# zeropoolnetwork/fawkes-crypto

Hardware: AMD Instinct MI355X
Metric: Groth16 proofs/sec + MSM scalar-muls/sec, BN254, 2^25 constraints (33552553 rows = 99.99 % of the 2^25 domain) (higher is better)
Workload: dtype u32

## Files before the change

### fawkes-crypto_amd/csrc/common.hpp

```cpp
#pragma once
#include <hip/hip_runtime.h>
#include <stdint.h>
#include <stdio.h>
#include <stdlib.h>
#include <map>
#include <string>
#include <new>
#include <stdexcept>
#include <type_traits>
#include <vector>
#include <functional>
#include <initializer_list>
#include "../../include/fawkes_hip.h"
#include "curve.hpp"

namespace fk {

struct DevBuf {
    void *p = nullptr;
    size_t cap = 0;
    hipError_t reserve(size_t bytes) {
        if (bytes <= cap) return hipSuccess;
        if (p) { hipError_t e = hipFree(p); p = nullptr; cap = 0; if (e != hipSuccess) return e; }
        size_t want = bytes + (bytes >> 3) + 256;
        hipError_t e = hipMalloc(&p, want);
        if (e != hipSuccess) { (void)hipGetLastError(); e = hipMalloc(&p, bytes); want = bytes; }
        if (e == hipSuccess) cap = want; else { p = nullptr; (void)hipGetLastError(); }
        return e;
    }
    void release() { if (p) (void)hipFree(p); p = nullptr; cap = 0; }
    template <class T> T *as() const { return (T *)p; }
};

struct CtxScratch {
    DevBuf misc;
    DevBuf ntt_s1, ntt_s2, ntt_io, hbuf, sc_a, sc_b, scan_tmp, stage_a, stage_b, stage_c, stage_z, stage_d;
    DevBuf check;
    DevBuf *begin() { return &misc; }
    DevBuf *end() { return begin() + sizeof(CtxScratch) / sizeof(DevBuf); }
    void release_scratch() { for (DevBuf *b = begin(); b != end(); ++b) b->release(); }
};
static_assert(std::is_standard_layout<CtxScratch>::value && sizeof(CtxScratch) % sizeof(DevBuf) == 0, "CtxScratch holds DevBuf members and nothing else");

struct NttDomain;

struct EventPair { hipEvent_t a, b; uint64_t units; };

struct MsmLane {
    hipStream_t st = nullptr;
    hipEvent_t ev_in = nullptr;
    hipEvent_t ev_sorted = nullptr;
    bool ev_sorted_valid = false;
    DevBuf digits, sorted, totals, starts, perm, overlist, tasktab, partials, s2_cnt1, s2_seg, s2_cnt2, s2_tmp_idx, s2_tmp_lo, buckets;
    DevBuf buckets2;
    const void *last_sort_scalars = nullptr; size_t last_sort_n = 0; unsigned last_sort_c = 0; bool last_merged = false;
};

struct MsmTail {
    bool active = false;
    uint32_t cb = 0, wide = 0, W = 0, nblk = 0;
    hipEvent_t done = nullptr;
    void *h_wp = nullptr;
    size_t h_cap = 0;
    DevBuf d_wp;
};
static constexpr int MSM_TAILS = 12;
static constexpr int MSM_LANES = 4;

struct QueryIdx {
    const uint32_t *a = nullptr, *b = nullptr;
    uint64_t n_a = 0, n_b = 0;
};

struct WitnessQueries {
    const uint8_t *d_a_aux = nullptr, *d_b_in = nullptr, *d_b_aux = nullptr;
    const QueryIdx *idx = nullptr;
};
struct FrontOpts {
    bool defer_back = false;
    bool gather_on_main = false;
};
struct ProveRun {
    WitnessQueries q;
    bool z_recorded = false;
    const std::function<int()> *before_block = nullptr;
};

struct KeyPre {
    void *lev = nullptr;
    size_t n = 0;
    uint32_t cb = 0, wide = 0, W = 0;
};

}

struct fk_ctx : fk::CtxScratch {
    int device = 0;
    hipStream_t stream = nullptr;
    std::string err;
    unsigned window_bits = 0;
    unsigned ntt_threads = 512;
    std::map<uint32_t, fk::NttDomain *> domains;
    fk::MsmLane lanes[fk::MSM_LANES];
    int lane_next = 0, lane_prev = 0;
    int co_tenants = 1;
    int lanes_in_use = fk::MSM_LANES;
    fk::MsmTail tails[fk::MSM_TAILS];
    hipStream_t aux = nullptr;
    hipEvent_t ev_aux = nullptr, ev_main = nullptr, ev_z = nullptr;
    std::vector<std::function<int()>> deferred, deferred_tails;
    hipEvent_t ev_acc_done = nullptr; bool ev_acc_done_valid = false;
    bool wit_active = false;
    struct EarlyFront { bool done = false; int tails[4] = {-1, -1, -1, -1}; const fk_key *key = nullptr; const struct fk_r1cs_dev *r1cs = nullptr; const void *d_z = nullptr; } early;
    int wit_tail[4] = {-1, -1, -1, -1};
    hipStream_t copy_st = nullptr;
    struct WitSlot {
        fk::DevBuf buf; hipEvent_t ready = nullptr; bool pending = false;
        hipEvent_t part = nullptr;
        bool deferred = false; const void *host_z = nullptr; size_t host_bytes = 0;
        const fk_key *key = nullptr; const struct fk_r1cs_dev *r1cs = nullptr; uint64_t r[4], s[4];
    } wslot[2];
    int wslot_next = 0;
    hipEvent_t ev_upload_gate = nullptr;
    hipEvent_t ev_chunk[16] = {nullptr};
    std::vector<fk::EventPair> ev_acc, ev_acc2, ev_ntt;
    std::vector<hipEvent_t> ev_pool;
    uint64_t acc_adds[2] = {0, 0};
    bool stats_on = true;
    bool debug = false;
};

struct fk_key {
    uint64_t m = 0;
    uint32_t num_input = 0, num_aux = 0;
    uint64_t n_h = 0, n_l = 0, n_a = 0, n_b = 0;
    uint32_t shard_index = 0, shard_count = 1;
    uint64_t h_lo = 0, h_hi = 0, l_lo = 0, l_hi = 0, a_lo = 0, a_hi = 0, b_lo = 0, b_hi = 0;
    uint64_t b2_lo = 0, b2_hi = 0;
    fk::G1Affine *d_h = nullptr, *d_l = nullptr, *d_a = nullptr, *d_b1 = nullptr;
    fk::G2Affine *d_b2 = nullptr;
    fk::G1Affine alpha_g1, beta_g1, delta_g1;
    fk::G2Affine beta_g2, delta_g2;
    fk::KeyPre pre_h, pre_l, pre_a, pre_b1, pre_b2;
    double load_s[2] = {0, 0};
};

#define FK_SET_ERR(ctx, code, ...)                                   \
    do {                                                             \
        char _b[512]; snprintf(_b, sizeof _b, __VA_ARGS__);          \
        (ctx)->err = _b;                                             \
        return (code);                                               \
    } while (0)

#define FK_HIP(ctx, expr)                                                                         \
    do {                                                                                          \
        hipError_t _e = (expr);                                                                   \
        if (_e != hipSuccess) {                                                                   \
            char _b[512];                                                                         \
            snprintf(_b, sizeof _b, "%s:%d: %s -> %s", __FILE__, __LINE__, #expr, hipGetErrorString(_e)); \
            (ctx)->err = _b;                                                                      \
            (void)hipGetLastError();    \
            return (_e == hipErrorOutOfMemory) ? FK_ERR_OOM : FK_ERR_HIP;                         \
        }                                                                                         \
    } while (0)

#define FK_DBG(ctx, name)                                                                         \
    do {                                                                                          \
        if ((ctx)->debug) {                                                                       \
            fprintf(stderr, "[fk] launch %s ...", name); fflush(stderr);                          \
            hipError_t _e = hipStreamSynchronize((ctx)->stream);                                  \
            fprintf(stderr, " %s\n", hipGetErrorString(_e)); fflush(stderr);                      \
        }                                                                                         \
    } while (0)

#define FK_TRY(expr) do { int _rc = (expr); if (_rc != FK_OK) return _rc; } while (0)
#define FK_CAT2_(a, b) a##b
#define FK_CAT_(a, b) FK_CAT2_(a, b)
#define FK_RANGE(name) fk::RoctxRange FK_CAT_(fk_range_, __LINE__)(name)

namespace fk {
static inline bool proof_holds_staging(const fk_ctx *ctx) { return ctx->early.done; }
static inline bool proof_holds_lanes(const fk_ctx *ctx) {
    return proof_holds_staging(ctx) || ctx->wit_active || !ctx->deferred.empty() || !ctx->deferred_tails.empty();
}

static inline int scratch_claim(fk_ctx *ctx, const char *who) {
    if (proof_holds_staging(ctx)) FK_SET_ERR(ctx, FK_ERR_BAD_ARG, "%s: an early front of a submitted proof is outstanding (call fk_prove_r1cs_wait first)", who);
    FK_HIP(ctx, hipSetDevice(ctx->device));
    return FK_OK;
}

struct HostStage {
    fk_ctx *ctx;
    size_t align = 16;
    uint8_t *cur = nullptr;
    size_t up(size_t bytes) const { return (bytes + align - 1) & ~(align - 1); }
    int use(DevBuf &buf, std::initializer_list<size_t> sizes, size_t slack = 0) {
        size_t sum = slack;
        for (size_t b : sizes) sum += up(b);
        FK_HIP(ctx, buf.reserve(sum));
        cur = buf.as<uint8_t>();
        return FK_OK;
    }
    template <class T> T *room(size_t bytes) { T *p = (T *)cur; cur += up(bytes); return p; }
    template <class T> int in(const void *host, size_t bytes, T **d) {
        *d = room<T>(bytes);
        if (bytes) FK_HIP(ctx, hipMemcpyAsync((void *)*d, host, bytes, hipMemcpyHostToDevice, ctx->stream));
        return FK_OK;
    }
    template <class T> int room(DevBuf &buf, size_t bytes, T **d) { FK_TRY(use(buf, {bytes})); *d = room<T>(bytes); return FK_OK; }
    template <class T> int in(DevBuf &buf, const void *host, size_t bytes, T **d) { FK_TRY(use(buf, {bytes})); return in(host, bytes, d); }
    int out(void *host, const void *d, size_t bytes, bool last = true) {
        FK_HIP(ctx, hipMemcpyAsync(host, d, bytes, hipMemcpyDeviceToHost, ctx->stream));
        if (last) FK_HIP(ctx, hipStreamSynchronize(ctx->stream));
        return FK_OK;
    }
};
}

template <class C, class F>
static inline int fk_guard(C *c, F &&body) noexcept {
    auto note = [&](const char *msg) noexcept { if (c) { try { c->err = msg; } catch (...) {} } };
    try { return body(); }
    catch (const std::bad_alloc &) { note("out of host memory"); return FK_ERR_OOM; }
    catch (const std::length_error &) { note("out of host memory (a container larger than this host can hold)"); return FK_ERR_OOM; }
    catch (const std::exception &e) { note(e.what()); return FK_ERR_HIP; }
    catch (...) { note("unknown C++ exception"); return FK_ERR_HIP; }
}

namespace fk {

std::string &tls_error();
unsigned host_threads();

struct RoctxApi { int (*push)(const char *) = nullptr; int (*pop)() = nullptr; };
const RoctxApi &roctx_api();
struct RoctxRange {
    bool on;
    explicit RoctxRange(const char *name) { const RoctxApi &r = roctx_api(); on = r.push != nullptr; if (on) (void)r.push(name); }
    ~RoctxRange() { if (on) (void)roctx_api().pop(); }
    RoctxRange(const RoctxRange &) = delete;
    RoctxRange &operator=(const RoctxRange &) = delete;
};

static inline int tune(const char *name, int dflt) {
#ifdef FK_EXPERIMENTS
    const char *e = getenv(name);
    return e ? atoi(e) : dflt;
#else
    (void)name;
    return dflt;
#endif
}

static inline uint32_t ceil_log2_u64(uint64_t n) { uint32_t k = 0; while (((uint64_t)1 << k) < n) k++; return k; }

static inline void h_slice(uint64_t n_h, uint32_t idx, uint32_t cnt, uint64_t *lo, uint64_t *hi) {
    const uint64_t m = n_h + 1;
    uint64_t a = (uint64_t)((unsigned __int128)m * idx / cnt), b = (uint64_t)((unsigned __int128)m * (idx + 1) / cnt);
    if (a > n_h) a = n_h;
    if (b > n_h) b = n_h;
    *lo = a; *hi = b;
}

static inline void work_slices(uint64_t n_l, uint64_t n_a, uint64_t n_b, uint32_t index, uint32_t count, uint64_t out[8], long double handicap = 0.0L) {
    const long double seg_w[4] = {1.0L, 1.0L, 1.0L, (long double)FK_G2_WORK};
    const uint64_t seg_n[4] = {n_l, n_a, n_b, n_b};
    long double total = 0; for (int i = 0; i < 4; i++) total += seg_w[i] * (long double)seg_n[i];
    auto cut = [&](uint32_t g, int seg) -> uint64_t {
        if (g >= count) return seg_n[seg];
        if (g == 0) return 0;
        long double x;
        if (handicap > 0 && count > 1 && handicap * (long double)count >= total + handicap)
            x = total * (long double)(g - 1) / (long double)(count - 1);
        else
            x = (total + handicap) * (long double)g / (long double)count - handicap;
        long double s0 = 0; for (int i = 0; i < seg; i++) s0 += seg_w[i] * (long double)seg_n[i];
        if (x <= s0) return 0;
        const long double q = (x - s0) / seg_w[seg];
        return q >= (long double)seg_n[seg] ? seg_n[seg] : (uint64_t)q;
    };
    for (int seg = 0; seg < 4; seg++) { out[2 * seg] = cut(index, seg); out[2 * seg + 1] = cut(index + 1, seg); }
}

static inline int key_plan_slices(fk_ctx *ctx, fk_key *k, double zlo, double zhi) {
    h_slice(k->n_h, k->shard_index, k->shard_count, &k->h_lo, &k->h_hi);
    auto eq = [&](uint64_t n, uint64_t *lo, uint64_t *hi) {
        *lo = (uint64_t)((unsigned __int128)n * k->shard_index / k->shard_count);
        *hi = (uint64_t)((unsigned __int128)n * (k->shard_index + 1) / k->shard_count);
    };
    auto fr = [&](uint64_t n, uint64_t *olo, uint64_t *ohi) {
        uint64_t a = (uint64_t)((long double)n * zlo + 0.5L), b = zhi >= 1.0 ? n : (uint64_t)((long double)n * zhi + 0.5L);
        if (a > n) a = n;
        if (b > n) b = n;
        if (b < a) b = a;
        *olo = a; *ohi = b;
    };
    if (zlo <= -1.5) {
        uint64_t r[8];
        const bool q0 = zlo <= -2.5 && k->shard_count > 1;
        if (q0) { k->h_lo = k->shard_index == 0 ? 0 : k->n_h; k->h_hi = k->n_h; }
        work_slices(k->n_l, k->n_a, k->n_b, k->shard_index, k->shard_count, r, q0 ? (long double)FK_Q0_HANDICAP * (long double)k->m : 0.0L);
        k->l_lo = r[0]; k->l_hi = r[1]; k->a_lo = r[2]; k->a_hi = r[3]; k->b_lo = r[4]; k->b_hi = r[5]; k->b2_lo = r[6]; k->b2_hi = r[7];
        return FK_OK;
    }
    if (zlo < 0.0) { eq(k->n_l, &k->l_lo, &k->l_hi); eq(k->n_a, &k->a_lo, &k->a_hi); eq(k->n_b, &k->b_lo, &k->b_hi); k->b2_lo = k->b_lo; k->b2_hi = k->b_hi; return FK_OK; }
    if (!(zhi <= 1.0 && zlo <= zhi)) FK_SET_ERR(ctx, FK_ERR_BAD_ARG, "key: bad z fraction range [%g, %g)", zlo, zhi);
    if (k->shard_count == 1 && !(zlo == 0.0 && zhi >= 1.0))
        FK_SET_ERR(ctx, FK_ERR_BAD_ARG, "key: a single shard holds the whole arrays (z_frac_lo = FK_Z_EQUAL_SPLIT or [0, 1)), got [%g, %g)", zlo, zhi);
    fr(k->n_l, &k->l_lo, &k->l_hi); fr(k->n_a, &k->a_lo, &k->a_hi); fr(k->n_b, &k->b_lo, &k->b_hi);
    k->b2_lo = k->b_lo; k->b2_hi = k->b_hi;
    return FK_OK;
}

int stats_begin(fk_ctx *ctx, std::vector<EventPair> &v, uint64_t units, hipStream_t st = nullptr);
int stats_end(fk_ctx *ctx, std::vector<EventPair> &v, hipStream_t st = nullptr);

int ntt_exec_simple(fk_ctx *ctx, Fr *d_data, uint32_t log_n, bool inverse, bool coset);
int quotient_dev(fk_ctx *ctx, Fr *d_a, Fr *d_b, Fr *d_c, uint64_t n, Fr *d_h_out, uint64_t *m_out);
void ntt_free_domains(fk_ctx *ctx);
int fr_mul_batch_dev(fk_ctx *ctx, const Fr *a, const Fr *b, Fr *o, size_t n);
int dq_gather(fk_ctx *ctx, const Fr *d_full, uint64_t n, uint32_t log_m, uint32_t rank, uint32_t log_w, Fr *d_local);
int dq_local(fk_ctx *ctx, Fr *d_x, const Fr *d_xb, const Fr *d_xc, uint32_t log_m, uint32_t rank, uint32_t log_w, int stage);
int dq_cross(fk_ctx *ctx, Fr *d_buf, uint32_t log_m, uint32_t rank, uint32_t log_w, int mode, const Fr *d_sub = nullptr);

int msm_g1_dev(fk_ctx *ctx, const G1Affine *d_bases, const Fr *d_scalars, size_t n, G1Xyzz *out, const KeyPre *pre = nullptr);
int msm_g1_begin(fk_ctx *ctx, const G1Affine *d_bases, const Fr *d_scalars, size_t n, int *tail, hipEvent_t ready = nullptr, const KeyPre *pre = nullptr, bool defer = false);
int msm_g1_end(fk_ctx *ctx, int tail, G1Xyzz *out);
int msm_g2_begin(fk_ctx *ctx, const G2Affine *d_bases, const Fr *d_scalars, size_t n, bool reuse_sort, int *tail, hipEvent_t ready = nullptr, const KeyPre *pre = nullptr, bool defer = false);
int key_precompute(fk_ctx *ctx, fk_key *key);
int key_levels_headroom(fk_ctx *ctx, const fk_key *key, int64_t *bytes);
void key_pre_free(fk_key *key);
int msm_g2_end(fk_ctx *ctx, int tail, G2Xyzz *out);
void msm_abandon(fk_ctx *ctx);
int msm_run_deferred(fk_ctx *ctx, hipEvent_t after);
int upload_deferred(fk_ctx *ctx, bool gate_on_main);
int witness_slot_reserve(fk_ctx *ctx, int slot, size_t bytes, bool *moved = nullptr);
int early_witness_begin(fk_ctx *ctx, const fk_key *key, const void *d_z, const WitnessQueries &q, int tails_out[4]);
bool early_front_applies(const fk_key *key);
int witness_queries_begin(fk_ctx *ctx, const fk_key *key, const void *d_z, const WitnessQueries &q);
int witness_queries_finish(fk_ctx *ctx, const fk_key *key, const void *d_h_slice, uint8_t out[FK_MSM_RESULT_BYTES]);
int prove_msms_dev(fk_ctx *ctx, const fk_key *key, Fr *d_a, Fr *d_b, Fr *d_c, uint64_t n, const Fr *d_z, const ProveRun &run,
                   uint8_t out[FK_MSM_RESULT_BYTES], fk_timings *tm);
int prove_dev(fk_ctx *ctx, const fk_key *key, Fr *d_a, Fr *d_b, Fr *d_c, uint64_t n, const Fr *d_z, const ProveRun &run, const uint64_t r[4],
              const uint64_t s[4], uint8_t out[FK_PROOF_BYTES], fk_timings *tm);
void msm_release(fk_ctx *ctx);
int streams_init(fk_ctx *ctx);
int msm_sync(fk_ctx *ctx);
int msm_g2_dev(fk_ctx *ctx, const G2Affine *d_bases, const Fr *d_scalars, size_t n, G2Xyzz *out, bool reuse_sort = false, const KeyPre *pre = nullptr);
int gen_points_g1(fk_ctx *ctx, G1Affine *d_out, size_t n, uint64_t seed);
int gen_points_g2(fk_ctx *ctx, G2Affine *d_out, size_t n, uint64_t seed);
int gen_scalars(fk_ctx *ctx, Fr *d_out, size_t n, uint64_t seed, int kind);
int gather_scalars(fk_ctx *ctx, const Fr *d_z, const uint32_t *d_idx, size_t n, Fr *d_out, hipStream_t st);
int compact_scalars(fk_ctx *ctx, const Fr *d_z, const uint8_t *d_density, size_t n, Fr *d_out, uint64_t *n_out, hipStream_t st = nullptr);

}
```

### fawkes-crypto_amd/csrc/msm.hip

```cpp
#include "common.hpp"
#include <algorithm>
#include <string.h>
#include <type_traits>

namespace fk {

static constexpr uint32_t SEG_MAX = 4096, SEG_MIN = 256;
static constexpr uint32_t SORT_THREADS = 256;

struct MsmPlan {
    size_t n;
    uint32_t c, W, B;
    uint32_t cb, wide;
    uint32_t nchunks;
    size_t chunk;
    uint32_t cap, cap_top;
    uint32_t L, T, nblk;
    uint32_t LB, nhi, nlo;
};
#ifndef FK_S2_TILE
#define FK_S2_TILE 8192
#endif
static constexpr uint32_t S2_TILE = FK_S2_TILE;
static constexpr uint32_t S2_EPT = S2_TILE / 1024;
// ... 653 lines not shown
        Walker<F> wk;
        for (uint32_t k = lo + threadIdx.x; k < hi; k += 64) {
            const uint32_t e = src[k];
            wk.add(bases[e & 0x7fffffffu], (e >> 31) != 0);
        }
        const Xyzz<F> acc = wk.result();
        static_assert(sizeof(Xyzz<F>) == sizeof(Xyzz<FC>), "layout");
        Xyzz<FC> accc;
        __builtin_memcpy(&accc, &acc, sizeof acc);
        wave_reduce(accc);
        if (threadIdx.x == 0) partials[task] = accc;
    }
}

template <class F>
__global__ __launch_bounds__(256) void msm_overflow_fold_kernel(const OverBucket *ob, const MsmDyn *dyn, const Xyzz<F> *partials, Xyzz<F> *buckets) {
    __shared__ Xyzz<F> sh[4];
    const uint32_t n_obs = dyn->n_obs;
    for (uint32_t i = blockIdx.x; i < n_obs; i += gridDim.x) {
        const OverBucket o = ob[i];
        Xyzz<F> acc = Xyzz<F>::inf();
        for (uint32_t k = threadIdx.x; k < o.ntask; k += 256) acc.add(partials[o.task0 + k]);
        block_reduce_256(acc, sh);
        if (threadIdx.x == 0) { Xyzz<F> b = buckets[o.g]; b.add(acc); buckets[o.g] = b; }
        __syncthreads();
    }
}

__global__ __launch_bounds__(1024) void msm_tasks_kernel(const OverEntry *over, MsmDyn *dyn, uint32_t B, int merged, Task *tasks, uint32_t max_tasks, OverBucket *obs) {
    __shared__ unsigned long long key[OVER_MAX];
    __shared__ uint32_t val[OVER_MAX];
    __shared__ uint32_t t0[OVER_MAX + 1];
    __shared__ uint32_t head[OVER_MAX + 1];
    __shared__ uint32_t wsum[16];
    __shared__ unsigned long long xsum[16];
    const uint32_t tid = threadIdx.x;
    uint32_t n = dyn->n_over; if (n > OVER_MAX) n = OVER_MAX;
    if (n == 0) { if (tid == 0) { dyn->seg = SEG_MIN; dyn->n_tasks = 0; dyn->n_obs = 0; } return; }
    const uint32_t cap = dyn->cap;
    uint32_t npow = 1; while (npow < n) npow <<= 1;
    for (uint32_t i = tid; i < npow; i += 1024) {
        if (i < n) { const OverEntry e = over[i]; key[i] = ((unsigned long long)(merged ? e.g % B : e.g) << 32) | e.g; val[i] = e.size; }
        else { key[i] = ~0ull; val[i] = 0; }
    }
    __syncthreads();
    for (uint32_t k = 2; k <= npow; k <<= 1)
        for (uint32_t j = k >> 1; j > 0; j >>= 1) {
            for (uint32_t i = tid; i < npow; i += 1024) {
                const uint32_t l = i ^ j;
                if (l > i) {
                    const bool up = (i & k) == 0;
                    const unsigned long long a = key[i], b = key[l];
                    if ((a > b) == up) { key[i] = b; key[l] = a; const uint32_t v = val[i]; val[i] = val[l]; val[l] = v; }
                }
            }
            __syncthreads();
        }
    unsigned long long mine = 0;
    for (uint32_t i = tid; i < n; i += 1024) mine += val[i] - cap;
    mine = wave_sum_u64(mine);
    if ((tid & 63) == 0) xsum[tid >> 6] = mine;
    __syncthreads();
    unsigned long long extra_total = 0;
    for (int w = 0; w < 16; w++) extra_total += xsum[w];
    unsigned long long sg = ((extra_total / 2048 + 63) / 64) * 64;
    const uint32_t SEG = (uint32_t)(sg < SEG_MIN ? SEG_MIN : (sg > SEG_MAX ? SEG_MAX : sg));
    const uint32_t per = (n + 1023) / 1024, lo = tid * per, hi = lo + per < n ? lo + per : n;
    uint32_t sum = 0, heads = 0;
    for (uint32_t i = lo; i < hi && lo < n; i++) {
        const uint32_t nt = (val[i] - cap + SEG - 1) / SEG;
        val[i] = nt; sum += nt;
        heads += (i == 0 || (key[i] >> 32) != (key[i - 1] >> 32)) ? 1u : 0u;
    }
    uint32_t n_tasks, n_obs;
    uint32_t run = block_excl_scan_1024(sum, wsum, &n_tasks);
    uint32_t hrun = block_excl_scan_1024(heads, wsum, &n_obs);
    for (uint32_t i = lo; i < hi && lo < n; i++) {
        t0[i] = run; run += val[i];
        if (i == 0 || (key[i] >> 32) != (key[i - 1] >> 32)) head[hrun++] = i;
    }
    if (tid == 0) { t0[n] = n_tasks; head[n_obs] = n; }
    __syncthreads();
    if (n_tasks > max_tasks) { if (tid == 0) { dyn->error = 2; dyn->seg = SEG; dyn->n_tasks = 0; dyn->n_obs = 0; } return; }
    for (uint32_t o = tid; o < n_obs; o += 1024) {
        const uint32_t a = head[o], b = head[o + 1];
        obs[o] = OverBucket{(uint32_t)(merged ? key[a] >> 32 : key[a] & 0xffffffffu), t0[a], t0[b] - t0[a]};
    }
    for (uint32_t t = tid; t < n_tasks; t += 1024) {
        uint32_t l = 0, h = n;
        while (h - l > 1) { const uint32_t mid = (l + h) >> 1; if (t0[mid] <= t) l = mid; else h = mid; }
        tasks[t] = Task{(uint32_t)(key[l] & 0xffffffffu), t - t0[l]};
    }
    if (tid == 0) { dyn->seg = SEG; dyn->n_tasks = n_tasks; dyn->n_obs = n_obs; }
}

template <class F>
__global__ __launch_bounds__(256) void msm_bucket_reduce_kernel(const Xyzz<F> *buckets, uint32_t B, uint32_t L, uint32_t T,
                                                                uint32_t nblk, Xyzz<F> *winparts) {
    __shared__ Xyzz<F> sh[4];
    const uint32_t w = blockIdx.y;
    const uint32_t t = blockIdx.x * 256 + threadIdx.x;
    Xyzz<F> acc = Xyzz<F>::inf();
    if (t < T) {
        Xyzz<F> run = Xyzz<F>::inf();
        const Xyzz<F> *bk = buckets + (size_t)w * B + (size_t)t * L;
        for (uint32_t s = L; s-- > 0;) {
            run.add(bk[s]);
            acc.add(run);
        }
        const uint32_t k = t * L;
        if (k) {
            Xyzz<F> m = Xyzz<F>::inf();
            for (int bit = 31 - __clz(k); bit >= 0; bit--) {
                m = Xyzz<F>::dbl(m);
                if ((k >> bit) & 1) m.add(run);
            }
            acc.add(m);
        }
    }
    block_reduce_256(acc, sh);
    if (threadIdx.x == 0) winparts[(size_t)w * nblk + blockIdx.x] = acc;
}

template <class F>
__global__ __launch_bounds__(256) void msm_fold_partials_kernel(const Xyzz<F> *winparts, uint32_t nblk, Xyzz<F> *out) {
    __shared__ Xyzz<F> sh[4];
    const uint32_t w = blockIdx.x;
    Xyzz<F> acc = Xyzz<F>::inf();
    for (uint32_t b = threadIdx.x; b < nblk; b += 256) acc.add(winparts[(size_t)w * nblk + b]);
    block_reduce_256(acc, sh);
    if (threadIdx.x == 0) out[w] = acc;
}

#define FK_DBG_ST(ctx, st, name)                                                                  \
    do {                                                                                          \
        if ((ctx)->debug) {                                                                       \
            fprintf(stderr, "[fk] launch %s ...", name); fflush(stderr);                          \
            hipError_t _e = hipStreamSynchronize(st);                                             \
            fprintf(stderr, " %s\n", hipGetErrorString(_e)); fflush(stderr);                      \
        }                                                                                         \
    } while (0)

int streams_init(fk_ctx *ctx) {
    if (!ctx->copy_st) FK_HIP(ctx, hipStreamCreateWithFlags(&ctx->copy_st, hipStreamNonBlocking));
    if (!ctx->aux) {
        FK_HIP(ctx, hipStreamCreateWithFlags(&ctx->aux, hipStreamNonBlocking));
        FK_HIP(ctx, hipEventCreateWithFlags(&ctx->ev_aux, hipEventDisableTiming));
    }
    for (MsmLane &ln : ctx->lanes) {
        if (ln.st) continue;
        FK_HIP(ctx, hipStreamCreateWithFlags(&ln.st, hipStreamNonBlocking));
        FK_HIP(ctx, hipEventCreateWithFlags(&ln.ev_in, hipEventDisableTiming));
        FK_HIP(ctx, hipEventCreateWithFlags(&ln.ev_sorted, hipEventDisableTiming));
    }
    for (hipEvent_t *e : {&ctx->ev_main, &ctx->ev_z, &ctx->ev_upload_gate}) if (!*e) FK_HIP(ctx, hipEventCreateWithFlags(e, hipEventDisableTiming));
    return FK_OK;
}

static int pinned_reserve(fk_ctx *ctx, void **p, size_t *cap, size_t bytes, size_t pad) {
    if (bytes + pad <= *cap) return FK_OK;
    if (*p) { FK_HIP(ctx, hipHostFree(*p)); *p = nullptr; *cap = 0; }
    FK_HIP(ctx, hipHostMalloc(p, bytes + (bytes >> 2) + pad, hipHostMallocDefault));
    *cap = bytes + (bytes >> 2) + pad;
    return FK_OK;
}

template <class F>
struct MsmJob {
    fk_ctx *ctx;
    MsmPlan p;
    MsmLane *ln;
    MsmTail *tl;
    const Affine<F> *bases, *lev;
    const Fr *scalars;
    size_t n, WB, max_tasks, max_tiles, wp_bytes;
    uint32_t WR;
    bool merged, have_sort;
    MsmDyn *dyn;
    uint32_t *digits, *sorted, *totals, *starts, *perm;
    Task *tasks;
    OverBucket *obs;
    Xyzz<F> *winparts;
};

template <class F>
static int msm_reserve(MsmJob<F> &j) {
    fk_ctx *ctx = j.ctx;
    const MsmPlan &p = j.p;
    MsmLane &ln = *j.ln;
    MsmTail &tl = *j.tl;
    const size_t n = j.n, WB = j.WB = (size_t)p.W * p.B;
    j.WR = j.merged ? 1 : p.W;
    j.wp_bytes = (size_t)j.WR * sizeof(Xyzz<F>);
    const size_t wp_dev_bytes = (size_t)j.WR * (p.nblk + 1) * sizeof(Xyzz<F>);
    const size_t max_tasks = j.max_tasks = std::max<size_t>(2048, (size_t)p.W * n / SEG_MAX) + OVER_MAX + 64;
    const uint32_t nseg = p.W * p.nhi;
    const size_t max_tiles = j.max_tiles = (size_t)p.W * ((n + S2_TILE - 1) / S2_TILE) + nseg + 1;
    struct Need { DevBuf *b; size_t bytes; };
    const Need needs[] = {
        {&ln.digits, (size_t)p.W * n * 4}, {&ln.sorted, (size_t)p.W * n * 4}, {&ln.totals, WB * 4}, {&ln.starts, WB * 4},
        {&ln.perm, WB * 4 + SIZE_BINS * 4}, {&ln.overlist, OVER_MAX * sizeof(OverEntry) + sizeof(MsmDyn) + 64}, {j.have_sort ? &ln.buckets2 : &ln.buckets, WB * sizeof(Xyzz<F>)},
        {&ln.tasktab, max_tasks * sizeof(Task) + OVER_MAX * sizeof(OverBucket) + 64}, {&ln.partials, max_tasks * sizeof(Xyzz<F>)},
        {&ln.s2_cnt1, (size_t)p.W * p.nchunks * p.nhi * 4}, {&ln.s2_seg, ((size_t)nseg * 4 + 2) * 4}, {&ln.s2_cnt2, max_tiles * p.nlo * 4},
        {&ln.s2_tmp_idx, (size_t)p.W * n * 4}, {&ln.s2_tmp_lo, (size_t)p.W * n * 2}};
    bool grow = false;
    for (const Need &nd : needs) grow = grow || nd.bytes > nd.b->cap;
    if (grow) {
        FK_HIP(ctx, hipStreamSynchronize(ln.st));
        for (const Need &nd : needs) FK_HIP(ctx, nd.b->reserve(nd.bytes));
        if (!j.have_sort) ln.last_sort_scalars = nullptr;
    }
    FK_HIP(ctx, tl.d_wp.reserve(wp_dev_bytes));
    FK_TRY(pinned_reserve(ctx, &tl.h_wp, &tl.h_cap, j.wp_bytes, 16));
    j.dyn = (MsmDyn *)((char *)ln.overlist.p + OVER_MAX * sizeof(OverEntry));
    j.tasks = ln.tasktab.as<Task>();
    j.obs = (OverBucket *)((char *)ln.tasktab.p + ((max_tasks * sizeof(Task) + 15) & ~(size_t)15));
    j.digits = ln.digits.as<uint32_t>(); j.sorted = ln.sorted.as<uint32_t>();
    j.totals = ln.totals.as<uint32_t>(); j.starts = ln.starts.as<uint32_t>();
    j.winparts = tl.d_wp.as<Xyzz<F>>();
    j.perm = ln.perm.as<uint32_t>();
    return FK_OK;
}

static void launch_scatter2(const MsmPlan &p, uint32_t n_tiles, hipStream_t st, const uint32_t *tmp_idx, const uint16_t *tmp_lo, size_t n, const uint32_t *tile_start, uint32_t nseg,
                            const uint32_t *seg_start, const uint32_t *seg_size, const uint32_t *cnt2, const uint32_t *starts, uint32_t *sorted) {
    const auto kernel = p.nlo <= 1024 ? s2_scatter2_kernel<1024> : (p.nlo <= 2048 ? s2_scatter2_kernel<2048> : s2_scatter2_kernel<4096>);
    hipLaunchKernelGGL(kernel, dim3(n_tiles), dim3(1024), 0, st, tmp_idx, tmp_lo, n, p.nhi, p.nlo, p.B, tile_start, nseg, seg_start, seg_size, cnt2, starts, sorted);
}

template <class F>
static int queue_sort(const MsmJob<F> &j) {
    fk_ctx *ctx = j.ctx;
    const MsmPlan &p = j.p;
    MsmLane &ln = *j.ln;
    hipStream_t st = ln.st;
    const size_t n = j.n;
    const uint32_t nseg = p.W * p.nhi;
    ln.last_sort_scalars = nullptr;
    hipLaunchKernelGGL(msm_digits_kernel, dim3((unsigned)(((n + 1) / 2 + 63) / 64)), dim3(64), 0, st, j.scalars, n, p.cb, p.wide, p.W, j.digits);
    FK_HIP(ctx, hipGetLastError());
    FK_DBG_ST(ctx, st, "msm_digits");
    FK_HIP(ctx, hipMemsetAsync(j.dyn, 0, sizeof(MsmDyn), st));
    uint32_t *cnt1 = ln.s2_cnt1.as<uint32_t>();
    uint32_t *seg_size = ln.s2_seg.as<uint32_t>(), *seg_start = seg_size + nseg, *seg_tiles = seg_start + nseg, *tile_start = seg_tiles + nseg;
    uint32_t *cnt2 = ln.s2_cnt2.as<uint32_t>(), *tmp_idx = ln.s2_tmp_idx.as<uint32_t>();
    uint16_t *tmp_lo = ln.s2_tmp_lo.as<uint16_t>();
    hipLaunchKernelGGL(s2_hist1_kernel, dim3(p.nchunks, p.W), dim3(SORT_THREADS), p.nhi * 4, st, j.digits, n, p.chunk, p.nchunks, p.LB, p.nhi, cnt1);
    hipLaunchKernelGGL(s2_prefix1_kernel, dim3(p.W), dim3(1024), p.nhi * 4, st, cnt1, p.nchunks, p.nhi, seg_size, seg_start, seg_tiles);
    hipLaunchKernelGGL(s2_tile_prefix_kernel, dim3(1), dim3(1024), 0, st, seg_tiles, nseg, tile_start);
    hipLaunchKernelGGL(s2_scatter1_n1024_kernel, dim3(p.nchunks, p.W), dim3(1024), 0, st, j.digits, n, p.chunk, p.nchunks, p.LB, p.nhi, cnt1, seg_start, tmp_idx, tmp_lo);
    FK_HIP(ctx, hipGetLastError());
    FK_DBG_ST(ctx, st, "msm_sort_pass1");
    const uint32_t n_tiles = (uint32_t)j.max_tiles;
    hipLaunchKernelGGL(s2_hist2_kernel, dim3(n_tiles), dim3(256), p.nlo * 4, st, tmp_lo, n, p.nhi, p.nlo, tile_start, nseg, seg_start, seg_size, cnt2);
    hipLaunchKernelGGL(s2_prefix2_kernel, dim3((nseg + 3) / 4), dim3(256), 0, st, cnt2, nseg, p.nhi, p.nlo, p.B, tile_start, seg_start, p.cap ? p.cap : 1u, j.totals, j.starts, j.dyn);
    launch_scatter2(p, n_tiles, st, tmp_idx, tmp_lo, n, tile_start, nseg, seg_start, seg_size, cnt2, j.starts, j.sorted);
    FK_HIP(ctx, hipGetLastError());
    FK_DBG_ST(ctx, st, "msm_sort_pass2");
    ln.last_sort_scalars = (const void *)j.scalars; ln.last_sort_n = n; ln.last_sort_c = p.c; ln.last_merged = j.merged;
    return FK_OK;
}

template <class F>
static int queue_size_order(const MsmJob<F> &j) {
    fk_ctx *ctx = j.ctx;
    const MsmPlan &p = j.p;
    MsmLane &ln = *j.ln;
    hipStream_t st = ln.st;
    const size_t WB = j.WB;
    MsmDyn *dyn = j.dyn;
    uint32_t *totals = j.totals, *perm = j.perm, *size_bins = perm + WB;
    unsigned long long *d_adds = &dyn->adds;
    static const int t_many = tune("FK_MSM_OVER_MANY", 2048);
    const uint32_t many = (uint32_t)std::min<size_t>(std::max<size_t>((size_t)t_many, WB / 8192), OVER_MAX - 64);
    hipLaunchKernelGGL(msm_cap_kernel, dim3(1), dim3(64), 0, st, dyn, p.cap ? p.cap : 1u, many);
    hipLaunchKernelGGL(msm_over_list_kernel, dim3((unsigned)((WB + 255) / 256)), dim3(256), 0, st, totals, WB, ln.overlist.as<OverEntry>(), dyn);
    hipLaunchKernelGGL(msm_tasks_kernel, dim3(1), dim3(1024), 0, st, ln.overlist.as<OverEntry>(), dyn, p.B, j.merged ? 1 : 0, j.tasks, (uint32_t)j.max_tasks, j.obs);
    FK_HIP(ctx, hipMemsetAsync(size_bins, 0, SIZE_BINS * 4, st));
    if (j.merged) {
        uint32_t *mt = perm + p.B;
        hipLaunchKernelGGL(msm_merge_totals_kernel, dim3(std::min<uint32_t>((p.B + 255) / 256, 1024)), dim3(256), 0, st, totals, p.B, p.W, dyn, mt, d_adds);
        hipLaunchKernelGGL(msm_size_hist_kernel, dim3((unsigned)std::min<size_t>((p.B + 255) / 256, 1024)), dim3(256), 0, st, mt, (size_t)p.B, dyn, p.W, size_bins, (unsigned long long *)nullptr);
        hipLaunchKernelGGL(msm_size_scan_kernel, dim3(1), dim3(SIZE_BINS), 0, st, size_bins);
        hipLaunchKernelGGL(msm_size_scatter_kernel, dim3((unsigned)((p.B + 1023) / 1024)), dim3(1024), 0, st, mt, (size_t)p.B, dyn, p.W, size_bins, perm);
    } else {
        hipLaunchKernelGGL(msm_size_hist_kernel, dim3((unsigned)std::min<size_t>((WB + 255) / 256, 1024)), dim3(256), 0, st, totals, WB, dyn, 1u, size_bins, d_adds);
        hipLaunchKernelGGL(msm_size_scan_kernel, dim3(1), dim3(SIZE_BINS), 0, st, size_bins);
        hipLaunchKernelGGL(msm_size_scatter_kernel, dim3((unsigned)((WB + 1023) / 1024)), dim3(1024), 0, st, totals, WB, dyn, 1u, size_bins, perm);
    }
    FK_HIP(ctx, hipGetLastError());
    FK_DBG_ST(ctx, st, "msm_size_order");
    if (ctx->debug) {
        MsmDyn h{};
        FK_HIP(ctx, hipMemcpy(&h, dyn, sizeof h, hipMemcpyDeviceToHost));
        fprintf(stderr, "[fk] msm n=%zu c=%u (W=%u: %u x %u bits + %u x %u bits) cap=%u (plan %u): %u oversized buckets, %u tasks of %u entries, %u fold groups\n", j.n, p.c,
                p.W, p.wide, p.cb + 1, p.W - p.wide, p.cb, h.cap, p.cap, h.n_over, h.n_tasks, h.seg, h.n_obs);
        fflush(stderr);
    }
    return FK_OK;
}

template <class F>
static Xyzz<F> *bucket_buf(const MsmJob<F> &j) { return (j.have_sort ? j.ln->buckets2 : j.ln->buckets).template as<Xyzz<F>>(); }

template <class F>
static int queue_accumulate(MsmJob<F> j) {
    fk_ctx *ctx = j.ctx;
    const MsmPlan &p = j.p;
    hipStream_t st = j.ln->st;
    constexpr int MINW = std::is_same<F, Fq>::value ? 4 : 2;
    Xyzz<F> *buckets = bucket_buf(j);
    std::vector<EventPair> &evv = (sizeof(F) == sizeof(Fq)) ? ctx->ev_acc : ctx->ev_acc2;
    FK_TRY(stats_begin(ctx, evv, (uint64_t)j.n, st));
    if (j.merged)
        hipLaunchKernelGGL(HIP_KERNEL_NAME(msm_accumulate_merged_kernel<F, MINW>), dim3((p.B + 255) / 256), dim3(256), 0, st, j.bases, j.lev, j.sorted, j.n,
                           j.starts, j.totals, p.B, p.W, j.dyn, j.perm, j.perm + p.B, buckets);
    else
        hipLaunchKernelGGL(HIP_KERNEL_NAME(msm_accumulate_kernel<F, MINW>), dim3((unsigned)((j.WB + 255) / 256)), dim3(256), 0, st, j.bases, j.sorted, j.n,
                           j.starts, j.totals, p.B, p.W, j.dyn, j.perm, buckets);
    FK_HIP(ctx, hipGetLastError());
    FK_TRY(stats_end(ctx, evv, st));
    if (!ctx->ev_acc_done) FK_HIP(ctx, hipEventCreateWithFlags(&ctx->ev_acc_done, hipEventDisableTiming));
    FK_HIP(ctx, hipEventRecord(ctx->ev_acc_done, st)); ctx->ev_acc_done_valid = true;
    FK_DBG_ST(ctx, st, "msm_accumulate");
    return FK_OK;
}

template <class F>
static int queue_tail(MsmJob<F> j) {
    using FC = typename ColdOf<F>::type;
    fk_ctx *ctx = j.ctx;
    const MsmPlan &p = j.p;
    MsmLane &ln = *j.ln;
    MsmTail &tl = *j.tl;
    hipStream_t st = ln.st;
    Xyzz<F> *buckets = bucket_buf(j);
    hipLaunchKernelGGL(HIP_KERNEL_NAME(msm_overflow_kernel<F, FC>), dim3(2048), dim3(64), 0, st,
                       j.bases, j.lev, j.sorted, j.n, j.starts, j.totals, p.B, j.dyn, j.tasks, ln.partials.as<Xyzz<FC>>());
    FK_HIP(ctx, hipGetLastError());
    FK_DBG_ST(ctx, st, "msm_overflow");
    hipLaunchKernelGGL(HIP_KERNEL_NAME(msm_overflow_fold_kernel<F>), dim3(256), dim3(256), 0, st, j.obs, j.dyn, ln.partials.as<Xyzz<F>>(), buckets);
    FK_HIP(ctx, hipGetLastError());
    FK_DBG_ST(ctx, st, "msm_overflow_fold");
    hipLaunchKernelGGL(HIP_KERNEL_NAME(msm_bucket_reduce_kernel<F>), dim3(p.nblk, j.WR), dim3(256), 0, st, buckets, p.B, p.L, p.T, p.nblk, j.winparts);
    Xyzz<F> *folded = j.winparts + (size_t)j.WR * p.nblk;
    hipLaunchKernelGGL(HIP_KERNEL_NAME(msm_fold_partials_kernel<F>), dim3(j.WR), dim3(256), 0, st, j.winparts, p.nblk, folded);
    FK_HIP(ctx, hipGetLastError());
    FK_HIP(ctx, hipMemcpyAsync(tl.h_wp, folded, j.wp_bytes, hipMemcpyDeviceToHost, st));
    FK_HIP(ctx, hipMemcpyAsync((char *)tl.h_wp + j.wp_bytes, &j.dyn->adds, 8, hipMemcpyDeviceToHost, st));
    FK_HIP(ctx, hipMemcpyAsync((char *)tl.h_wp + j.wp_bytes + 8, &j.dyn->error, 4, hipMemcpyDeviceToHost, st));
    FK_HIP(ctx, hipEventRecord(tl.done, st));
    FK_DBG_ST(ctx, st, "msm_bucket_reduce");
    return FK_OK;
}

static void lanes_advance(fk_ctx *ctx, int li, bool defer = false) {
    static const int t_lanes = tune("FK_MSM_LANES", 0);
    const int n_lanes = (t_lanes >= 1 && t_lanes <= MSM_LANES && !defer && ctx->deferred.empty())
                            ? t_lanes : (ctx->lanes_in_use >= 2 && ctx->lanes_in_use <= MSM_LANES ? ctx->lanes_in_use : MSM_LANES);
    ctx->lane_prev = li; ctx->lane_next = (li + 1) % n_lanes;
}

template <class F>
static int msm_begin(fk_ctx *ctx, const Affine<F> *d_bases, const Fr *d_scalars, size_t n, bool reuse_sort, int *tail_out, hipEvent_t ready, const KeyPre *pre = nullptr, bool defer = false) {
    *tail_out = -1;
    if (n == 0) return FK_OK;
    if (n >= ((size_t)1 << 31)) FK_SET_ERR(ctx, FK_ERR_BAD_ARG, "msm: n too large");
    int ti = -1;
    for (int i = 0; i < MSM_TAILS; i++) if (!ctx->tails[i].active) { ti = i; break; }
    if (ti < 0) FK_SET_ERR(ctx, FK_ERR_BAD_ARG, "msm: too many outstanding multiplications");
    MsmTail &tl = ctx->tails[ti];
    if (!tl.done) FK_HIP(ctx, hipEventCreateWithFlags(&tl.done, hipEventDisableTiming));
    MsmPlan p = make_plan(n, ctx->window_bits);
    bool merged = false;
    if (pre && pre->lev && pre->n == n) {
        const MsmPlan pm = make_plan(n, ctx->window_bits, true);
        if (pm.cb == pre->cb && pm.wide == pre->wide && pm.W == pre->W) { p = pm; merged = true; }
    }
    MsmLane &prev = ctx->lanes[ctx->lane_prev];
    const bool have_sort = reuse_sort && prev.st && prev.last_sort_scalars == (const void *)d_scalars && prev.last_sort_n == n && prev.last_sort_c == p.c && prev.last_merged == merged;
    const int li = have_sort ? ctx->lane_prev : ctx->lane_next;
    MsmLane &ln = ctx->lanes[li];
    if (!ln.st) FK_SET_ERR(ctx, FK_ERR_HIP, "msm: the context's streams were not created");
    lanes_advance(ctx, li, defer);
    if (ready) FK_HIP(ctx, hipStreamWaitEvent(ln.st, ready, 0));
    else {
        FK_HIP(ctx, hipEventRecord(ln.ev_in, ctx->stream));
        FK_HIP(ctx, hipStreamWaitEvent(ln.st, ln.ev_in, 0));
    }
    MsmJob<F> job{};
    job.ctx = ctx; job.p = p; job.ln = &ln; job.tl = &tl;
    job.bases = d_bases; job.lev = merged ? (const Affine<F> *)pre->lev : nullptr; job.scalars = d_scalars;
    job.n = n; job.merged = merged; job.have_sort = have_sort;
    FK_TRY(msm_reserve(job));
    if (!have_sort) {
        FK_TRY(queue_sort(job));
        FK_TRY(queue_size_order(job));
        FK_HIP(ctx, hipEventRecord(ln.ev_sorted, ln.st)); ln.ev_sorted_valid = true;
    }
    tl.active = true; tl.cb = p.cb; tl.wide = p.wide; tl.W = job.WR; tl.nblk = 1;
    *tail_out = ti;
    if (defer) {
        ctx->deferred.push_back([job] { return queue_accumulate<F>(job); });
        ctx->deferred_tails.push_back([job] { return queue_tail<F>(job); });
        return FK_OK;
    }
    FK_TRY(queue_accumulate<F>(job));
    return queue_tail<F>(job);
}

int msm_run_deferred(fk_ctx *ctx, hipEvent_t after) {
    if (after) for (MsmLane &ln : ctx->lanes) if (ln.st) FK_HIP(ctx, hipStreamWaitEvent(ln.st, after, 0));
    std::vector<std::function<int()>> accs, tails;
    accs.swap(ctx->deferred); tails.swap(ctx->deferred_tails);
    for (auto &f : accs) FK_TRY(f());
    for (auto &f : tails) FK_TRY(f());
    return FK_OK;
}

template <class F>
static int msm_end(fk_ctx *ctx, int tail, Xyzz<F> *out) {
    *out = Xyzz<F>::inf();
    if (tail < 0) return FK_OK;
    if (tail >= MSM_TAILS || !ctx->tails[tail].active) FK_SET_ERR(ctx, FK_ERR_BAD_ARG, "msm: bad tail handle");
    MsmTail &tl = ctx->tails[tail];
    tl.active = false;
    FK_HIP(ctx, hipEventSynchronize(tl.done));
    const Xyzz<F> *wp = (const Xyzz<F> *)tl.h_wp;
    { const char *extra = (const char *)tl.h_wp + (size_t)tl.W * tl.nblk * sizeof(Xyzz<F>);
      uint64_t adds; uint32_t err;
      memcpy(&adds, extra, 8); memcpy(&err, extra + 8, 4);
      ctx->acc_adds[sizeof(F) == sizeof(Fq) ? 0 : 1] += adds;
      if (err) FK_SET_ERR(ctx, FK_ERR_HIP, "msm: the oversized-bucket tables overflowed (%s)", err == 1 ? "more than OVER_MAX buckets above the cap" : "more segment tasks than the bound"); }
    Xyzz<F> acc = Xyzz<F>::inf();
    for (uint32_t w = tl.W; w-- > 0;) {
        const uint32_t cw = tl.cb + (w < tl.wide ? 1 : 0);
        for (uint32_t k = 0; k < cw; k++) acc = Xyzz<F>::dbl(acc);
        for (uint32_t b = 0; b < tl.nblk; b++) acc.add(wp[(size_t)w * tl.nblk + b]);
    }
    *out = acc;
    if (ctx->debug) { fprintf(stderr, "[fk] msm host horner done\n"); fflush(stderr); }
    return FK_OK;
}

int msm_sync(fk_ctx *ctx) {
    if (ctx->aux) FK_HIP(ctx, hipStreamSynchronize(ctx->aux));
    for (MsmLane &ln : ctx->lanes) if (ln.st) FK_HIP(ctx, hipStreamSynchronize(ln.st));
    return FK_OK;
}

void msm_abandon(fk_ctx *ctx) {
    ctx->wit_active = false;
    ctx->early.done = false;
    ctx->deferred.clear(); ctx->deferred_tails.clear();
    if (ctx->aux) (void)hipStreamSynchronize(ctx->aux);
    for (int i = 0; i < MSM_TAILS; i++) ctx->tails[i].active = false;
    for (MsmLane &ln : ctx->lanes) { if (ln.st) (void)hipStreamSynchronize(ln.st); ln.last_sort_scalars = nullptr; }
}

void msm_release(fk_ctx *ctx) {
    if (ctx->aux) { (void)hipStreamSynchronize(ctx->aux); (void)hipStreamDestroy(ctx->aux); ctx->aux = nullptr; }
    if (ctx->ev_aux) { (void)hipEventDestroy(ctx->ev_aux); ctx->ev_aux = nullptr; }
    if (ctx->ev_main) { (void)hipEventDestroy(ctx->ev_main); ctx->ev_main = nullptr; }
    if (ctx->ev_z) { (void)hipEventDestroy(ctx->ev_z); ctx->ev_z = nullptr; }
    if (ctx->ev_upload_gate) { (void)hipEventDestroy(ctx->ev_upload_gate); ctx->ev_upload_gate = nullptr; }
    for (hipEvent_t &e : ctx->ev_chunk) if (e) { (void)hipEventDestroy(e); e = nullptr; }
    if (ctx->ev_acc_done) { (void)hipEventDestroy(ctx->ev_acc_done); ctx->ev_acc_done = nullptr; ctx->ev_acc_done_valid = false; }
    for (MsmLane &ln : ctx->lanes) {
        if (ln.st) (void)hipStreamSynchronize(ln.st);
        for (DevBuf *b : {&ln.digits, &ln.sorted, &ln.totals, &ln.starts, &ln.perm, &ln.overlist, &ln.tasktab, &ln.partials, &ln.s2_cnt1, &ln.s2_seg,
                          &ln.s2_cnt2, &ln.s2_tmp_idx, &ln.s2_tmp_lo, &ln.buckets, &ln.buckets2})
            b->release();
        if (ln.ev_in) (void)hipEventDestroy(ln.ev_in);
        if (ln.ev_sorted) (void)hipEventDestroy(ln.ev_sorted);
        if (ln.st) (void)hipStreamDestroy(ln.st);
        ln = MsmLane();
    }
    for (int i = 0; i < MSM_TAILS; i++) {
        MsmTail &tl = ctx->tails[i];
        if (tl.done) (void)hipEventDestroy(tl.done);
        if (tl.h_wp) (void)hipHostFree(tl.h_wp);
        tl.d_wp.release();
        tl = MsmTail();
    }
}

int msm_g1_begin(fk_ctx *ctx, const G1Affine *d_bases, const Fr *d_scalars, size_t n, int *tail, hipEvent_t ready, const KeyPre *pre, bool defer) {
    return msm_begin<Fq>(ctx, d_bases, d_scalars, n, false, tail, ready, pre, defer);
}
int msm_g1_end(fk_ctx *ctx, int tail, G1Xyzz *out) { return msm_end<Fq>(ctx, tail, out); }
int msm_g2_begin(fk_ctx *ctx, const G2Affine *d_bases, const Fr *d_scalars, size_t n, bool reuse_sort, int *tail, hipEvent_t ready, const KeyPre *pre, bool defer) {
    return msm_begin<Fq2>(ctx, d_bases, d_scalars, n, reuse_sort, tail, ready, pre, defer);
}
int msm_g2_end(fk_ctx *ctx, int tail, G2Xyzz *out) { return msm_end<Fq2>(ctx, tail, out); }

template <class F>
static int msm_run(fk_ctx *ctx, const Affine<F> *d_bases, const Fr *d_scalars, size_t n, Xyzz<F> *out, bool reuse_sort = false, const KeyPre *pre = nullptr) {
    int tail = -1;
    *out = Xyzz<F>::inf();
    FK_TRY(msm_begin<F>(ctx, d_bases, d_scalars, n, reuse_sort, &tail, nullptr, pre));
    return msm_end<F>(ctx, tail, out);
}

int msm_g1_dev(fk_ctx *ctx, const G1Affine *d_bases, const Fr *d_scalars, size_t n, G1Xyzz *out, const KeyPre *pre) {
    return msm_run<Fq>(ctx, d_bases, d_scalars, n, out, false, pre);
}
int msm_g2_dev(fk_ctx *ctx, const G2Affine *d_bases, const Fr *d_scalars, size_t n, G2Xyzz *out, bool reuse_sort, const KeyPre *pre) {
    return msm_run<Fq2>(ctx, d_bases, d_scalars, n, out, reuse_sort, pre);
}

static void msm_plan_info(size_t n, unsigned window_bits, bool merged, fk_msm_plan_info *out) {
    const MsmPlan p = make_plan(n, window_bits, merged);
    *out = fk_msm_plan_info{(uint64_t)p.n, (uint64_t)p.chunk, p.c, p.W, p.B, p.cb, p.wide, p.nchunks, p.cap, p.L, p.T, p.nblk, p.LB, p.nhi, p.nlo,
                            S1_TILE, S2_TILE, S2_MAX_HI, OVER_MAX, SEG_MIN, SEG_MAX, SIZE_BINS};
}

static int msm_front_dump(fk_ctx *ctx, const Fr *d_scalars, size_t n, bool merged, uint32_t *digits, uint32_t *sorted, uint32_t *totals, uint32_t *starts,
                          uint32_t *perm, fk_msm_dyn_info *dyn_out, uint32_t *tasks, size_t tasks_cap, uint32_t *obs, size_t obs_cap) {
    if (n == 0) return FK_OK;
    if (n >= ((size_t)1 << 31)) FK_SET_ERR(ctx, FK_ERR_BAD_ARG, "msm: n too large");
    if (proof_holds_lanes(ctx)) FK_SET_ERR(ctx, FK_ERR_BAD_ARG, "msm front dump: a proof is in flight on this context");
    int ti = -1;
    for (int i = 0; i < MSM_TAILS; i++) if (!ctx->tails[i].active) { ti = i; break; }
    if (ti < 0) FK_SET_ERR(ctx, FK_ERR_BAD_ARG, "msm: too many outstanding multiplications");
    const int li = ctx->lane_next;
    MsmLane &ln = ctx->lanes[li];
    if (!ln.st) FK_SET_ERR(ctx, FK_ERR_HIP, "msm: the context's streams were not created");
    lanes_advance(ctx, li);
    FK_HIP(ctx, hipEventRecord(ln.ev_in, ctx->stream));
    FK_HIP(ctx, hipStreamWaitEvent(ln.st, ln.ev_in, 0));
    MsmJob<Fq> job{};
    job.ctx = ctx; job.p = make_plan(n, ctx->window_bits, merged); job.ln = &ln; job.tl = &ctx->tails[ti];
    job.scalars = d_scalars; job.n = n; job.merged = merged;
    const MsmPlan &p = job.p;
    FK_TRY(msm_reserve(job));
    FK_TRY(queue_sort(job));
    FK_TRY(queue_size_order(job));
    ln.last_sort_scalars = nullptr;
    FK_HIP(ctx, hipStreamSynchronize(ln.st));
    const size_t Wn = (size_t)p.W * n, WB = job.WB;
    FK_HIP(ctx, hipMemcpy(digits, job.digits, Wn * 4, hipMemcpyDeviceToHost));
    FK_HIP(ctx, hipMemcpy(sorted, job.sorted, Wn * 4, hipMemcpyDeviceToHost));
    FK_HIP(ctx, hipMemcpy(totals, job.totals, WB * 4, hipMemcpyDeviceToHost));
    FK_HIP(ctx, hipMemcpy(starts, job.starts, WB * 4, hipMemcpyDeviceToHost));
    FK_HIP(ctx, hipMemcpy(perm, job.perm, (merged ? 2 * (size_t)p.B : WB) * 4, hipMemcpyDeviceToHost));
    MsmDyn h{};
    FK_HIP(ctx, hipMemcpy(&h, job.dyn, sizeof h, hipMemcpyDeviceToHost));
    *dyn_out = fk_msm_dyn_info{h.cap, h.n_over, h.seg, h.n_tasks, h.n_obs, h.error, (uint64_t)h.adds};
    static_assert(sizeof(Task) == 8 && sizeof(OverBucket) == 12, "fk_msm_front_dump hands these out as 2 and 3 words");
    const size_t nt = std::min<size_t>(std::min<size_t>(h.n_tasks, job.max_tasks), tasks_cap), no = std::min<size_t>(std::min<size_t>(h.n_obs, OVER_MAX), obs_cap);
    if (nt) FK_HIP(ctx, hipMemcpy(tasks, job.tasks, nt * sizeof(Task), hipMemcpyDeviceToHost));
    if (no) FK_HIP(ctx, hipMemcpy(obs, job.obs, no * sizeof(OverBucket), hipMemcpyDeviceToHost));
    return FK_OK;
}

template <class F>
static int precompute_levels(fk_ctx *ctx, const Affine<F> *d_bases, size_t n, KeyPre *out, const char *name, bool require, size_t reserve) {
    *out = KeyPre();
    const char *e = getenv("FK_MSM_PRE_MIN_LOG2");
    const int min_lg = e ? atoi(e) : 21;
    if (min_lg < 6 || min_lg > 40 || n + n / 2 < ((size_t)1 << min_lg)) return FK_OK;
    const MsmPlan p = make_plan(n, ctx->window_bits, true);
    if (p.W < 2) return FK_OK;
    const size_t bytes = (size_t)(p.W - 1) * n * sizeof(Affine<F>);
    size_t fr = 0, tot = 0;
    FK_HIP(ctx, hipMemGetInfo(&fr, &tot));
    void *lev = nullptr;
    const bool fits = bytes + reserve <= fr;
    if (!fits || hipMalloc(&lev, bytes) != hipSuccess) {
        (void)hipGetLastError();
        char msg[320];
        snprintf(msg, sizeof msg, "key: fixed-base levels of %s (%zu points, %.1f GiB) do not fit into the %.1f GiB of free HBM", name, n,
                 (double)bytes / (double)(1ull << 30), (double)fr / (double)(1ull << 30));
        if (require) { ctx->err = std::string(msg) + " and FK_MSM_PRECOMP=require"; return FK_ERR_OOM; }
        ctx->err += (ctx->err.empty() ? "warning: " : "; ") + std::string(msg) + " -- that array takes the slower W-bucket-set path";
        return FK_OK;
    }
    const Affine<F> *prev = d_bases;
    for (uint32_t w = 1; w < p.W; w++) {
        Affine<F> *cur = (Affine<F> *)lev + (size_t)(w - 1) * n;
        const uint32_t bits = p.cb + ((w - 1) < p.wide ? 1 : 0);
        constexpr int NB = sizeof(F) == sizeof(Fq) ? 4 : 2;
        hipLaunchKernelGGL(HIP_KERNEL_NAME(msm_level_kernel<F, NB>), dim3((unsigned)(((n + NB - 1) / NB + 255) / 256)), dim3(256), 0, ctx->stream, prev, n, bits, cur);
        prev = cur;
    }
    if (hipGetLastError() != hipSuccess || hipStreamSynchronize(ctx->stream) != hipSuccess) { (void)hipFree(lev); FK_SET_ERR(ctx, FK_ERR_HIP, "msm: level precomputation failed"); }
    out->lev = lev; out->n = n; out->cb = p.cb; out->wide = p.wide; out->W = p.W;
    return FK_OK;
}

void key_pre_free(fk_key *k) {
    for (KeyPre *p : {&k->pre_h, &k->pre_l, &k->pre_a, &k->pre_b1, &k->pre_b2}) { if (p->lev) (void)hipFree(p->lev); *p = KeyPre(); }
}

static size_t proof_scratch_still_needed(fk_ctx *ctx, const fk_key *k) {
    const size_t pts = (size_t)(k->h_hi - k->h_lo) + (k->l_hi - k->l_lo) + (k->a_hi - k->a_lo) + std::max(k->b_hi - k->b_lo, k->b2_hi - k->b2_lo);
    const size_t nv = (size_t)k->num_input + k->num_aux;
    const size_t nmax = std::max<size_t>(std::max<size_t>(k->h_hi - k->h_lo, k->l_hi - k->l_lo), std::max<size_t>(k->a_hi - k->a_lo, std::max(k->b_hi - k->b_lo, k->b2_hi - k->b2_lo)));
    const MsmPlan pl = make_plan(nmax, ctx->window_bits, true);
    const size_t lane_fixed = (size_t)pl.W * pl.B * (MSM_LANES * (sizeof(Xyzz<Fq>) + 16) + sizeof(Xyzz<Fq2>)) + ((size_t)1 << 30);
    const uint64_t h_held = k->h_hi - k->h_lo;
    const size_t quot = h_held == 0 ? 0 : h_held >= k->n_h ? (size_t)k->m * 32 * (6 + 10) : (size_t)k->m * 32 * 6 + (size_t)k->m / k->shard_count * 32 * 10;
    const size_t need = pts * 14 * 13 + lane_fixed + quot + 2 * nv * 32;
    size_t have = 0;
    for (const MsmLane &ln : ctx->lanes)
        for (const DevBuf *b : {&ln.digits, &ln.sorted, &ln.totals, &ln.starts, &ln.perm, &ln.overlist, &ln.tasktab, &ln.partials, &ln.s2_cnt1, &ln.s2_seg,
                                &ln.s2_cnt2, &ln.s2_tmp_idx, &ln.s2_tmp_lo, &ln.buckets, &ln.buckets2}) have += b->cap;
    for (const DevBuf *b : {&ctx->ntt_s1, &ctx->ntt_s2, &ctx->ntt_io, &ctx->hbuf, &ctx->sc_a, &ctx->sc_b, &ctx->stage_a, &ctx->stage_b, &ctx->stage_c, &ctx->stage_z,
                            &ctx->stage_d, &ctx->wslot[0].buf, &ctx->wslot[1].buf}) have += b->cap;
    return (need > have ? need - have : 0) * (size_t)std::max(1, ctx->co_tenants);
}

int key_levels_headroom(fk_ctx *ctx, const fk_key *k, int64_t *bytes) {
    size_t fr = 0, tot = 0;
    FK_HIP(ctx, hipMemGetInfo(&fr, &tot));
    *bytes = (int64_t)fr - (int64_t)proof_scratch_still_needed(ctx, k) - ((int64_t)2 << 30);
    return FK_OK;
}

int key_precompute(fk_ctx *ctx, fk_key *k) {
    const char *e = getenv("FK_MSM_PRECOMP");
    const bool require = e && !strcmp(e, "require");
    const int on = e && !require ? atoi(e) : 1;
    key_pre_free(k);
    ctx->err.clear();
    if (!on) return FK_OK;
    const size_t reserve = proof_scratch_still_needed(ctx, k) + ((size_t)8 << 30);
    struct Cand { const char *name; int which; size_t n, bytes; double worth; };
    std::vector<Cand> cand;
    const bool b_shared = k->b2_lo == k->b_lo && k->b2_hi == k->b_hi && k->d_b1 && k->d_b2;
    auto level_bytes = [&](size_t n, size_t pt) -> size_t {
        const char *e2 = getenv("FK_MSM_PRE_MIN_LOG2");
        const int min_lg = e2 ? atoi(e2) : 21;
        if (min_lg < 6 || min_lg > 40 || n + n / 2 < ((size_t)1 << min_lg)) return 0;
        const MsmPlan p = make_plan(n, ctx->window_bits, true);
        return p.W < 2 ? 0 : (size_t)(p.W - 1) * n * pt;
    };
    auto add_cand = [&](const char *name, int which, const void *d, size_t n, size_t pt, double w) {
        const size_t b = d ? level_bytes(n, pt) : 0;
        if (b) cand.push_back({name, which, n, b, w * (double)n});
    };
    add_cand("h", 0, k->d_h, k->h_hi - k->h_lo, 64, 1.0);
    add_cand("l", 1, k->d_l, k->l_hi - k->l_lo, 64, 1.0);
    add_cand("a", 2, k->d_a, k->a_hi - k->a_lo, 64, 1.0);
    if (b_shared) {
        const size_t nb = k->b_hi - k->b_lo, bb = level_bytes(nb, 64 + 128);
        if (bb) cand.push_back({"b_g1 + b_g2", 5, nb, bb, (1.0 + (double)FK_G2_WORK) * (double)nb});
    } else {
        add_cand("b_g1", 3, k->d_b1, k->b_hi - k->b_lo, 64, 1.0);
        add_cand("b_g2", 4, k->d_b2, k->b2_hi - k->b2_lo, 128, (double)FK_G2_WORK);
    }
    size_t fr = 0, tot = 0;
    FK_HIP(ctx, hipMemGetInfo(&fr, &tot));
    const size_t budget = fr > reserve ? fr - reserve : 0;
    uint32_t best = 0; double best_w = -1; size_t best_b = 0;
    for (uint32_t mask = 0; mask < (1u << cand.size()); mask++) {
        size_t b = 0; double w = 0;
        for (size_t i = 0; i < cand.size(); i++) if ((mask >> i) & 1) { b += cand[i].bytes; w += cand[i].worth; }
        if (b <= budget && (w > best_w || (w == best_w && b < best_b))) { best = mask; best_w = w; best_b = b; }
    }
    for (size_t i = 0; i < cand.size(); i++) {
        const Cand &c = cand[i];
        if (!((best >> i) & 1)) {
            char msg[320];
            snprintf(msg, sizeof msg, "key: fixed-base levels of %s (%zu points, %.1f GiB) left out: %.1f GiB of HBM are free for levels and the arrays chosen instead carry more work",
                     c.name, c.n, (double)c.bytes / (double)(1ull << 30), (double)budget / (double)(1ull << 30));
            if (require) { ctx->err = std::string(msg) + " and FK_MSM_PRECOMP=require"; return FK_ERR_OOM; }
            ctx->err += (ctx->err.empty() ? "warning: " : "; ") + std::string(msg) + " -- that array takes the slower W-bucket-set path";
            continue;
        }
        switch (c.which) {
            case 0: FK_TRY(precompute_levels<Fq>(ctx, k->d_h, c.n, &k->pre_h, "h", require, 0)); break;
            case 1: FK_TRY(precompute_levels<Fq>(ctx, k->d_l, c.n, &k->pre_l, "l", require, 0)); break;
            case 2: FK_TRY(precompute_levels<Fq>(ctx, k->d_a, c.n, &k->pre_a, "a", require, 0)); break;
            case 3: FK_TRY(precompute_levels<Fq>(ctx, k->d_b1, c.n, &k->pre_b1, "b_g1", require, 0)); break;
            case 4: FK_TRY(precompute_levels<Fq2>(ctx, k->d_b2, c.n, &k->pre_b2, "b_g2", require, 0)); break;
            default:
                FK_TRY(precompute_levels<Fq2>(ctx, k->d_b2, c.n, &k->pre_b2, "b_g2", require, 0));
                FK_TRY(precompute_levels<Fq>(ctx, k->d_b1, c.n, &k->pre_b1, "b_g1", require, 0));
                if (k->pre_b2.lev && !k->pre_b1.lev) { (void)hipFree(k->pre_b2.lev); k->pre_b2 = KeyPre(); }
                if (k->pre_b1.lev && !k->pre_b2.lev) { (void)hipFree(k->pre_b1.lev); k->pre_b1 = KeyPre(); }
        }
    }
    return FK_OK;
}

static __host__ __device__ inline uint64_t splitmix64(uint64_t &s) {
    s += 0x9E3779B97F4A7C15ull;
    uint64_t z = s;
    z = (z ^ (z >> 30)) * 0xBF58476D1CE4E5B9ull;
    z = (z ^ (z >> 27)) * 0x94D049BB133111EBull;
    return z ^ (z >> 31);
}

template <class F>
__global__ __launch_bounds__(64) void gen_points_kernel(Affine<F> gen, Affine<F> step, Affine<F> *out, size_t n, uint32_t per, uint64_t seed) {
    size_t t = (size_t)blockIdx.x * blockDim.x + threadIdx.x;
    size_t lo = t * per;
    if (lo >= n) return;
    uint64_t s = seed ^ (0xA0761D6478BD642Full * (t + 1));
    uint32_t k[8];
    for (int i = 0; i < 4; i++) { uint64_t v = splitmix64(s); k[2 * i] = (uint32_t)v; k[2 * i + 1] = (uint32_t)(v >> 32); }
    k[7] &= 0x0fffffffu;
    Xyzz<F> acc = Xyzz<F>::inf();
    for (int i = 251; i >= 0; i--) {
        acc = Xyzz<F>::dbl(acc);
        if ((k[i >> 5] >> (i & 31)) & 1) acc.add_mixed(gen);
    }
    size_t hi = lo + per < n ? lo + per : n;
    for (size_t i = lo; i < hi; i++) {
        out[i] = acc.to_affine();
        acc.add_mixed(step);
    }
}

static G1Affine g1_generator() { G1Affine g; g.x = Fq::from_u64(1); g.y = Fq::from_u64(2); return g; }
static Fq fq_words(const uint32_t (&w)[8]) { Fq t; for (int i = 0; i < 8; i++) t.v[i] = w[i]; return t; }
static G2Affine g2_generator() {
    const uint32_t x0[8] = FK_G2_GEN_X0, x1[8] = FK_G2_GEN_X1, y0[8] = FK_G2_GEN_Y0, y1[8] = FK_G2_GEN_Y1;
    G2Affine g;
    g.x.c0 = fq_words(x0); g.x.c1 = fq_words(x1);
    g.y.c0 = fq_words(y0); g.y.c1 = fq_words(y1);
    return g;
}

template <class F>
static int gen_points(fk_ctx *ctx, const Affine<F> &gen, Affine<F> *d_out, size_t n, uint64_t seed) {
    if (!n) return FK_OK;
    uint64_t s = seed * 0x9E3779B97F4A7C15ull + 12345;
    uint32_t kd[8];
    for (int i = 0; i < 4; i++) { uint64_t v = splitmix64(s); kd[2 * i] = (uint32_t)v; kd[2 * i + 1] = (uint32_t)(v >> 32); }
    kd[7] &= 0x0fffffffu; kd[0] |= 1;
    Affine<F> step = Xyzz<F>::mul_scalar(Xyzz<F>::from_affine(gen), kd).to_affine();
    const uint32_t per = 16;
    const size_t threads = (n + per - 1) / per;
    using FC = typename ColdOf<F>::type;
    Affine<FC> genc, stepc;
    static_assert(sizeof(genc) == sizeof(gen), "layout");
    memcpy(&genc, &gen, sizeof gen); memcpy(&stepc, &step, sizeof step);
    hipLaunchKernelGGL(HIP_KERNEL_NAME(gen_points_kernel<FC>), dim3((unsigned)((threads + 63) / 64)), dim3(64), 0, ctx->stream, genc, stepc,
                       reinterpret_cast<Affine<FC> *>(d_out), n, per, seed);
    FK_HIP(ctx, hipGetLastError());
    return FK_OK;
}
int gen_points_g1(fk_ctx *ctx, G1Affine *d_out, size_t n, uint64_t seed) { return gen_points<Fq>(ctx, g1_generator(), d_out, n, seed); }
int gen_points_g2(fk_ctx *ctx, G2Affine *d_out, size_t n, uint64_t seed) { return gen_points<Fq2>(ctx, g2_generator(), d_out, n, seed); }

__global__ void gen_scalars_kernel(Fr *out, size_t n, uint64_t seed, int kind) {
    size_t i = (size_t)blockIdx.x * blockDim.x + threadIdx.x;
    if (i >= n) return;
    uint64_t s = seed ^ (0xE7037ED1A0B428DBull * (i + 1));
    Fr v;
    for (int k = 0; k < 4; k++) { uint64_t x = splitmix64(s); v.v[2 * k] = (uint32_t)x; v.v[2 * k + 1] = (uint32_t)(x >> 32); }
    v.v[7] &= 0x3fffffffu;
    v = Fr::reduce_once(v);
    if (kind == 1) {
        uint64_t sel = splitmix64(s);
        if (sel & 1) { for (int k = 0; k < 8; k++) v.v[k] = 0; v.v[0] = (uint32_t)((sel >> 1) & 1); }
    } else if (kind == 2) {
        const uint32_t sel = (uint32_t)(splitmix64(s) >> 32) >> 12;
        if (sel < 55575u) { for (int k = 0; k < 8; k++) v.v[k] = 0; }
        else if (sel < 55575u + 26214u) { for (int k = 0; k < 8; k++) v.v[k] = 0; v.v[0] = 1; }
    }
    out[i] = Fr::to_mont(v);
}
int gen_scalars(fk_ctx *ctx, Fr *d_out, size_t n, uint64_t seed, int kind) {
    if (!n) return FK_OK;
    hipLaunchKernelGGL(gen_scalars_kernel, dim3((unsigned)((n + 255) / 256)), dim3(256), 0, ctx->stream, d_out, n, seed, kind);
    FK_HIP(ctx, hipGetLastError());
    return FK_OK;
}

static constexpr uint32_t CP_BLOCK = 2048;

__global__ __launch_bounds__(256) void compact_count_kernel(const uint8_t *dens, size_t n, uint32_t *blk) {
    __shared__ uint32_t sh[256];
    const size_t base = (size_t)blockIdx.x * CP_BLOCK + (size_t)threadIdx.x * 8;
    uint32_t c = 0;
    for (int k = 0; k < 8; k++) if (base + k < n && dens[base + k]) c++;
    sh[threadIdx.x] = c;
    __syncthreads();
    for (uint32_t off = 128; off; off >>= 1) { if (threadIdx.x < off) sh[threadIdx.x] += sh[threadIdx.x + off]; __syncthreads(); }
    if (threadIdx.x == 0) blk[blockIdx.x] = sh[0];
}
__global__ __launch_bounds__(1024) void scan_small_kernel(uint32_t *v, uint32_t n, uint32_t *total) {
    __shared__ uint32_t part[1024];
    const uint32_t tid = threadIdx.x, ipt = (n + 1023) / 1024;
    const uint32_t lo = tid * ipt, hi = lo + ipt < n ? lo + ipt : n;
    uint32_t sum = 0;
    for (uint32_t i = lo; i < hi && lo < n; i++) sum += v[i];
    part[tid] = sum;
    __syncthreads();
    for (uint32_t off = 1; off < 1024; off <<= 1) {
        uint32_t x = tid >= off ? part[tid - off] : 0;
        __syncthreads();
        part[tid] += x;
        __syncthreads();
    }
    uint32_t run = part[tid] - sum;
    for (uint32_t i = lo; i < hi && lo < n; i++) { uint32_t x = v[i]; v[i] = run; run += x; }
    if (tid == 1023) *total = part[1023];
}
__global__ __launch_bounds__(256) void compact_scatter_kernel(const Fr *z, const uint8_t *dens, size_t n, const uint32_t *blk, Fr *out) {
    __shared__ uint32_t sh[256];
    const size_t base = (size_t)blockIdx.x * CP_BLOCK + (size_t)threadIdx.x * 8;
    uint32_t c = 0;
    for (int k = 0; k < 8; k++) if (base + k < n && dens[base + k]) c++;
    sh[threadIdx.x] = c;
    __syncthreads();
    for (uint32_t off = 1; off < 256; off <<= 1) {
        uint32_t x = threadIdx.x >= off ? sh[threadIdx.x - off] : 0;
        __syncthreads();
        sh[threadIdx.x] += x;
        __syncthreads();
    }
    size_t pos = (size_t)blk[blockIdx.x] + sh[threadIdx.x] - c;
    for (int k = 0; k < 8; k++) if (base + k < n && dens[base + k]) out[pos++] = z[base + k];
}

__global__ __launch_bounds__(256) void gather_scalars_kernel(const Fr *z, const uint32_t *idx, size_t n, Fr *out) {
    const size_t i = (size_t)blockIdx.x * blockDim.x + threadIdx.x;
    if (i < n) out[i] = z[idx[i]];
}

int gather_scalars(fk_ctx *ctx, const Fr *d_z, const uint32_t *d_idx, size_t n, Fr *d_out, hipStream_t st) {
    if (!n) return FK_OK;
    hipLaunchKernelGGL(gather_scalars_kernel, dim3((unsigned)((n + 63) / 64)), dim3(64), 0, st, d_z, d_idx, n, d_out);
    FK_HIP(ctx, hipGetLastError());
    return FK_OK;
}

int compact_scalars(fk_ctx *ctx, const Fr *d_z, const uint8_t *d_density, size_t n, Fr *d_out, uint64_t *n_out, hipStream_t st) {
    *n_out = 0;
    if (!n) return FK_OK;
    if (!st) st = ctx->stream;
    const uint32_t nb = (uint32_t)((n + CP_BLOCK - 1) / CP_BLOCK);
    FK_HIP(ctx, ctx->scan_tmp.reserve((size_t)nb * 4 + 16));
    uint32_t *blk = ctx->scan_tmp.as<uint32_t>();
    uint32_t *d_total = blk + nb;
// ... 29 lines not shown
```

### fawkes-crypto_amd/csrc/prover.hip

```cpp
#include <execinfo.h>
#include <signal.h>
#include <unistd.h>
#include "common.hpp"
#include <chrono>
#include <mutex>
#include <string.h>
#include <stdlib.h>

using namespace fk;

namespace fk {

int stats_begin(fk_ctx *ctx, std::vector<EventPair> &v, uint64_t units, hipStream_t st) {
    if (!ctx->stats_on) return FK_OK;
    if (v.size() >= 4096) {
        for (auto &old : v) { ctx->ev_pool.push_back(old.a); ctx->ev_pool.push_back(old.b); }
        v.clear();
    }
    EventPair ep{};
    ep.units = units;
    for (hipEvent_t *e : {&ep.a, &ep.b}) {
        if (!ctx->ev_pool.empty()) { *e = ctx->ev_pool.back(); ctx->ev_pool.pop_back(); }
        else FK_HIP(ctx, hipEventCreate(e));
    }
    FK_HIP(ctx, hipEventRecord(ep.a, st ? st : ctx->stream));
    v.push_back(ep);
    return FK_OK;
}
int stats_end(fk_ctx *ctx, std::vector<EventPair> &v, hipStream_t st) {
    if (!ctx->stats_on) return FK_OK;
    FK_HIP(ctx, hipEventRecord(v.back().b, st ? st : ctx->stream));
    return FK_OK;
}

static void g1_to_raw(uint8_t out[64], const G1Xyzz &p) { G1Affine a = p.to_affine(); memcpy(out, &a, 64); }
static void g2_to_raw(uint8_t out[128], const G2Xyzz &p) { G2Affine a = p.to_affine(); memcpy(out, &a, 128); }
static G1Affine g1_from_raw(const uint8_t *b) { G1Affine a; memcpy(&a, b, 64); return a; }
static G2Affine g2_from_raw(const uint8_t *b) { G2Affine a; memcpy(&a, b, 128); return a; }

static void slice(uint64_t n, uint32_t idx, uint32_t cnt, uint64_t *lo, uint64_t *hi) {
    *lo = (uint64_t)((unsigned __int128)n * idx / cnt);
    *hi = (uint64_t)((unsigned __int128)n * (idx + 1) / cnt);
}

static double now_ms() {
    return std::chrono::duration<double, std::milli>(std::chrono::steady_clock::now().time_since_epoch()).count();
}

}

static_assert(sizeof(G1Affine) == 64 && sizeof(G2Affine) == 128 && sizeof(Fr) == 32, "raw layouts");

extern "C" {

int fk_init(int device_id, fk_ctx **out) {
    if (!out) return FK_ERR_BAD_ARG;
    *out = nullptr;
    int ndev = 0;
    if (hipGetDeviceCount(&ndev) != hipSuccess || ndev <= 0) return FK_ERR_HIP;
    if (device_id < 0 || device_id >= ndev) return FK_ERR_BAD_ARG;
    if (hipSetDevice(device_id) != hipSuccess) return FK_ERR_HIP;
    fk_ctx *ctx = new fk_ctx();
    ctx->device = device_id;
    { const char *d = getenv("FK_DEBUG"); ctx->debug = d && d[0] && d[0] != '0'; }
    { const char *t = getenv("FK_CO_TENANTS"); if (t) { const int v = atoi(t); if (v >= 1 && v <= 64) ctx->co_tenants = v; } }
    if (ctx->debug || getenv("FK_BACKTRACE")) {
        static std::once_flag once;
        std::call_once(once, [] {
            void *warm[4];
            (void)backtrace(warm, 4);
            static struct sigaction prev_segv, prev_abrt;
            auto h = +[](int sig, siginfo_t *info, void *uctx) {
                void *bt[64];
                const int n = backtrace(bt, 64);
                const char msg[] = "[fk] fatal signal, native backtrace:\n";
                (void)!write(2, msg, sizeof msg - 1);
                backtrace_symbols_fd(bt, n, 2);
                const struct sigaction &prev = sig == SIGSEGV ? prev_segv : prev_abrt;
                if ((prev.sa_flags & SA_SIGINFO) && prev.sa_sigaction) { prev.sa_sigaction(sig, info, uctx); return; }
                if (!(prev.sa_flags & SA_SIGINFO) && prev.sa_handler != SIG_DFL && prev.sa_handler != SIG_IGN && prev.sa_handler) { prev.sa_handler(sig); return; }
                signal(sig, SIG_DFL); raise(sig);
            };
            struct sigaction sa;
            memset(&sa, 0, sizeof sa);
            sa.sa_sigaction = h;
            sa.sa_flags = SA_SIGINFO | SA_ONSTACK;
            sigemptyset(&sa.sa_mask);
            sigaction(SIGSEGV, &sa, &prev_segv);
            sigaction(SIGABRT, &sa, &prev_abrt);
        });
    }
    { const int v = tune("FK_NTT_THREADS", 512); if (v == 64 || v == 128 || v == 256 || v == 512 || v == 1024) ctx->ntt_threads = (unsigned)v; }
    if (hipStreamCreate(&ctx->stream) != hipSuccess) { delete ctx; return FK_ERR_HIP; }
    if (streams_init(ctx) != FK_OK) { fk_free(ctx); return FK_ERR_HIP; }
    *out = ctx;
    return FK_OK;
}

void fk_free(fk_ctx *ctx) {
    if (!ctx) return;
    (void)hipSetDevice(ctx->device);
    (void)hipStreamSynchronize(ctx->stream);
    ntt_free_domains(ctx);
    msm_release(ctx);
    ctx->release_scratch();
    for (auto &v : {&ctx->ev_acc, &ctx->ev_acc2, &ctx->ev_ntt}) for (auto &ep : *v) { (void)hipEventDestroy(ep.a); (void)hipEventDestroy(ep.b); }
    for (hipEvent_t e : ctx->ev_pool) (void)hipEventDestroy(e);
    if (ctx->copy_st) { (void)hipStreamSynchronize(ctx->copy_st); (void)hipStreamDestroy(ctx->copy_st); }
    for (auto &w : ctx->wslot) { w.buf.release(); if (w.ready) (void)hipEventDestroy(w.ready); if (w.part) (void)hipEventDestroy(w.part); }
    (void)hipStreamDestroy(ctx->stream);
    delete ctx;
}

const char *fk_last_error(const fk_ctx *ctx) { return ctx ? ctx->err.c_str() : fk::tls_error().c_str(); }

int fk_trim(fk_ctx *ctx) { return fk_guard(ctx, [&]() -> int {
    if (!ctx) return FK_ERR_BAD_ARG;
    FK_HIP(ctx, hipSetDevice(ctx->device));
    for (const auto &w : ctx->wslot) if (w.pending) FK_SET_ERR(ctx, FK_ERR_BAD_ARG, "trim: a submitted proof is outstanding (call fk_prove_r1cs_wait first)");
    if (proof_holds_lanes(ctx)) FK_SET_ERR(ctx, FK_ERR_BAD_ARG, "trim: multiplications are in flight");
    for (const auto &t : ctx->tails) if (t.active) FK_SET_ERR(ctx, FK_ERR_BAD_ARG, "trim: a multiplication begun with a *_begin_* call has not been collected");
    FK_HIP(ctx, hipStreamSynchronize(ctx->stream));
    FK_TRY(msm_sync(ctx));
    if (ctx->copy_st) FK_HIP(ctx, hipStreamSynchronize(ctx->copy_st));
    ntt_free_domains(ctx);
    msm_release(ctx);
    ctx->release_scratch();
    for (auto &w : ctx->wslot) { w.buf.release(); w.deferred = false; if (w.ready) { (void)hipEventDestroy(w.ready); w.ready = nullptr; } if (w.part) { (void)hipEventDestroy(w.part); w.part = nullptr; } }
    ctx->lane_prev = 0; ctx->lane_next = 0;
    FK_TRY(streams_init(ctx));
    return FK_OK;
}); }

int fk_set_window_bits(fk_ctx *ctx, unsigned c) { return fk_guard(ctx, [&]() -> int {
    if (!ctx) return FK_ERR_BAD_ARG;
    if (c != 0 && (c < 2 || c > 22)) FK_SET_ERR(ctx, FK_ERR_BAD_ARG, "window bits must be 0 or 2..22");
    ctx->window_bits = c;
    return FK_OK;
}); }

int fk_dev_alloc(fk_ctx *ctx, size_t bytes, void **dptr) { return fk_guard(ctx, [&]() -> int {
    if (!ctx || !dptr) return FK_ERR_BAD_ARG;
    FK_HIP(ctx, hipSetDevice(ctx->device));
    FK_HIP(ctx, hipMalloc(dptr, bytes ? bytes : 16));
    return FK_OK;
}); }
int fk_dev_free(fk_ctx *ctx, void *dptr) { return fk_guard(ctx, [&]() -> int {
    if (!ctx) return FK_ERR_BAD_ARG;
    if (dptr) FK_HIP(ctx, hipFree(dptr));
    return FK_OK;
}); }
int fk_upload(fk_ctx *ctx, void *dptr, const void *host, size_t bytes) { return fk_guard(ctx, [&]() -> int {
    if (!ctx) return FK_ERR_BAD_ARG;
    if (bytes) FK_HIP(ctx, hipMemcpyAsync(dptr, host, bytes, hipMemcpyHostToDevice, ctx->stream));
    FK_HIP(ctx, hipStreamSynchronize(ctx->stream));
    return FK_OK;
// ... 34 lines not shown
int fk_witness_upload_async(fk_ctx *ctx, int slot, const void *z_host, size_t bytes) { return fk_guard(ctx, [&]() -> int {
    if (!ctx) return FK_ERR_BAD_ARG;
    if (slot < 0 || slot > 1 || (bytes && !z_host)) FK_SET_ERR(ctx, FK_ERR_BAD_ARG, "witness upload: slot must be 0 or 1, buffer non-null");
    FK_TRY(witness_slot_reserve(ctx, slot, bytes));
    fk_ctx::WitSlot &w = ctx->wslot[slot];
    if (bytes) FK_HIP(ctx, hipMemcpyAsync(w.buf.p, z_host, bytes, hipMemcpyHostToDevice, ctx->copy_st));
    FK_HIP(ctx, hipEventRecord(w.ready, ctx->copy_st));
    return FK_OK;
}); }
int fk_witness_slot(fk_ctx *ctx, int slot, size_t total_bytes, void **dptr, void **copy_stream) { return fk_guard(ctx, [&]() -> int {
    if (!ctx) return FK_ERR_BAD_ARG;
    if (slot < 0 || slot > 1) FK_SET_ERR(ctx, FK_ERR_BAD_ARG, "witness slot must be 0 or 1");
    FK_TRY(witness_slot_reserve(ctx, slot, total_bytes));
    if (dptr) *dptr = ctx->wslot[slot].buf.p;
    if (copy_stream) *copy_stream = (void *)ctx->copy_st;
    return FK_OK;
}); }
int fk_witness_upload_part_async(fk_ctx *ctx, int slot, const void *z_host_part, size_t offset, size_t len) { return fk_guard(ctx, [&]() -> int {
    if (!ctx) return FK_ERR_BAD_ARG;
    if (slot < 0 || slot > 1 || (len && !z_host_part)) FK_SET_ERR(ctx, FK_ERR_BAD_ARG, "witness upload: slot must be 0 or 1, buffer non-null");
    fk_ctx::WitSlot &w = ctx->wslot[slot];
    if (!w.ready || offset + len > w.buf.cap) FK_SET_ERR(ctx, FK_ERR_BAD_ARG, "witness upload: piece [%zu, %zu) outside the slot (call fk_witness_slot first)", offset, offset + len);
    FK_HIP(ctx, hipSetDevice(ctx->device));
    if (len) FK_HIP(ctx, hipMemcpyAsync((uint8_t *)w.buf.p + offset, z_host_part, len, hipMemcpyHostToDevice, ctx->copy_st));
    FK_HIP(ctx, hipEventRecord(w.part, ctx->copy_st));
    return FK_OK;
}); }
int fk_witness_mark_ready(fk_ctx *ctx, int slot) { return fk_guard(ctx, [&]() -> int {
    if (!ctx) return FK_ERR_BAD_ARG;
    if (slot < 0 || slot > 1 || !ctx->wslot[slot].ready) FK_SET_ERR(ctx, FK_ERR_BAD_ARG, "witness slot %d holds nothing", slot);
    FK_HIP(ctx, hipSetDevice(ctx->device));
    FK_HIP(ctx, hipEventRecord(ctx->wslot[slot].ready, ctx->copy_st));
    return FK_OK;
}); }
int fk_witness_ptr(fk_ctx *ctx, int slot, void **dptr) { return fk_guard(ctx, [&]() -> int {
    if (!ctx || !dptr) return FK_ERR_BAD_ARG;
    if (slot < 0 || slot > 1 || !ctx->wslot[slot].ready) FK_SET_ERR(ctx, FK_ERR_BAD_ARG, "witness slot %d holds nothing", slot);
    FK_HIP(ctx, hipSetDevice(ctx->device));
    FK_HIP(ctx, hipStreamWaitEvent(ctx->stream, ctx->wslot[slot].ready, 0));
    *dptr = ctx->wslot[slot].buf.p;
    return FK_OK;
}); }

}
namespace fk {
int witness_slot_reserve(fk_ctx *ctx, int slot, size_t bytes, bool *moved) {
    FK_HIP(ctx, hipSetDevice(ctx->device));
    if (!ctx->copy_st) FK_HIP(ctx, hipStreamCreateWithFlags(&ctx->copy_st, hipStreamNonBlocking));
    fk_ctx::WitSlot &w = ctx->wslot[slot];
    if (!w.ready) FK_HIP(ctx, hipEventCreateWithFlags(&w.ready, hipEventDisableTiming));
    if (!w.part) FK_HIP(ctx, hipEventCreateWithFlags(&w.part, hipEventDisableTiming));
    if (moved) *moved = false;
    if (bytes > w.buf.cap) {
        FK_HIP(ctx, hipStreamSynchronize(ctx->copy_st));
        FK_HIP(ctx, hipStreamSynchronize(ctx->stream));
        FK_TRY(msm_sync(ctx));
        FK_HIP(ctx, w.buf.reserve(bytes));
        if (moved) *moved = true;
    }
    return FK_OK;
}
int upload_deferred(fk_ctx *ctx, bool gate_on_main) {
    for (int s = 0; s < 2; s++) {
        fk_ctx::WitSlot &w = ctx->wslot[s];
        if (!w.deferred) continue;
        w.deferred = false;
        if (gate_on_main) {
            FK_HIP(ctx, hipEventRecord(ctx->ev_upload_gate, ctx->stream));
            FK_HIP(ctx, hipStreamWaitEvent(ctx->copy_st, ctx->ev_upload_gate, 0));
        }
        FK_TRY(fk_witness_upload_async(ctx, s, w.host_z, w.host_bytes));
    }
    return FK_OK;
}
}
extern "C" {

static int key_alloc_slices(fk_ctx *ctx, fk_key *k, double zlo, double zhi) {
    FK_TRY(key_plan_slices(ctx, k, zlo, zhi));
    FK_HIP(ctx, hipMalloc((void **)&k->d_h, (k->h_hi - k->h_lo) * 64 + 64));
    FK_HIP(ctx, hipMalloc((void **)&k->d_l, (k->l_hi - k->l_lo) * 64 + 64));
    FK_HIP(ctx, hipMalloc((void **)&k->d_a, (k->a_hi - k->a_lo) * 64 + 64));
    FK_HIP(ctx, hipMalloc((void **)&k->d_b1, (k->b_hi - k->b_lo) * 64 + 64));
    FK_HIP(ctx, hipMalloc((void **)&k->d_b2, (k->b2_hi - k->b2_lo) * 128 + 128));
    return FK_OK;
}

void fk_key_free(fk_ctx *ctx, fk_key *k) {
    if (!k) return;
    if (ctx) (void)hipSetDevice(ctx->device);
    for (void *p : {(void *)k->d_h, (void *)k->d_l, (void *)k->d_a, (void *)k->d_b1, (void *)k->d_b2}) if (p) (void)hipFree(p);
    key_pre_free(k);
    delete k;
}

static int key_check_shape(fk_ctx *ctx, uint64_t m, uint32_t num_input, uint64_t n_h, uint64_t n_l, uint32_t num_aux,
                           uint32_t shard_index, uint32_t shard_count) {
    if (m == 0 || (m & (m - 1))) FK_SET_ERR(ctx, FK_ERR_BAD_ARG, "key: m must be a power of two");
    if (m > ((uint64_t)1 << (FK_FR_S - 1))) FK_SET_ERR(ctx, FK_ERR_DOMAIN_TOO_LARGE, "key: m exceeds 2^%d", FK_FR_S - 1);
    if (num_input == 0) FK_SET_ERR(ctx, FK_ERR_BAD_ARG, "key: num_input must include the constant ONE");
    if (n_h != m - 1) FK_SET_ERR(ctx, FK_ERR_KEY_MISMATCH, "key: h must hold m-1 points");
    if (n_l != num_aux) FK_SET_ERR(ctx, FK_ERR_KEY_MISMATCH, "key: l must hold num_aux points");
    if (shard_count == 0 || shard_index >= shard_count) FK_SET_ERR(ctx, FK_ERR_BAD_ARG, "key: bad shard %u/%u", shard_index, shard_count);
    return FK_OK;
}
int fk_key_load(fk_ctx *ctx, const fk_key_desc *d, fk_key **out) { return fk_guard(ctx, [&]() -> int {
    FK_RANGE("fk_key_load");
    if (!ctx || !d || !out) return FK_ERR_BAD_ARG;
    *out = nullptr;
    FK_HIP(ctx, hipSetDevice(ctx->device));
    FK_TRY(key_check_shape(ctx, d->m, d->num_input, d->n_h, d->n_l, d->num_aux, d->shard_index, d->shard_count));
    if (!d->alpha_g1 || !d->beta_g1 || !d->delta_g1 || !d->beta_g2 || !d->delta_g2) FK_SET_ERR(ctx, FK_ERR_BAD_ARG, "key: missing vk points");
    if ((d->n_h && !d->h) || (d->n_l && !d->l) || (d->n_a && !d->a) || (d->n_b && (!d->b_g1 || !d->b_g2)))
        FK_SET_ERR(ctx, FK_ERR_BAD_ARG, "key: missing key array");
    fk_key *k = new fk_key();
    k->m = d->m; k->num_input = d->num_input; k->num_aux = d->num_aux;
    k->n_h = d->n_h; k->n_l = d->n_l; k->n_a = d->n_a; k->n_b = d->n_b;
    k->shard_index = d->shard_index; k->shard_count = d->shard_count;
    k->alpha_g1 = g1_from_raw(d->alpha_g1); k->beta_g1 = g1_from_raw(d->beta_g1); k->delta_g1 = g1_from_raw(d->delta_g1);
    k->beta_g2 = g2_from_raw(d->beta_g2); k->delta_g2 = g2_from_raw(d->delta_g2);
    int rc = key_alloc_slices(ctx, k, d->z_frac_lo, d->z_frac_hi);
    auto up = [&](void *dst, const uint8_t *src, uint64_t lo, uint64_t hi, size_t w) -> int {
        if (hi > lo) FK_HIP(ctx, hipMemcpy(dst, src + lo * w, (hi - lo) * w, hipMemcpyHostToDevice));
        return FK_OK;
    };
    if (rc == FK_OK) rc = up(k->d_h, d->h, k->h_lo, k->h_hi, 64);
    if (rc == FK_OK) rc = up(k->d_l, d->l, k->l_lo, k->l_hi, 64);
    if (rc == FK_OK) rc = up(k->d_a, d->a, k->a_lo, k->a_hi, 64);
    if (rc == FK_OK) rc = up(k->d_b1, d->b_g1, k->b_lo, k->b_hi, 64);
    if (rc == FK_OK) rc = up(k->d_b2, d->b_g2, k->b2_lo, k->b2_hi, 128);
    if (rc == FK_OK) rc = key_precompute(ctx, k);
    if (rc != FK_OK) { fk_key_free(ctx, k); return rc; }
    *out = k;
    return FK_OK;
}); }

int fk_key_host_vk(const uint8_t *alpha_g1, const uint8_t *beta_g1, const uint8_t *delta_g1, const uint8_t *beta_g2,
                   const uint8_t *delta_g2, fk_key **out) {
    if (!alpha_g1 || !beta_g1 || !delta_g1 || !beta_g2 || !delta_g2 || !out) return FK_ERR_BAD_ARG;
    fk_key *k = new fk_key();
    k->alpha_g1 = g1_from_raw(alpha_g1); k->beta_g1 = g1_from_raw(beta_g1); k->delta_g1 = g1_from_raw(delta_g1);
    k->beta_g2 = g2_from_raw(beta_g2); k->delta_g2 = g2_from_raw(delta_g2);
    *out = k;
    return FK_OK;
}

int fk_key_precomputed(const fk_key *k, uint32_t out[5]) {
    if (!k || !out) return FK_ERR_BAD_ARG;
    const KeyPre *p[5] = {&k->pre_h, &k->pre_l, &k->pre_a, &k->pre_b1, &k->pre_b2};
    for (int i = 0; i < 5; i++) out[i] = p[i]->lev ? p[i]->W : 0;
    return FK_OK;
}

int fk_key_levels_plan(const fk_key *k, double out[15]) {
    if (!k || !out) return FK_ERR_BAD_ARG;
    const KeyPre *p[5] = {&k->pre_h, &k->pre_l, &k->pre_a, &k->pre_b1, &k->pre_b2};
    const uint64_t n[5] = {k->h_hi - k->h_lo, k->l_hi - k->l_lo, k->a_hi - k->a_lo, k->b_hi - k->b_lo, k->b2_hi - k->b2_lo};
    for (int i = 0; i < 5; i++) {
        const double pt = i == 4 ? 128.0 : 64.0, work = (i == 4 ? (double)FK_G2_WORK : 1.0) * (double)n[i];
        if (p[i]->lev) { out[3 * i] = p[i]->W; out[3 * i + 1] = (double)(p[i]->W - 1) * (double)n[i] * pt / 1073741824.0; out[3 * i + 2] = work * 4.6e-8; }
        else { out[3 * i] = 0; out[3 * i + 1] = n[i] + n[i] / 2 >= (1ull << 21) ? -11.0 * (double)n[i] * pt / 1073741824.0 : 0.0; out[3 * i + 2] = 0; }
    }
    return FK_OK;
}

int fk_key_derive_levels(fk_ctx *ctx, fk_key *k) { return fk_guard(ctx, [&]() -> int {
    if (!ctx || !k) return FK_ERR_BAD_ARG;
    FK_HIP(ctx, hipSetDevice(ctx->device));
    FK_HIP(ctx, hipStreamSynchronize(ctx->stream));
    FK_TRY(msm_sync(ctx));
    const auto t0 = std::chrono::steady_clock::now();
    FK_TRY(key_precompute(ctx, k));
    k->load_s[1] = std::chrono::duration<double>(std::chrono::steady_clock::now() - t0).count();
    return FK_OK;
}); }

int fk_key_drop_levels(fk_ctx *ctx, fk_key *k) { return fk_guard(ctx, [&]() -> int {
    if (!ctx || !k) return FK_ERR_BAD_ARG;
    FK_HIP(ctx, hipSetDevice(ctx->device));
    FK_HIP(ctx, hipStreamSynchronize(ctx->stream));
    FK_TRY(msm_sync(ctx));
    key_pre_free(k);
    return FK_OK;
}); }

int fk_key_levels_headroom(fk_ctx *ctx, const fk_key *k, int64_t *bytes) { return fk_guard(ctx, [&]() -> int {
    if (!ctx || !k || !bytes) return FK_ERR_BAD_ARG;
    FK_HIP(ctx, hipSetDevice(ctx->device));
    return key_levels_headroom(ctx, k, bytes);
}); }

int fk_key_load_profile(const fk_key *k, double out[2]) {
    if (!k || !out) return FK_ERR_BAD_ARG;
    out[0] = k->load_s[0]; out[1] = k->load_s[1];
    return FK_OK;
}

int fk_key_shard_info(const fk_key *k, uint64_t out[8]) {
    if (!k || !out) return FK_ERR_BAD_ARG;
    const uint64_t v[8] = {k->h_lo, k->h_hi, k->l_lo, k->l_hi, k->a_lo, k->a_hi, k->b_lo, k->b_hi};
    memcpy(out, v, sizeof v);
    return FK_OK;
}

int fk_key_shard_info2(const fk_key *k, uint64_t out[10]) {
    if (!k || !out) return FK_ERR_BAD_ARG;
    const uint64_t v[10] = {k->h_lo, k->h_hi, k->l_lo, k->l_hi, k->a_lo, k->a_hi, k->b_lo, k->b_hi, k->b2_lo, k->b2_hi};
    memcpy(out, v, sizeof v);
    return FK_OK;
}

int fk_key_synthetic(fk_ctx *ctx, uint64_t m, uint32_t num_input, uint32_t num_aux, uint64_t n_a, uint64_t n_b,
                     uint64_t seed, uint32_t shard_index, uint32_t shard_count, double z_frac_lo, double z_frac_hi, fk_key **out) { return fk_guard(ctx, [&]() -> int {
    if (!ctx || !out) return FK_ERR_BAD_ARG;
    *out = nullptr;
    FK_HIP(ctx, hipSetDevice(ctx->device));
    FK_TRY(key_check_shape(ctx, m, num_input, m - 1, num_aux, num_aux, shard_index, shard_count));
    fk_key *k = new fk_key();
    k->m = m; k->num_input = num_input; k->num_aux = num_aux;
    k->n_h = m - 1; k->n_l = num_aux; k->n_a = n_a; k->n_b = n_b;
    k->shard_index = shard_index; k->shard_count = shard_count;
    int rc = key_alloc_slices(ctx, k, z_frac_lo, z_frac_hi);
    const uint64_t sd = seed * 1000003ull + shard_index * 7919ull;
    if (rc == FK_OK) rc = gen_points_g1(ctx, k->d_h, k->h_hi - k->h_lo, sd + 1);
    if (rc == FK_OK) rc = gen_points_g1(ctx, k->d_l, k->l_hi - k->l_lo, sd + 2);
    if (rc == FK_OK) rc = gen_points_g1(ctx, k->d_a, k->a_hi - k->a_lo, sd + 3);
    if (rc == FK_OK) rc = gen_points_g1(ctx, k->d_b1, k->b_hi - k->b_lo, sd + 4);
    if (rc == FK_OK) rc = gen_points_g2(ctx, k->d_b2, k->b2_hi - k->b2_lo, sd + 5);
    if (rc == FK_OK) {
        FK_HIP(ctx, ctx->misc.reserve(8 * 128));
        G1Affine *t1 = ctx->misc.as<G1Affine>();
        rc = gen_points_g1(ctx, t1, 3, seed + 99);
        G1Affine h1[3];
        if (rc == FK_OK) { if (hipMemcpy(h1, t1, sizeof h1, hipMemcpyDeviceToHost) != hipSuccess) rc = FK_ERR_HIP; }
        G2Affine *t2 = ctx->misc.as<G2Affine>();
        if (rc == FK_OK) rc = gen_points_g2(ctx, t2, 2, seed + 98);
        G2Affine h2[2];
        if (rc == FK_OK) { if (hipMemcpy(h2, t2, sizeof h2, hipMemcpyDeviceToHost) != hipSuccess) rc = FK_ERR_HIP; }
        k->alpha_g1 = h1[0]; k->beta_g1 = h1[1]; k->delta_g1 = h1[2]; k->beta_g2 = h2[0]; k->delta_g2 = h2[1];
    }
    if (rc == FK_OK) { if (hipStreamSynchronize(ctx->stream) != hipSuccess) rc = FK_ERR_HIP; }
    if (rc == FK_OK) rc = key_precompute(ctx, k);
    if (rc != FK_OK) { fk_key_free(ctx, k); return rc; }
    *out = k;
    return FK_OK;
}); }

static bool sorts_first(const fk_key *key) {
    static int t = -2;
    if (t == -2) { const char *e = getenv("FK_PROVE_SORTS_FIRST"); t = e ? atoi(e) : -1; }
    return t >= 0 ? t != 0 : key->h_hi - key->h_lo >= (1ull << 25) - 1;
}

static void lanes_choose(fk_ctx *ctx, const fk_key *key) { ctx->lanes_in_use = sorts_first(key) ? MSM_LANES : 3; }

static int witness_begin(fk_ctx *ctx, const fk_key *key, const Fr *d_z, const WitnessQueries &q, hipEvent_t z_ready, FrontOpts opt = {}) {
    if (!key || !d_z) FK_SET_ERR(ctx, FK_ERR_BAD_ARG, "prove: null argument");
    if (ctx->wit_active) FK_SET_ERR(ctx, FK_ERR_BAD_ARG, "prove: witness multiplications already in flight");
    bool any_tail = false;
    for (int i = 0; i < MSM_TAILS; i++) any_tail = any_tail || ctx->tails[i].active;
    if (!any_tail) ctx->lane_next = 0;
    lanes_choose(ctx, key);
    FK_HIP(ctx, hipSetDevice(ctx->device));
    const uint32_t v_in = key->num_input, v_aux = key->num_aux;
    for (int i = 0; i < 4; i++) ctx->wit_tail[i] = -1;
    auto body = [&]() -> int {
        hipStream_t ax = opt.gather_on_main ? ctx->stream : ctx->aux;
        if (z_ready && !opt.gather_on_main) FK_HIP(ctx, hipStreamWaitEvent(ax, z_ready, 0));
        FK_HIP(ctx, ctx->sc_b.reserve(((size_t)v_in + v_aux) * sizeof(Fr)));
        FK_HIP(ctx, ctx->sc_a.reserve(((size_t)v_in + v_aux) * sizeof(Fr)));
        Fr *sb = ctx->sc_b.as<Fr>(), *sa = ctx->sc_a.as<Fr>();
        if (const QueryIdx *qi = q.idx) {
            if (qi->n_b != key->n_b) FK_SET_ERR(ctx, FK_ERR_KEY_MISMATCH, "prove: b query needs %llu points, key holds %llu",
                                                (unsigned long long)qi->n_b, (unsigned long long)key->n_b);
            if (qi->n_a != key->n_a) FK_SET_ERR(ctx, FK_ERR_KEY_MISMATCH, "prove: a query needs %llu points, key holds %llu",
                                                (unsigned long long)qi->n_a, (unsigned long long)key->n_a);
            FK_TRY(gather_scalars(ctx, d_z, qi->b + key->b_lo, key->b_hi - key->b_lo, sb + key->b_lo, ax));
            if (key->b2_lo != key->b_lo || key->b2_hi != key->b_hi) {
                const uint64_t lo = key->b2_lo, hi = key->b2_hi;
                const uint64_t c_lo = std::max(lo, key->b_lo), c_hi = std::min(hi, key->b_hi);
                if (c_lo >= c_hi) FK_TRY(gather_scalars(ctx, d_z, qi->b + lo, hi - lo, sb + lo, ax));
                else {
                    if (lo < c_lo) FK_TRY(gather_scalars(ctx, d_z, qi->b + lo, c_lo - lo, sb + lo, ax));
                    if (c_hi < hi) FK_TRY(gather_scalars(ctx, d_z, qi->b + c_hi, hi - c_hi, sb + c_hi, ax));
                }
            }
            FK_TRY(gather_scalars(ctx, d_z, qi->a + key->a_lo, key->a_hi - key->a_lo, sa + key->a_lo, ax));
        } else {
            uint64_t n_b_in = 0, n_b_aux = 0, n_a_aux = 0;
            FK_TRY(compact_scalars(ctx, d_z, q.d_b_in, v_in, sb, &n_b_in, ax));
            FK_TRY(compact_scalars(ctx, d_z + v_in, q.d_b_aux, v_aux, sb + n_b_in, &n_b_aux, ax));
            if (n_b_in + n_b_aux != key->n_b) FK_SET_ERR(ctx, FK_ERR_KEY_MISMATCH, "prove: b query needs %llu points, key holds %llu",
                                                         (unsigned long long)(n_b_in + n_b_aux), (unsigned long long)key->n_b);
            FK_HIP(ctx, hipMemcpyAsync(sa, d_z, (size_t)v_in * sizeof(Fr), hipMemcpyDeviceToDevice, ax));
            FK_TRY(compact_scalars(ctx, d_z + v_in, q.d_a_aux, v_aux, sa + v_in, &n_a_aux, ax));
            if (v_in + n_a_aux != key->n_a) FK_SET_ERR(ctx, FK_ERR_KEY_MISMATCH, "prove: a query needs %llu points, key holds %llu",
                                                       (unsigned long long)(v_in + n_a_aux), (unsigned long long)key->n_a);
        }
        FK_HIP(ctx, hipEventRecord(ctx->ev_aux, ax));
        FK_TRY(msm_g1_begin(ctx, key->d_b1, sb + key->b_lo, key->b_hi - key->b_lo, &ctx->wit_tail[0], ctx->ev_aux, &key->pre_b1, opt.defer_back));
        FK_TRY(msm_g2_begin(ctx, key->d_b2, sb + key->b2_lo, key->b2_hi - key->b2_lo, key->b2_lo == key->b_lo && key->b2_hi == key->b_hi,
                            &ctx->wit_tail[1], ctx->ev_aux, &key->pre_b2, opt.defer_back));
        FK_TRY(msm_g1_begin(ctx, key->d_l, d_z + v_in + key->l_lo, key->l_hi - key->l_lo, &ctx->wit_tail[2], z_ready ? z_ready : ctx->ev_aux, &key->pre_l, opt.defer_back));
        FK_TRY(msm_g1_begin(ctx, key->d_a, sa + key->a_lo, key->a_hi - key->a_lo, &ctx->wit_tail[3], ctx->ev_aux, &key->pre_a, opt.defer_back));
        return FK_OK;
    };
    const int rc = body();
    if (rc != FK_OK) { msm_abandon(ctx); return rc; }
    ctx->wit_active = true;
    return FK_OK;
}

extern "C++" {
namespace fk {
int early_witness_begin(fk_ctx *ctx, const fk_key *key, const void *d_z, const WitnessQueries &q, int tails_out[4]) {
    if (!early_front_applies(key)) return 0;
    const int rc = witness_begin(ctx, key, (const Fr *)d_z, q, ctx->ev_z, FrontOpts{true, true});
    if (rc != FK_OK) return -rc;
    memcpy(tails_out, ctx->wit_tail, 4 * sizeof(int));
    return 1;
}
bool early_front_applies(const fk_key *key) {
    static const int t_wfirst = tune("FK_PROVE_WITNESS_FIRST", 1), t_accgate = tune("FK_PROVE_ACC_AFTER_NTT", 1), t_early = tune("FK_PROVE_EARLY_FRONT", 1);
    return t_early && t_wfirst && t_accgate && key && sorts_first(key);
}
}
}

static int witness_end(fk_ctx *ctx, uint8_t out[FK_MSM_RESULT_BYTES], int tail_h = -1, const int *tails = nullptr) {
    if (!tails) {
        if (!ctx->wit_active) { msm_abandon(ctx); FK_SET_ERR(ctx, FK_ERR_BAD_ARG, "prove: no witness multiplications in flight"); }
        ctx->wit_active = false;
        tails = ctx->wit_tail;
    }
    const int tw[4] = {tails[0], tails[1], tails[2], tails[3]};
    G1Xyzz H = G1Xyzz::inf(), L, A, B1; G2Xyzz B2;
    auto body = [&]() -> int {
        FK_TRY(msm_g1_end(ctx, tw[0], &B1));
        FK_TRY(msm_g2_end(ctx, tw[1], &B2));
        FK_TRY(msm_g1_end(ctx, tw[2], &L));
        FK_TRY(msm_g1_end(ctx, tw[3], &A));
        if (tail_h >= 0) FK_TRY(msm_g1_end(ctx, tail_h, &H));
        return FK_OK;
    };
    const int rc = body();
    if (rc != FK_OK) { msm_abandon(ctx); return rc; }
    g1_to_raw(out, H); g1_to_raw(out + 64, L); g1_to_raw(out + 128, A); g1_to_raw(out + 192, B1); g2_to_raw(out + 256, B2);
    return FK_OK;
}

static int prove_msms_z(fk_ctx *ctx, const fk_key *key, const Fr *d_z, const WitnessQueries &q, uint8_t out[FK_MSM_RESULT_BYTES], fk_timings *tm) {
    if (!out) FK_SET_ERR(ctx, FK_ERR_BAD_ARG, "prove: null argument");
    const double t0 = now_ms();
    FK_HIP(ctx, hipSetDevice(ctx->device));
    FK_HIP(ctx, hipEventRecord(ctx->ev_main, ctx->stream));
    FK_TRY(witness_begin(ctx, key, d_z, q, ctx->ev_main));
    FK_TRY(witness_end(ctx, out));
    if (tm) tm->msm_l_ms = now_ms() - t0;
    return FK_OK;
}

static int prove_msms_run(fk_ctx *ctx, const fk_key *key, Fr *d_a, Fr *d_b, Fr *d_c, uint64_t n, const Fr *d_z, const ProveRun &run,
                          uint8_t out[FK_MSM_RESULT_BYTES], fk_timings *tm) {
    if (!key || !d_a || !d_b || !d_c || !d_z || !out) FK_SET_ERR(ctx, FK_ERR_BAD_ARG, "prove: null argument");
    if (n == 0 || n > key->m || (key->m > 1 && n <= key->m / 2)) FK_SET_ERR(ctx, FK_ERR_KEY_MISMATCH, "prove: %llu rows do not match key domain %llu",
                                                      (unsigned long long)n, (unsigned long long)key->m);
    FK_HIP(ctx, hipSetDevice(ctx->device));
    FK_RANGE("prove: queue front, quotient, accumulations; wait for the results");
    const double t0 = now_ms();
    FK_HIP(ctx, ctx->hbuf.reserve(key->m * sizeof(Fr)));
    Fr *d_h = ctx->hbuf.as<Fr>();
    uint64_t m = 0;
    const bool early = ctx->early.done && ctx->early.key == key && ctx->early.d_z == (const void *)d_z;
    if (ctx->early.done && !early) { msm_abandon(ctx); FK_SET_ERR(ctx, FK_ERR_BAD_ARG, "prove: an early front of another proof is outstanding"); }
    ctx->early.done = false;
    if (!early) ctx->lane_next = 0;
    lanes_choose(ctx, key);
    static const int t_wfirst = tune("FK_PROVE_WITNESS_FIRST", 1);
    const bool wfirst = t_wfirst != 0;
    if (!run.z_recorded) FK_HIP(ctx, hipEventRecord(ctx->ev_z, ctx->stream));
    const bool gate = wfirst && sorts_first(key);
    static const int t_accgate = tune("FK_PROVE_ACC_AFTER_NTT", 1);
    if (early && !gate) { msm_abandon(ctx); FK_SET_ERR(ctx, FK_ERR_BAD_ARG, "prove: early front without the sorts-first schedule"); }
    if (gate) {
        if (early) {
            memcpy(ctx->wit_tail, ctx->early.tails, sizeof ctx->wit_tail);
            ctx->wit_active = true;
        } else {
            const int rcw = witness_begin(ctx, key, d_z, run.q, ctx->ev_z, FrontOpts{t_accgate != 0});
            if (rcw != FK_OK) { msm_abandon(ctx); return rcw; }
        }
        for (MsmLane &ln : ctx->lanes)
            if (ln.ev_sorted_valid) { FK_HIP(ctx, hipStreamWaitEvent(ctx->stream, ln.ev_sorted, 0)); ln.ev_sorted_valid = false; }
    }
    { const int rcu = upload_deferred(ctx, true); if (rcu != FK_OK) { if (gate) msm_abandon(ctx); return rcu; } }
    int rcq;
    { FK_RANGE("prove: queue quotient (6 transforms)"); rcq = quotient_dev(ctx, d_a, d_b, d_c, n, d_h, &m); }
    if (rcq != FK_OK) { if (gate) msm_abandon(ctx); return rcq; }
    const double t1 = now_ms();
    if (wfirst) {
        FK_HIP(ctx, hipEventRecord(ctx->ev_main, ctx->stream));
        if (gate) { const int rcd = msm_run_deferred(ctx, ctx->ev_main); if (rcd != FK_OK) { msm_abandon(ctx); return rcd; } }
        if (!gate) {
            const int rcw = witness_begin(ctx, key, d_z, run.q, ctx->ev_z);
            if (rcw != FK_OK) { msm_abandon(ctx); return rcw; }
        }
        int t_h0 = -1;
        const int rch = msm_g1_begin(ctx, key->d_h, d_h + key->h_lo, key->h_hi - key->h_lo, &t_h0, ctx->ev_main, &key->pre_h);
        if (rch != FK_OK) { msm_abandon(ctx); return rch; }
        const double t2w = now_ms();
        if (gate && run.before_block) {
            int mine[4];
            memcpy(mine, ctx->wit_tail, sizeof mine);
            ctx->wit_active = false;
            int rce;
            { FK_RANGE("prove: queue the NEXT proof's early front"); rce = (*run.before_block)(); }
            if (rce != FK_OK) { msm_abandon(ctx); return rce; }
            { FK_RANGE("prove: wait for the five multiplications"); FK_TRY(witness_end(ctx, out, t_h0, mine)); }
        } else { FK_RANGE("prove: wait for the five multiplications"); FK_TRY(witness_end(ctx, out, t_h0)); }
        if (tm) { tm->ntt_ms = t1 - t0; tm->msm_l_ms = t2w - t1; tm->msm_h_ms = now_ms() - t2w; tm->total_ms = now_ms() - t0; }
        return FK_OK;
    }
    FK_HIP(ctx, hipEventRecord(ctx->ev_main, ctx->stream));
    int t_h = -1;
    FK_TRY(msm_g1_begin(ctx, key->d_h, d_h + key->h_lo, key->h_hi - key->h_lo, &t_h, ctx->ev_main, &key->pre_h));
    const int rc = witness_begin(ctx, key, d_z, run.q, ctx->ev_main);
    if (rc != FK_OK) { msm_abandon(ctx); return rc; }
    const double t2 = now_ms();
    FK_TRY(witness_end(ctx, out, t_h));
    if (tm) { tm->ntt_ms = t1 - t0; tm->msm_l_ms = t2 - t1; tm->msm_h_ms = now_ms() - t2; tm->total_ms = now_ms() - t0; }
    return FK_OK;
}

extern "C++" {
namespace fk {
int prove_msms_dev(fk_ctx *ctx, const fk_key *key, Fr *d_a, Fr *d_b, Fr *d_c, uint64_t n, const Fr *d_z, const ProveRun &run,
                   uint8_t out[FK_MSM_RESULT_BYTES], fk_timings *tm) {
    return fk_guard(ctx, [&]() -> int { return prove_msms_run(ctx, key, d_a, d_b, d_c, n, d_z, run, out, tm); });
}

int prove_dev(fk_ctx *ctx, const fk_key *key, Fr *d_a, Fr *d_b, Fr *d_c, uint64_t n, const Fr *d_z, const ProveRun &run, const uint64_t r[4],
              const uint64_t s[4], uint8_t out[FK_PROOF_BYTES], fk_timings *tm) {
    if (key && key->shard_count != 1) FK_SET_ERR(ctx, FK_ERR_BAD_ARG, "fk_prove needs an unsharded key (use fk_prove_msms + fk_prove_assemble)");
    if (tm) memset(tm, 0, sizeof *tm);
    uint8_t msms[FK_MSM_RESULT_BYTES];
    FK_TRY(prove_msms_dev(ctx, key, d_a, d_b, d_c, n, d_z, run, msms, tm));
    const double t0 = now_ms();
    FK_TRY(fk_prove_assemble(ctx, key, msms, 1, r, s, out));
    if (tm) { tm->assemble_ms = now_ms() - t0; tm->total_ms += tm->assemble_ms; }
    return FK_OK;
}

int witness_queries_begin(fk_ctx *ctx, const fk_key *key, const void *d_z, const WitnessQueries &q) {
    FK_HIP(ctx, hipSetDevice(ctx->device));
    FK_HIP(ctx, hipEventRecord(ctx->ev_main, ctx->stream));
    return witness_begin(ctx, key, (const Fr *)d_z, q, ctx->ev_main);
}

int witness_queries_finish(fk_ctx *ctx, const fk_key *key, const void *d_h_slice, uint8_t out[FK_MSM_RESULT_BYTES]) {
    if (!key || !out || (!d_h_slice && key->h_hi > key->h_lo)) { msm_abandon(ctx); FK_SET_ERR(ctx, FK_ERR_BAD_ARG, "prove: null argument"); }
    FK_HIP(ctx, hipSetDevice(ctx->device));
    int t_h = -1;
    const int rc = msm_g1_begin(ctx, key->d_h, (const Fr *)d_h_slice, key->h_hi - key->h_lo, &t_h, nullptr, &key->pre_h);
    if (rc != FK_OK) { msm_abandon(ctx); return rc; }
    return witness_end(ctx, out, t_h);
}
}
}

int fk_prove_msms_z_dev(fk_ctx *ctx, const fk_key *key, const void *d_z, const void *d_a_aux, const void *d_b_in,
                        const void *d_b_aux, uint8_t out[FK_MSM_RESULT_BYTES], fk_timings *tm) { return fk_guard(ctx, [&]() -> int {
    if (!ctx) return FK_ERR_BAD_ARG;
    if (tm) memset(tm, 0, sizeof *tm);
    return prove_msms_z(ctx, key, (const Fr *)d_z, {(const uint8_t *)d_a_aux, (const uint8_t *)d_b_in, (const uint8_t *)d_b_aux}, out, tm);
}); }

int fk_prove_msm_h_dev(fk_ctx *ctx, const fk_key *key, const void *d_h_slice, uint8_t out[FK_G1_BYTES]) { return fk_guard(ctx, [&]() -> int {
    if (!ctx) return FK_ERR_BAD_ARG;
    if (!key || !out || (!d_h_slice && key->h_hi > key->h_lo)) FK_SET_ERR(ctx, FK_ERR_BAD_ARG, "prove: null argument");
    FK_TRY(scratch_claim(ctx, "msm over the h array"));
    G1Xyzz H;
    FK_TRY(msm_g1_dev(ctx, key->d_h, (const Fr *)d_h_slice, key->h_hi - key->h_lo, &H, &key->pre_h));
    g1_to_raw(out, H);
    return FK_OK;
}); }

int fk_prove_msm_array_dev(fk_ctx *ctx, const fk_key *key, int which, const void *d_scalars, uint8_t *out) { return fk_guard(ctx, [&]() -> int {
    if (!ctx) return FK_ERR_BAD_ARG;
    if (!key || !out || which < FK_ARRAY_H || which > FK_ARRAY_B_G2) FK_SET_ERR(ctx, FK_ERR_BAD_ARG, "msm over a key array: null argument or unknown array");
    FK_TRY(scratch_claim(ctx, "msm over a key array"));
    const uint64_t n = which == FK_ARRAY_H ? key->h_hi - key->h_lo : which == FK_ARRAY_L ? key->l_hi - key->l_lo
                     : which == FK_ARRAY_A ? key->a_hi - key->a_lo : which == FK_ARRAY_B_G1 ? key->b_hi - key->b_lo : key->b2_hi - key->b2_lo;
    if (!d_scalars && n) FK_SET_ERR(ctx, FK_ERR_BAD_ARG, "msm over a key array: null scalars");
    if (which == FK_ARRAY_B_G2) {
        G2Xyzz R;
        FK_TRY(msm_g2_dev(ctx, key->d_b2, (const Fr *)d_scalars, n, &R, false, &key->pre_b2));
        g2_to_raw(out, R);
        return FK_OK;
    }
    const G1Affine *bases = which == FK_ARRAY_H ? key->d_h : which == FK_ARRAY_L ? key->d_l : which == FK_ARRAY_A ? key->d_a : key->d_b1;
    const KeyPre *pre = which == FK_ARRAY_H ? &key->pre_h : which == FK_ARRAY_L ? &key->pre_l : which == FK_ARRAY_A ? &key->pre_a : &key->pre_b1;
    G1Xyzz R;
    FK_TRY(msm_g1_dev(ctx, bases, (const Fr *)d_scalars, n, &R, pre));
    g1_to_raw(out, R);
    return FK_OK;
}); }

int fk_prove_msms_z_begin_dev(fk_ctx *ctx, const fk_key *key, const void *d_z, const void *d_a_aux, const void *d_b_in, const void *d_b_aux) { return fk_guard(ctx, [&]() -> int {
    if (!ctx) return FK_ERR_BAD_ARG;
    return witness_queries_begin(ctx, key, d_z, {(const uint8_t *)d_a_aux, (const uint8_t *)d_b_in, (const uint8_t *)d_b_aux});
}); }

int fk_prove_msms_finish_dev(fk_ctx *ctx, const fk_key *key, const void *d_h_slice, uint8_t out[FK_MSM_RESULT_BYTES]) { return fk_guard(ctx, [&]() -> int {
    if (!ctx) return FK_ERR_BAD_ARG;
    return witness_queries_finish(ctx, key, d_h_slice, out);
}); }

int fk_prove_msms_hz_dev(fk_ctx *ctx, const fk_key *key, const void *d_h_slice, const void *d_z, const void *d_a_aux, const void *d_b_in,
                         const void *d_b_aux, uint8_t out[FK_MSM_RESULT_BYTES], fk_timings *tm) { return fk_guard(ctx, [&]() -> int {
    if (!ctx) return FK_ERR_BAD_ARG;
    if (tm) memset(tm, 0, sizeof *tm);
    FK_TRY(witness_queries_begin(ctx, key, d_z, {(const uint8_t *)d_a_aux, (const uint8_t *)d_b_in, (const uint8_t *)d_b_aux}));
    return witness_queries_finish(ctx, key, d_h_slice, out);
}); }

int fk_prove_msms_dev(fk_ctx *ctx, const fk_key *key, void *d_a, void *d_b, void *d_c, uint64_t n, const void *d_z,
                      const void *d_a_aux, const void *d_b_in, const void *d_b_aux, uint8_t out[FK_MSM_RESULT_BYTES], fk_timings *tm) { return fk_guard(ctx, [&]() -> int {
    if (!ctx) return FK_ERR_BAD_ARG;
    if (tm) memset(tm, 0, sizeof *tm);
    return prove_msms_dev(ctx, key, (Fr *)d_a, (Fr *)d_b, (Fr *)d_c, n, (const Fr *)d_z,
                          ProveRun{{(const uint8_t *)d_a_aux, (const uint8_t *)d_b_in, (const uint8_t *)d_b_aux}}, out, tm);
}); }

int fk_prove_assemble(fk_ctx *ctx, const fk_key *key, const uint8_t *parts, uint32_t n_parts, const uint64_t r_[4],
                      const uint64_t s_[4], uint8_t out[FK_PROOF_BYTES]) { return fk_guard(ctx, [&]() -> int {
    fk_ctx local;
    if (!ctx) ctx = &local;
    if (!key || !parts || !n_parts || !r_ || !s_ || !out) FK_SET_ERR(ctx, FK_ERR_BAD_ARG, "assemble: null argument");
    if (key->delta_g1.is_inf() || key->delta_g2.is_inf()) FK_SET_ERR(ctx, FK_ERR_UNEXPECTED_IDENTITY, "delta is the identity");
    G1Xyzz H = G1Xyzz::inf(), L = G1Xyzz::inf(), A = G1Xyzz::inf(), B1 = G1Xyzz::inf();
    G2Xyzz B2 = G2Xyzz::inf();
    for (uint32_t i = 0; i < n_parts; i++) {
        const uint8_t *p = parts + (size_t)i * FK_MSM_RESULT_BYTES;
        H.add_mixed(g1_from_raw(p)); L.add_mixed(g1_from_raw(p + 64)); A.add_mixed(g1_from_raw(p + 128));
        B1.add_mixed(g1_from_raw(p + 192)); B2.add_mixed(g2_from_raw(p + 256));
    }
    Fr rm, sm; memcpy(&rm, r_, 32); memcpy(&sm, s_, 32);
    const Fr rc = Fr::from_mont(rm), sc = Fr::from_mont(sm), rsc = Fr::from_mont(Fr::mul(rm, sm));
    const G1Xyzz d1 = G1Xyzz::from_affine(key->delta_g1), a1 = G1Xyzz::from_affine(key->alpha_g1), b1 = G1Xyzz::from_affine(key->beta_g1);
    const G2Xyzz d2 = G2Xyzz::from_affine(key->delta_g2);
    G1Xyzz gA = G1Xyzz::mul_scalar(d1, rc.v); gA.add_mixed(key->alpha_g1); gA.add(A);
    G2Xyzz gB = G2Xyzz::mul_scalar(d2, sc.v); gB.add_mixed(key->beta_g2); gB.add(B2);
    G1Xyzz gC = G1Xyzz::mul_scalar(d1, rsc.v);
    gC.add(G1Xyzz::mul_scalar(a1, sc.v));
    gC.add(G1Xyzz::mul_scalar(b1, rc.v));
    gC.add(G1Xyzz::mul_scalar(A, sc.v));
    gC.add(G1Xyzz::mul_scalar(B1, rc.v));
    gC.add(H); gC.add(L);
    const G1Affine pa = gA.to_affine(), pc = gC.to_affine();
    const G2Affine pb = gB.to_affine();
    const Fq words[8] = {Fq::from_mont(pa.x), Fq::from_mont(pa.y), Fq::from_mont(pb.x.c0), Fq::from_mont(pb.x.c1),
                         Fq::from_mont(pb.y.c0), Fq::from_mont(pb.y.c1), Fq::from_mont(pc.x), Fq::from_mont(pc.y)};
    memcpy(out, words, 256);
    return FK_OK;
}); }
// ... 315 lines not shown
```

### fawkes-crypto_amd/csrc/spmv.hip

```cpp
#include "common.hpp"
#include <string.h>
#include <algorithm>
#include <atomic>
#include <chrono>
#include <thread>
#include <unordered_map>
#include <string>

#include "r1cs.hpp"
#include "../../include/fawkes_hip_inspect.h"

namespace fk {

struct SpmvArgs {
    const uint64_t *ptr[3];
    const uint32_t *col[3];
    const uint32_t *cidx[3];
    Fr *out[3];
};

struct TileDims { uint32_t base_gates, base_input, base_aux; };
template <bool TILED, bool SLICED>
__global__ __launch_bounds__(256) void spmv_kernel(SpmvArgs a, const Fr *table, const Fr *z, uint64_t num_gates, uint32_t num_input, uint32_t lg0, uint32_t lg1,
                                                   uint32_t lg2, TileDims td, uint32_t binned, uint32_t log_w, uint32_t rank) {
// ... 389 lines not shown
            std::vector<uint64_t> hs(R * 3), ln(R * 3, 0);
            for (uint64_t g = g0 > dd_back ? g0 - dd_back : 0; g < g1; g++) {
                const size_t slot = (size_t)(g % R) * 3;
                for (int k = 0; k < 3; k++) {
                    const uint64_t lo = ptrs[k][g], len = ptrs[k][g + 1] - lo;
                    ln[slot + k] = 0;
                    if (len < dd_min) continue;
                    uint64_t h = len;
                    for (uint64_t i = 0; i < len; i++) h = (h ^ (cols[k][lo + i] | (uint64_t)h_cidx[k][lo + i] << 32)) * 0x9e3779b97f4a7c15ull + (h >> 31);
                    hs[slot + k] = h; ln[slot + k] = len;
                    if (g < g0) continue;
                    auto same = [&](uint64_t g2, int k2) {
                        const size_t s2 = (size_t)(g2 % R) * 3 + k2;
                        if (ln[s2] != len || hs[s2] != h) return false;
                        const uint64_t lo2 = ptrs[k2][g2];
                        return memcmp(cols[k2] + lo2, cols[k] + lo, len * 4) == 0 && memcmp(h_cidx[k2] + lo2, h_cidx[k] + lo, len * 4) == 0;
                    };
                    uint64_t prev = NONE;
                    for (int k2 = k - 1; k2 >= 0 && prev == NONE; k2--) if (same(g, k2)) prev = g * 3 + k2;
                    for (uint64_t d = 1; d <= dd_back && d <= g && prev == NONE; d++)
                        for (int k2 = 2; k2 >= 0 && prev == NONE; k2--) if (same(g - d, k2)) prev = (g - d) * 3 + k2;
                    if (prev != NONE) found.push_back({g * 3 + k, prev});
                }
            }
        };
        const uint32_t n_thr = ng >= ((uint64_t)1 << 20) ? std::min(16u, std::max(1u, host_threads())) : 1u;
        std::vector<std::vector<Cand>> found(n_thr);
        std::vector<uint64_t> alias;
        std::vector<uint8_t> is_alias[3];
        try {
            std::atomic<bool> threw{false};
            auto guarded = [&](uint32_t t) { try { scan(ng * t / n_thr, ng * (t + 1) / n_thr, found[t]); } catch (...) { threw = true; } };
            {
                std::vector<std::thread> pool;
                for (uint32_t t = 1; t < n_thr; t++) { try { pool.emplace_back(guarded, t); } catch (...) { guarded(t); } }
                guarded(0);
                for (auto &th : pool) th.join();
            }
            if (threw) throw std::bad_alloc();
            struct Seen { uint64_t key, prev; bool alias; };
            const uint64_t RS = 3 * ((uint64_t)dd_back + 1);
            std::vector<Seen> ring(RS, Seen{NONE, NONE, false});
            for (uint32_t t = 0; t < n_thr; t++) {
                for (const Cand &c : found[t]) {
                    const uint64_t g = c.key / 3; const uint32_t dm = (uint32_t)(c.key % 3);
                    Seen &me = ring[c.key % RS];
                    me = Seen{c.key, c.prev, false};
                    if (!((r->bins.mask >> dm) & 1)) continue;
                    uint64_t best = NONE;
                    for (uint64_t cur = c.prev; cur != NONE && g - cur / 3 <= dd_back;) {
                        const Seen &e = ring[cur % RS];
                        const bool known = e.key == cur;
                        if (!known || !e.alias) best = cur;
                        cur = known ? e.prev : NONE;
                    }
                    if (best == NONE) continue;
                    me.alias = true;
                    const uint64_t sg = best / 3, sm = best % 3;
                    if (is_alias[dm].empty()) is_alias[dm].assign(ng, 0);
                    is_alias[dm][g] = 1;
                    alias.push_back(g | (g - sg) << 32 | (uint64_t)dm << 48 | sm << 50);
                    r->alias_terms += ptrs[dm][g + 1] - ptrs[dm][g];
                }
                std::vector<Cand>().swap(found[t]);
            }
        } catch (...) { ctx->err = "r1cs: out of host memory while looking for repeated rows"; return fail(FK_ERR_OOM); }
        if (!alias.empty()) {
            BinArgs &d = r->bins_dd;
            d.mask = r->bins.mask;
            std::vector<uint32_t> dd[3];
            for (uint32_t s = 0; s < r->bins.nseg; s++) {
                const uint32_t k = r->bins.mtx[s], nr = r->bins.n_rows[s];
                const uint32_t *src = r->h_rowlist[k].data() + r->bins.list_off[s];
                uint32_t off = r->bins.list_off[s], kept = nr;
                const uint32_t *lo = src;
                if (!is_alias[k].empty()) {
                    off = (uint32_t)dd[k].size();
                    for (uint32_t i = 0; i < nr; i++) if (!is_alias[k][src[i]]) dd[k].push_back(src[i]);
                    kept = (uint32_t)dd[k].size() - off;
                }
                if (!kept) continue;
                const uint32_t sd = d.nseg++;
                const uint64_t per = 256u >> r->bins.lg[s];
                d.lg[sd] = r->bins.lg[s]; d.mtx[sd] = k; d.n_rows[sd] = kept; d.list_off[sd] = off;
                d.first_block[sd + 1] = d.first_block[sd] + (uint32_t)((kept + per - 1) / per);
                if (!is_alias[k].empty()) lo = dd[k].data() + off;
                for (uint32_t j = 0; j <= r->win_k && r->win_k; j++) {
                    const uint64_t bound = r->win_row[j];
                    r->win_cnt_dd[j][sd] = (uint32_t)(std::partition_point(lo, lo + kept, [&](uint32_t row) { return row < bound; }) - lo);
                }
            }
            for (uint32_t j = 0; j <= r->win_k && r->win_k; j++) {
                const uint64_t bound = r->win_row[j];
                r->win_alias[j] = (uint64_t)(std::partition_point(alias.begin(), alias.end(), [&](uint64_t e) { return (e & 0xffffffffull) < bound; }) - alias.begin());
            }
            for (int k = 0; k < 3; k++) {
                d.rowlist[k] = r->rowlist[k];
                if (is_alias[k].empty()) continue;
                if (hipMalloc((void **)&r->rowlist_dd[k], dd[k].size() * 4 + 4) != hipSuccess) { ctx->err = "r1cs: device allocation failed"; return fail(FK_ERR_OOM); }
                if (!dd[k].empty() && hipMemcpy(r->rowlist_dd[k], dd[k].data(), dd[k].size() * 4, hipMemcpyHostToDevice) != hipSuccess) { ctx->err = "r1cs: upload failed"; return fail(FK_ERR_HIP); }
                d.rowlist[k] = r->rowlist_dd[k];
            }
            if (hipMalloc((void **)&r->d_alias, alias.size() * 8) != hipSuccess) { ctx->err = "r1cs: device allocation failed"; return fail(FK_ERR_OOM); }
            if (hipMemcpy(r->d_alias, alias.data(), alias.size() * 8, hipMemcpyHostToDevice) != hipSuccess) { ctx->err = "r1cs: upload failed"; return fail(FK_ERR_HIP); }
            r->n_alias = alias.size();
        }
        if (getenv("FK_GATES_TRACE")) fprintf(stderr, "[fk] r1cs load: %.2f s so far, alias plan done (%llu aliases for %llu terms)\n", std::chrono::duration<double>(std::chrono::steady_clock::now() - t_load0).count(),
                                              (unsigned long long)r->n_alias, (unsigned long long)r->alias_terms);
    }
    if (copies > 1 && wave_copies && copies >= wave_copies && r->bins.mask && cs->num_gates < ((uint64_t)1 << 30)) {
        std::vector<uint32_t> wl;
        for (uint64_t g = 0; g < cs->num_gates; g++)
            for (uint32_t k = 0; k < 3; k++) {
                const uint64_t l = ptrs[k][g + 1] - ptrs[k][g];
                if (((r->bins.mask >> k) & 1) && l >= wave_lo && l < wave_hi) wl.push_back(k << 30 | (uint32_t)g);
            }
        if (!wl.empty() && (uint64_t)((copies + 63) / 64) * wl.size() < 0xfffffff0ull) {
            if (hipMalloc((void **)&r->d_wavelist, wl.size() * 4) != hipSuccess) { ctx->err = "r1cs: device allocation failed"; return fail(FK_ERR_OOM); }
            if (hipMemcpy(r->d_wavelist, wl.data(), wl.size() * 4, hipMemcpyHostToDevice) != hipSuccess) { ctx->err = "r1cs: upload failed"; return fail(FK_ERR_HIP); }
            r->n_wavelist = (uint32_t)wl.size();
        }
    }
    if (copies > 1) {
        auto rep = [&](std::vector<uint8_t> &f, size_t skip, size_t per) {
            std::vector<uint8_t> o(skip + per * copies + (skip + per * copies == 0));
            for (size_t i = 0; i < skip; i++) o[i] = f[i];
            for (uint32_t j = 0; j < copies; j++) for (size_t i = 0; i < per; i++) o[skip + j * per + i] = f[skip + i];
            f.swap(o);
        };
        rep(a_aux, 0, cs->num_aux); rep(b_aux, 0, cs->num_aux); rep(b_in, 1, cs->num_input - 1);
    }
    r->n_table = table.size();
    if (hipMalloc((void **)&r->table, table.size() * sizeof(Fr)) != hipSuccess || hipMalloc((void **)&r->d_a_aux, a_aux.size()) != hipSuccess ||
        hipMalloc((void **)&r->d_b_in, b_in.size()) != hipSuccess || hipMalloc((void **)&r->d_b_aux, b_aux.size()) != hipSuccess) {
        ctx->err = "r1cs: device allocation failed"; return fail(FK_ERR_OOM);
    }
    if (hipMemcpy(r->table, table.data(), table.size() * sizeof(Fr), hipMemcpyHostToDevice) != hipSuccess ||
        hipMemcpy(r->d_a_aux, a_aux.data(), a_aux.size(), hipMemcpyHostToDevice) != hipSuccess ||
        hipMemcpy(r->d_b_in, b_in.data(), b_in.size(), hipMemcpyHostToDevice) != hipSuccess ||
        hipMemcpy(r->d_b_aux, b_aux.data(), b_aux.size(), hipMemcpyHostToDevice) != hipSuccess) { ctx->err = "r1cs: upload failed"; return fail(FK_ERR_HIP); }
    for (uint32_t j = 0; j < r->num_aux; j++) { r->n_a_aux += a_aux[j]; r->n_b_aux += b_aux[j]; }
    for (uint32_t i = 0; i < r->num_input; i++) r->n_b_in += b_in[i];
    {
        std::vector<uint32_t> ia, ib;
        ia.reserve(r->num_input + r->n_a_aux); ib.reserve(r->n_b_in + r->n_b_aux);
        for (uint32_t i = 0; i < r->num_input; i++) { ia.push_back(i); if (b_in[i]) ib.push_back(i); }
        for (uint32_t j = 0; j < r->num_aux; j++) { if (a_aux[j]) ia.push_back(r->num_input + j); if (b_aux[j]) ib.push_back(r->num_input + j); }
        if (hipMalloc((void **)&r->d_idx_a, ia.size() * 4 + 4) != hipSuccess || hipMalloc((void **)&r->d_idx_b, ib.size() * 4 + 4) != hipSuccess) {
            ctx->err = "r1cs: device allocation failed"; return fail(FK_ERR_OOM);
        }
        if ((ia.size() && hipMemcpy(r->d_idx_a, ia.data(), ia.size() * 4, hipMemcpyHostToDevice) != hipSuccess) ||
            (ib.size() && hipMemcpy(r->d_idx_b, ib.data(), ib.size() * 4, hipMemcpyHostToDevice) != hipSuccess)) { ctx->err = "r1cs: upload failed"; return fail(FK_ERR_HIP); }
        r->qidx.a = r->d_idx_a; r->qidx.b = r->d_idx_b; r->qidx.n_a = ia.size(); r->qidx.n_b = ib.size();
    }
    *out = r;
    return FK_OK;
}

int fk_r1cs_load(fk_ctx *ctx, const fk_r1cs *cs, fk_r1cs_dev **out) { return fk_guard(ctx, [&]() -> int { return r1cs_load_impl(ctx, cs, 1, out); }); }
}
namespace fk {
int r1cs_load_coded(fk_ctx *ctx, uint32_t num_input, uint32_t num_aux, uint64_t num_gates, const uint64_t *const ptr[3], const uint32_t *const col[3],
                    const uint32_t *const cidx[3], const Fr *table, uint64_t n_table, fk_r1cs_dev **out, const uint8_t *const density[3]) {
    fk_r1cs cs{};
    cs.num_input = num_input; cs.num_aux = num_aux; cs.num_gates = num_gates;
    cs.a_ptr = ptr[0]; cs.a_col = col[0]; cs.b_ptr = ptr[1]; cs.b_col = col[1]; cs.c_ptr = ptr[2]; cs.c_col = col[2];
    return r1cs_load_impl(ctx, &cs, 1, out, cidx, table, n_table, density);
}
}
extern "C" {
int fk_r1cs_load_tiled(fk_ctx *ctx, const fk_r1cs *instance, uint32_t copies, fk_r1cs_dev **out) { return fk_guard(ctx, [&]() -> int { return r1cs_load_impl(ctx, instance, copies, out); }); }

int fk_r1cs_load_coded(fk_ctx *ctx, const fk_r1cs *cs, const uint32_t *a_cidx, const uint32_t *b_cidx, const uint32_t *c_cidx, const uint64_t *table,
                       uint64_t n_table, fk_r1cs_dev **out) { return fk_guard(ctx, [&]() -> int {
    if (!ctx) return FK_ERR_BAD_ARG;
    if (!cs || !table || !n_table || !out) FK_SET_ERR(ctx, FK_ERR_BAD_ARG, "r1cs: null argument");
    const uint32_t *cidx[3] = {a_cidx, b_cidx, c_cidx};
    const uint64_t *ptrs[3] = {cs->a_ptr, cs->b_ptr, cs->c_ptr};
    for (int k = 0; k < 3; k++) if (ptrs[k] && ptrs[k][cs->num_gates] && !cidx[k]) FK_SET_ERR(ctx, FK_ERR_BAD_ARG, "r1cs: null coefficient index array");
    return r1cs_load_impl(ctx, cs, 1, out, cidx, (const Fr *)table, n_table);
}); }

int fk_r1cs_density_ptrs(const fk_r1cs_dev *r, const void *out[3]) {
    if (!r || !out) return FK_ERR_BAD_ARG;
    out[0] = r->d_a_aux; out[1] = r->d_b_in; out[2] = r->d_b_aux;
    return FK_OK;
}

int fk_r1cs_info(const fk_r1cs_dev *r, uint64_t out[8]) {
    if (!r || !out) return FK_ERR_BAD_ARG;
    const uint64_t v[8] = {r->num_gates + r->num_input, r->nnz[0], r->nnz[1], r->nnz[2], r->n_table,
                           (uint64_t)r->num_input + r->n_a_aux, r->n_b_in + r->n_b_aux, (uint64_t)r->num_input + r->num_aux};
    memcpy(out, v, sizeof v);
    return FK_OK;
}

int fk_r1cs_alias_info(const fk_r1cs_dev *r, uint64_t out[4]) {
    if (!r || !out) return FK_ERR_BAD_ARG;
    out[0] = r->n_alias; out[1] = r->n_alias ? r->alias_terms : 0; out[2] = r->alias_min; out[3] = r->alias_lookback;
    return FK_OK;
}

int fk_r1cs_aliases(const fk_r1cs_dev *r, uint64_t cap, uint32_t *dst_mtx, uint32_t *dst_row, uint32_t *src_mtx, uint32_t *src_row) {
    if (!r || !dst_mtx || !dst_row || !src_mtx || !src_row || cap < r->n_alias) return FK_ERR_BAD_ARG;
    if (!r->n_alias) return FK_OK;
    try {
        std::vector<uint64_t> h(r->n_alias);
        if (hipMemcpy(h.data(), r->d_alias, h.size() * 8, hipMemcpyDeviceToHost) != hipSuccess) return FK_ERR_HIP;
        for (uint64_t i = 0; i < h.size(); i++) {
            const uint64_t e = h[i];
            dst_row[i] = (uint32_t)e; src_row[i] = (uint32_t)e - ((uint32_t)(e >> 32) & 0xffffu);
            dst_mtx[i] = (uint32_t)(e >> 48) & 3u; src_mtx[i] = (uint32_t)(e >> 50) & 3u;
        }
    } catch (...) { return FK_ERR_OOM; }
    return FK_OK;
}

int fk_r1cs_windows(const fk_r1cs_dev *r, uint32_t *n_windows, uint64_t rows[17], uint64_t need[16]) {
    if (!r || !n_windows) return FK_ERR_BAD_ARG;
    *n_windows = r->win_k;
    for (uint32_t j = 0; j <= r->win_k && rows; j++) rows[j] = r->win_row[j];
    for (uint32_t j = 0; j < r->win_k && need; j++) need[j] = r->win_need[j];
    return FK_OK;
}

}
namespace fk {
static int slice_lists(fk_ctx *ctx, const fk_r1cs_dev *r, uint32_t log_w, const SliceLists **out) {
    std::lock_guard<std::mutex> lock(r->slice_mu);
    SliceLists &sl = r->slices[log_w];
    if (!sl.built) {
        const uint32_t W = 1u << log_w;
        for (int k = 0; k < 3; k++) {
            if (!((r->bins.mask >> k) & 1)) continue;
            const std::vector<uint32_t> &src = r->h_rowlist[k];
            std::vector<uint32_t> dst(src.size());
            for (uint32_t s = 0; s < r->bins.nseg; s++) {
                if (r->bins.mtx[s] != (uint32_t)k) continue;
                const uint32_t off = r->bins.list_off[s], nr = r->bins.n_rows[s];
                uint32_t c[8] = {0};
                for (uint32_t i = 0; i < nr; i++) c[src[off + i] & (W - 1)]++;
                uint32_t pos[8], acc = 0;
                for (uint32_t q = 0; q < W; q++) { sl.cnt[s][q] = c[q]; sl.offs[s][q] = acc; pos[q] = acc; acc += c[q]; }
                for (uint32_t i = 0; i < nr; i++) { const uint32_t row = src[off + i]; dst[off + pos[row & (W - 1)]++] = row; }
            }
            FK_HIP(ctx, hipMalloc((void **)&sl.d_list[k], dst.size() * 4 + 4));
            if (!dst.empty()) FK_HIP(ctx, hipMemcpy(sl.d_list[k], dst.data(), dst.size() * 4, hipMemcpyHostToDevice));
        }
        sl.built = true;
    }
    *out = &sl;
    return FK_OK;
}

int r1cs_eval_impl(fk_ctx *ctx, const fk_r1cs_dev *r, const void *d_z, void *d_a, void *d_b, void *d_c, bool sliced, uint32_t rank, uint32_t log_w, uint64_t n_out, int window = -1) {
    FK_HIP(ctx, hipSetDevice(ctx->device));
    SpmvArgs a;
    for (int k = 0; k < 3; k++) { a.ptr[k] = r->ptr[k]; a.col[k] = r->col[k]; a.cidx[k] = r->cidx[k]; }
    a.out[0] = (Fr *)d_a; a.out[1] = (Fr *)d_b; a.out[2] = (Fr *)d_c;
    const uint64_t rows = r->num_gates + r->num_input;
    const uint64_t W = (uint64_t)1 << log_w;
    const uint64_t my_rows = sliced ? (rows > rank ? (rows - rank + W - 1) / W : 0) : rows;
    if (sliced) {
        if (my_rows > n_out) FK_SET_ERR(ctx, FK_ERR_BAD_ARG, "r1cs eval: the slice holds %llu rows, the arrays %llu", (unsigned long long)my_rows, (unsigned long long)n_out);
        if (n_out > my_rows) for (int k = 0; k < 3; k++) FK_HIP(ctx, hipMemsetAsync(a.out[k] + my_rows, 0, (n_out - my_rows) * sizeof(Fr), ctx->stream));
    }
    uint32_t lg[3], lgmax = 0;
    static const int t_div = std::max(1, tune("FK_SPMV_TERMS_PER_LANE", 2));
    for (int k = 0; k < 3; k++) {
        const uint64_t mean = r->num_gates ? r->nnz[k] / r->num_gates : 0;
        lg[k] = 0;
        while (!((r->bins.mask >> k) & 1) && lg[k] < 6 && ((uint64_t)t_div << lg[k]) <= mean) lg[k]++;
        if (lg[k] > lgmax) lgmax = lg[k];
    }
    const uint64_t lanes = my_rows << lgmax;
    const TileDims td{r->base_gates, r->base_input, r->base_aux};
    const uint32_t binned = r->bins.mask;
    const dim3 grid((unsigned)((lanes + 255) / 256), 3), block(256);
    const bool tiled = r->copies > 1;
    if (lanes && window <= 0) {
#define FK_SPMV_LAUNCH(T_, S_) hipLaunchKernelGGL(HIP_KERNEL_NAME(spmv_kernel<T_, S_>), grid, block, 0, ctx->stream, a, r->table, (const Fr *)d_z, r->num_gates, \
                                                  r->num_input, lg[0], lg[1], lg[2], td, binned, log_w, rank)
        if (tiled) { if (sliced) FK_SPMV_LAUNCH(true, true); else FK_SPMV_LAUNCH(true, false); }
        else { if (sliced) FK_SPMV_LAUNCH(false, true); else FK_SPMV_LAUNCH(false, false); }
#undef FK_SPMV_LAUNCH
    }
    const bool dedup = r->n_alias && !tiled && !sliced && spmv_dedup_on();
    if (binned) {
        BinArgs b = dedup ? r->bins_dd : r->bins;
        SliceArgs sa;
        if (sliced) {
            const SliceLists *sl = nullptr;
            FK_TRY(slice_lists(ctx, r, log_w, &sl));
            sa.log_w = log_w; sa.rank = rank;
            const uint32_t g = (uint32_t)(r->base_gates & (W - 1));
            uint32_t P = 1;
            while ((uint32_t)((uint64_t)P * g) & (W - 1)) P++;
            sa.P = P;
            for (uint32_t p_ = 0; p_ < P; p_++) sa.rho[p_] = (uint32_t)((rank + W * P - ((uint64_t)p_ * g & (W - 1))) & (W - 1));
            b.first_block[0] = 0;
            for (uint32_t s = 0; s < b.nseg; s++) {
                memcpy(sa.cnt[s], sl->cnt[s], sizeof sa.cnt[s]); memcpy(sa.offs[s], sl->offs[s], sizeof sa.offs[s]);
                uint64_t T = 0, part = 0;
                const uint32_t tail = r->copies % P;
                for (uint32_t p_ = 0; p_ < P; p_++) { T += sa.cnt[s][sa.rho[p_]]; if (p_ < tail) part += sa.cnt[s][sa.rho[p_]]; }
                sa.T[s] = (uint32_t)T;
// ... 42 lines not shown
    FK_HIP(ctx, hipGetLastError());
    FK_DBG(ctx, "spmv");
    return FK_OK;
}
}
extern "C" {

int fk_r1cs_eval_dev(fk_ctx *ctx, const fk_r1cs_dev *r, const void *d_z, void *d_a, void *d_b, void *d_c) { return fk_guard(ctx, [&]() -> int {
    if (!ctx) return FK_ERR_BAD_ARG;
    if (!r || !d_z || !d_a || !d_b || !d_c) FK_SET_ERR(ctx, FK_ERR_BAD_ARG, "r1cs eval: null argument");
    return r1cs_eval_impl(ctx, r, d_z, d_a, d_b, d_c, false, 0, 0, 0);
}); }

int fk_r1cs_eval_slice_dev(fk_ctx *ctx, const fk_r1cs_dev *r, const void *d_z, uint32_t log_m, uint32_t rank, uint32_t log_w, void *d_a, void *d_b, void *d_c) { return fk_guard(ctx, [&]() -> int {
    if (!ctx) return FK_ERR_BAD_ARG;
    if (!r || !d_z || !d_a || !d_b || !d_c) FK_SET_ERR(ctx, FK_ERR_BAD_ARG, "r1cs eval: null argument");
    if (log_w > 3 || (rank >> log_w) || log_m < log_w || log_m >= FK_FR_S) FK_SET_ERR(ctx, FK_ERR_BAD_ARG, "r1cs eval: bad slice (rank %u of 2^%u, domain 2^%u)", rank, log_w, log_m);
    if (r->num_gates + r->num_input > ((uint64_t)1 << log_m)) FK_SET_ERR(ctx, FK_ERR_BAD_ARG, "r1cs eval: the system has more rows than the domain 2^%u", log_m);
    return r1cs_eval_impl(ctx, r, d_z, d_a, d_b, d_c, true, rank, log_w, (uint64_t)1 << (log_m - log_w));
}); }

}
namespace fk {
int prove_r1cs_dev_impl(fk_ctx *ctx, const fk_key *key, const fk_r1cs_dev *r, const void *d_z, const uint64_t rr[4], const uint64_t ss[4],
                        uint8_t out_proof[FK_PROOF_BYTES], fk_timings *tm, const std::function<int()> *after_eval, const std::function<int()> *before_block) {
    if (!key || !r || !d_z) FK_SET_ERR(ctx, FK_ERR_BAD_ARG, "prove: null argument");
    uint64_t rows = 0;
    FK_TRY(r1cs_fits_key(ctx, r, key, &rows));
    FK_HIP(ctx, hipSetDevice(ctx->device));
    const size_t mb = key->m * sizeof(Fr);
    if (after_eval && ctx->early.done) { msm_abandon(ctx); FK_SET_ERR(ctx, FK_ERR_BAD_ARG, "prove: an early front of a submitted proof is outstanding"); }
    ProveRun run{r1cs_queries(r), false, before_block};
    if (ctx->early.done && ctx->early.key == key && ctx->early.r1cs == r && ctx->early.d_z == d_z) {
        run.z_recorded = true;
    } else {
        if (ctx->early.done) { msm_abandon(ctx); FK_SET_ERR(ctx, FK_ERR_BAD_ARG, "prove: an early front of another proof is outstanding"); }
        FK_HIP(ctx, ctx->stage_a.reserve(mb)); FK_HIP(ctx, ctx->stage_b.reserve(mb)); FK_HIP(ctx, ctx->stage_c.reserve(mb));
        static const int t_zearly = tune("FK_PROVE_Z_EARLY", 1);
        if (t_zearly) {
            FK_HIP(ctx, hipEventRecord(ctx->ev_z, ctx->stream));
            run.z_recorded = true;
        }
        FK_TRY(fk_r1cs_eval_dev(ctx, r, d_z, ctx->stage_a.p, ctx->stage_b.p, ctx->stage_c.p));
        if (after_eval) FK_TRY((*after_eval)());
    }
    return prove_dev(ctx, key, ctx->stage_a.as<Fr>(), ctx->stage_b.as<Fr>(), ctx->stage_c.as<Fr>(), rows, (const Fr *)d_z, run, rr, ss, out_proof, tm);
}
}
extern "C" {

int fk_prove_r1cs_dev(fk_ctx *ctx, const fk_key *key, const fk_r1cs_dev *r, const void *d_z, const uint64_t rr[4], const uint64_t ss[4],
                      uint8_t out_proof[FK_PROOF_BYTES], fk_timings *tm) { return fk_guard(ctx, [&]() -> int {
    FK_RANGE("fk_prove_r1cs_dev");
    if (!ctx) return FK_ERR_BAD_ARG;
    return prove_r1cs_dev_impl(ctx, key, r, d_z, rr, ss, out_proof, tm, nullptr, nullptr);
}); }

int fk_prove_msms_hz_r1cs_dev(fk_ctx *ctx, const fk_key *key, const fk_r1cs_dev *r, const void *d_h_slice, const void *d_z,
                              uint8_t out[FK_MSM_RESULT_BYTES]) { return fk_guard(ctx, [&]() -> int {
    if (!ctx) return FK_ERR_BAD_ARG;
    if (!key || !r || !d_z) FK_SET_ERR(ctx, FK_ERR_BAD_ARG, "prove: null argument");
    FK_TRY(r1cs_fits_key(ctx, r, key, nullptr));
    FK_TRY(witness_queries_begin(ctx, key, d_z, r1cs_queries(r)));
    return witness_queries_finish(ctx, key, d_h_slice, out);
}); }

int fk_prove_msms_z_begin_r1cs_dev(fk_ctx *ctx, const fk_key *key, const fk_r1cs_dev *r, const void *d_z) { return fk_guard(ctx, [&]() -> int {
    if (!ctx) return FK_ERR_BAD_ARG;
    if (!key || !r || !d_z) FK_SET_ERR(ctx, FK_ERR_BAD_ARG, "prove: null argument");
    FK_TRY(r1cs_fits_key(ctx, r, key, nullptr));
    return witness_queries_begin(ctx, key, d_z, r1cs_queries(r));
}); }

}
namespace fk {
static int prove_r1cs_chunked(fk_ctx *ctx, const fk_key *key, const fk_r1cs_dev *r, uint64_t rows, const uint64_t *z, const uint64_t rr[4], const uint64_t ss[4],
                              uint8_t out_proof[FK_PROOF_BYTES], fk_timings *tm) {
    const size_t mb = key->m * sizeof(Fr);
    FK_HIP(ctx, ctx->stage_a.reserve(mb)); FK_HIP(ctx, ctx->stage_b.reserve(mb)); FK_HIP(ctx, ctx->stage_c.reserve(mb));
    FK_HIP(ctx, hipEventRecord(ctx->ev_upload_gate, ctx->stream));
    FK_HIP(ctx, hipStreamWaitEvent(ctx->copy_st, ctx->ev_upload_gate, 0));
    Fr *d_z = ctx->stage_z.as<Fr>();
    uint64_t off = 0;
    ProveRun run{r1cs_queries(r)};
    int rc = FK_OK;
    for (uint32_t j = 0; j < r->win_k && rc == FK_OK; j++) {
        const uint64_t end = r->win_need[j];
        hipError_t e = hipSuccess;
        if (end > off) e = hipMemcpyAsync(d_z + off, z + 4 * off, (end - off) * sizeof(Fr), hipMemcpyHostToDevice, ctx->copy_st);
        if (e == hipSuccess && !ctx->ev_chunk[j]) e = hipEventCreateWithFlags(&ctx->ev_chunk[j], hipEventDisableTiming);
        if (e == hipSuccess) e = hipEventRecord(ctx->ev_chunk[j], ctx->copy_st);
        if (e == hipSuccess) e = hipStreamWaitEvent(ctx->stream, ctx->ev_chunk[j], 0);
        off = std::max(off, end);
        if (e == hipSuccess && j + 1 == r->win_k) {
            e = hipEventRecord(ctx->ev_z, ctx->stream);
            run.z_recorded = e == hipSuccess;
        }
        if (e != hipSuccess) { rc = FK_ERR_HIP; ctx->err = std::string("prove: chunked hand-over: ") + hipGetErrorString(e); break; }
        rc = r1cs_eval_impl(ctx, r, d_z, ctx->stage_a.p, ctx->stage_b.p, ctx->stage_c.p, false, 0, 0, 0, (int)j);
    }
    if (rc == FK_OK) return prove_dev(ctx, key, ctx->stage_a.as<Fr>(), ctx->stage_b.as<Fr>(), ctx->stage_c.as<Fr>(), rows, d_z, run, rr, ss, out_proof, tm);
    (void)hipStreamSynchronize(ctx->copy_st); (void)hipStreamSynchronize(ctx->stream);
    return rc;
}
}
extern "C" {

int fk_prove_r1cs(fk_ctx *ctx, const fk_key *key, const fk_r1cs_dev *r, const uint64_t *z, const uint64_t rr[4], const uint64_t ss[4],
                  uint8_t out_proof[FK_PROOF_BYTES], fk_timings *tm) { return fk_guard(ctx, [&]() -> int {
    FK_RANGE("fk_prove_r1cs");
    if (!ctx) return FK_ERR_BAD_ARG;
    if (!key || !r || !z) FK_SET_ERR(ctx, FK_ERR_BAD_ARG, "prove: null argument");
    FK_HIP(ctx, hipSetDevice(ctx->device));
    const size_t zb = ((size_t)r->num_input + r->num_aux) * sizeof(Fr);
    FK_HIP(ctx, ctx->stage_z.reserve(zb));
    static const bool t_chunked = !(getenv("FK_PROVE_CHUNKED_UPLOAD") && atoi(getenv("FK_PROVE_CHUNKED_UPLOAD")) == 0);
    if (t_chunked && r->win_k >= 2 && !ctx->early.done && !ctx->wslot[0].pending && !ctx->wslot[1].pending) {
        uint64_t rows = 0;
        FK_TRY(r1cs_fits_key(ctx, r, key, &rows));
        return prove_r1cs_chunked(ctx, key, r, rows, z, rr, ss, out_proof, tm);
    }
    FK_HIP(ctx, hipMemcpyAsync(ctx->stage_z.p, z, zb, hipMemcpyHostToDevice, ctx->stream));
    return fk_prove_r1cs_dev(ctx, key, r, ctx->stage_z.p, rr, ss, out_proof, tm);
}); }

int fk_prove_r1cs_submit(fk_ctx *ctx, const fk_key *key, const fk_r1cs_dev *r, const uint64_t *z, const uint64_t rr[4], const uint64_t ss[4], int *ticket) { return fk_guard(ctx, [&]() -> int {
    if (!ctx) return FK_ERR_BAD_ARG;
    if (!key || !r || !z || !rr || !ss || !ticket) FK_SET_ERR(ctx, FK_ERR_BAD_ARG, "prove: null argument");
    const int slot = ctx->wslot_next;
    if (ctx->wslot[slot].pending) FK_SET_ERR(ctx, FK_ERR_BAD_ARG, "prove: two proofs are already submitted (call fk_prove_r1cs_wait first)");
    fk_ctx::WitSlot &w = ctx->wslot[slot];
    const size_t zb = ((size_t)r->num_input + r->num_aux) * sizeof(Fr);
    static const int t_defer = tune("FK_UPLOAD_DEFER", 1);
    if (t_defer && ctx->wslot[slot ^ 1].pending && zb <= w.buf.cap && w.ready) { w.deferred = true; w.host_z = z; w.host_bytes = zb; }
    else { w.deferred = false; FK_TRY(fk_witness_upload_async(ctx, slot, z, zb)); }
    w.pending = true; w.key = key; w.r1cs = r;
    memcpy(w.r, rr, 32); memcpy(w.s, ss, 32);
    ctx->wslot_next = slot ^ 1;
    *ticket = slot;
    return FK_OK;
}); }
}
namespace fk {
static int early_front(fk_ctx *ctx, int slot) {
    fk_ctx::WitSlot &w = ctx->wslot[slot];
    const fk_key *key = w.key; const fk_r1cs_dev *r = w.r1cs;
    if (w.deferred) { w.deferred = false; FK_TRY(fk_witness_upload_async(ctx, slot, w.host_z, w.host_bytes)); }
    void *d_z = nullptr;
    FK_TRY(fk_witness_ptr(ctx, slot, &d_z));
    if (ctx->ev_acc_done_valid) FK_HIP(ctx, hipStreamWaitEvent(ctx->stream, ctx->ev_acc_done, 0));
    const size_t mb = key->m * sizeof(Fr);
    if (mb > ctx->stage_a.cap || mb > ctx->stage_b.cap || mb > ctx->stage_c.cap) return FK_OK;
    FK_HIP(ctx, hipEventRecord(ctx->ev_z, ctx->stream));
    int tails[4];
    const int wb = early_witness_begin(ctx, key, d_z, r1cs_queries(r), tails);
    if (wb < 0) return -wb;
    if (wb == 0) return FK_OK;
    FK_TRY(fk_r1cs_eval_dev(ctx, r, d_z, ctx->stage_a.p, ctx->stage_b.p, ctx->stage_c.p));
    ctx->early.done = true; ctx->early.key = key; ctx->early.r1cs = r; ctx->early.d_z = d_z;
    memcpy(ctx->early.tails, tails, sizeof tails);
    return FK_OK;
}
}
extern "C" {
int fk_prove_r1cs_wait(fk_ctx *ctx, int ticket, uint8_t out_proof[FK_PROOF_BYTES], fk_timings *tm) { return fk_guard(ctx, [&]() -> int {
    FK_RANGE("fk_prove_r1cs_wait");
    if (!ctx) return FK_ERR_BAD_ARG;
    if (ticket < 0 || ticket > 1 || !ctx->wslot[ticket].pending) FK_SET_ERR(ctx, FK_ERR_BAD_ARG, "prove: no submitted proof with ticket %d", ticket);
    fk_ctx::WitSlot &w = ctx->wslot[ticket];
    w.pending = false;
    if (w.deferred) { w.deferred = false; FK_TRY(fk_witness_upload_async(ctx, ticket, w.host_z, w.host_bytes)); }
    void *d_z = nullptr;
    const bool early = ctx->early.done && ctx->early.key == w.key && ctx->early.r1cs == w.r1cs && ctx->early.d_z == ctx->wslot[ticket].buf.p;
    if (early) d_z = ctx->wslot[ticket].buf.p;
    else FK_TRY(fk_witness_ptr(ctx, ticket, &d_z));
    const fk_ctx::WitSlot &o = ctx->wslot[ticket ^ 1];
    const std::function<int()> front = [ctx, ticket]() { return early_front(ctx, ticket ^ 1); };
    const bool next = o.pending && o.key == w.key && o.r1cs == w.r1cs && early_front_applies(w.key);
    return prove_r1cs_dev_impl(ctx, w.key, w.r1cs, d_z, w.r, w.s, out_proof, tm, nullptr, next ? &front : nullptr);
}); }

}
```

### include/fawkes_hip_inspect.h

```cpp
#ifndef FAWKES_HIP_INSPECT_H
#define FAWKES_HIP_INSPECT_H
#include "fawkes_hip.h"
#ifdef __cplusplus
extern "C" {
#endif

int fk_r1cs_alias_info(const fk_r1cs_dev *r1cs, uint64_t out[4]);
int fk_r1cs_aliases(const fk_r1cs_dev *r1cs, uint64_t cap, uint32_t *dst_mtx, uint32_t *dst_row, uint32_t *src_mtx, uint32_t *src_row);

#ifdef __cplusplus
}
#endif
#endif
```

Baseline: 4.458.

## Share L-query sort with padded A-query MSM when A indices match aux witness

When the A-query's aux indices match the L-query's witness range (checked via a fingerprint of the A index array), the A bases are scattered into a padded base array aligned to L. The A MSM then adopts the L lane's digit sort and bucket ordering instead of re-gathering scalars and re-sorting. The input portion of A becomes a small separate uncounted MSM that is added back at the end. This removes a full gather, radix sort and size-order pass for the A MSM. In exchange it keeps an extra padded base array with precomputed levels in device memory, and adds lane-lending events and bookkeeping.

```diff
diff --git a/fawkes-crypto_amd/csrc/common.hpp b/fawkes-crypto_amd/csrc/common.hpp
--- a/fawkes-crypto_amd/csrc/common.hpp
+++ b/fawkes-crypto_amd/csrc/common.hpp
@@ -4,6 +4,7 @@
 #include <stdio.h>
 #include <stdlib.h>
 #include <map>
+#include <mutex>
 #include <string>
 #include <new>
 #include <stdexcept>
@@ -54,6 +55,9 @@
     DevBuf digits, sorted, totals, starts, perm, overlist, tasktab, partials, s2_cnt1, s2_seg, s2_cnt2, s2_tmp_idx, s2_tmp_lo, buckets;
     DevBuf buckets2;
     const void *last_sort_scalars = nullptr; size_t last_sort_n = 0; unsigned last_sort_c = 0; bool last_merged = false;
+    hipEvent_t ev_lent = nullptr;
+    bool lent_valid = false;
+    int lent_pending = 0;
 };
 
 struct MsmTail {
@@ -70,6 +74,8 @@
 struct QueryIdx {
     const uint32_t *a = nullptr, *b = nullptr;
     uint64_t n_a = 0, n_b = 0;
+    uint64_t a_fp = 0;
+    bool a_fp_valid = false;
 };
 
 struct WitnessQueries {
@@ -111,8 +117,8 @@
     std::vector<std::function<int()>> deferred, deferred_tails;
     hipEvent_t ev_acc_done = nullptr; bool ev_acc_done_valid = false;
     bool wit_active = false;
-    struct EarlyFront { bool done = false; int tails[4] = {-1, -1, -1, -1}; const fk_key *key = nullptr; const struct fk_r1cs_dev *r1cs = nullptr; const void *d_z = nullptr; } early;
-    int wit_tail[4] = {-1, -1, -1, -1};
+    struct EarlyFront { bool done = false; int tails[5] = {-1, -1, -1, -1, -1}; const fk_key *key = nullptr; const struct fk_r1cs_dev *r1cs = nullptr; const void *d_z = nullptr; } early;
+    int wit_tail[5] = {-1, -1, -1, -1, -1};
     hipStream_t copy_st = nullptr;
     struct WitSlot {
         fk::DevBuf buf; hipEvent_t ready = nullptr; bool pending = false;
@@ -142,6 +148,10 @@
     fk::G1Affine alpha_g1, beta_g1, delta_g1;
     fk::G2Affine beta_g2, delta_g2;
     fk::KeyPre pre_h, pre_l, pre_a, pre_b1, pre_b2;
+    struct APad { fk::G1Affine *d = nullptr; fk::KeyPre pre; uint64_t n_a = 0, n_l = 0, fp = 0; bool used = false, refused = false; };
+    static constexpr int A_PADS = 2;
+    mutable APad a_pad[A_PADS];
+    mutable std::mutex a_pad_mu;
     double load_s[2] = {0, 0};
 };
 
@@ -181,6 +191,7 @@
 namespace fk {
 static inline bool proof_holds_staging(const fk_ctx *ctx) { return ctx->early.done; }
 static inline bool proof_holds_lanes(const fk_ctx *ctx) {
+    for (const MsmLane &ln : ctx->lanes) if (ln.lent_pending) return true;
     return proof_holds_staging(ctx) || ctx->wit_active || !ctx->deferred.empty() || !ctx->deferred_tails.empty();
 }
 
@@ -325,10 +336,13 @@
 int dq_cross(fk_ctx *ctx, Fr *d_buf, uint32_t log_m, uint32_t rank, uint32_t log_w, int mode, const Fr *d_sub = nullptr);
 
 int msm_g1_dev(fk_ctx *ctx, const G1Affine *d_bases, const Fr *d_scalars, size_t n, G1Xyzz *out, const KeyPre *pre = nullptr);
-int msm_g1_begin(fk_ctx *ctx, const G1Affine *d_bases, const Fr *d_scalars, size_t n, int *tail, hipEvent_t ready = nullptr, const KeyPre *pre = nullptr, bool defer = false);
+int msm_g1_begin(fk_ctx *ctx, const G1Affine *d_bases, const Fr *d_scalars, size_t n, int *tail, hipEvent_t ready = nullptr, const KeyPre *pre = nullptr, bool defer = false, bool uncounted = false);
+int msm_g1_begin_adopt(fk_ctx *ctx, const G1Affine *d_bases, const Fr *d_scalars, size_t n, int lender, int lane, bool *adopted, int *tail, const KeyPre *pre = nullptr, bool defer = false);
 int msm_g1_end(fk_ctx *ctx, int tail, G1Xyzz *out);
 int msm_g2_begin(fk_ctx *ctx, const G2Affine *d_bases, const Fr *d_scalars, size_t n, bool reuse_sort, int *tail, hipEvent_t ready = nullptr, const KeyPre *pre = nullptr, bool defer = false);
 int key_precompute(fk_ctx *ctx, fk_key *key);
+int key_a_pad(fk_ctx *ctx, const fk_key *key, const QueryIdx *qi, const fk_key::APad **pad);
+int query_fingerprint(fk_ctx *ctx, const uint32_t *d_idx, size_t n, uint64_t *out);
 int key_levels_headroom(fk_ctx *ctx, const fk_key *key, int64_t *bytes);
 void key_pre_free(fk_key *key);
 int msm_g2_end(fk_ctx *ctx, int tail, G2Xyzz *out);
@@ -336,7 +350,7 @@
 int msm_run_deferred(fk_ctx *ctx, hipEvent_t after);
 int upload_deferred(fk_ctx *ctx, bool gate_on_main);
 int witness_slot_reserve(fk_ctx *ctx, int slot, size_t bytes, bool *moved = nullptr);
-int early_witness_begin(fk_ctx *ctx, const fk_key *key, const void *d_z, const WitnessQueries &q, int tails_out[4]);
+int early_witness_begin(fk_ctx *ctx, const fk_key *key, const void *d_z, const WitnessQueries &q, int tails_out[5]);
 bool early_front_applies(const fk_key *key);
 int witness_queries_begin(fk_ctx *ctx, const fk_key *key, const void *d_z, const WitnessQueries &q);
 int witness_queries_finish(fk_ctx *ctx, const fk_key *key, const void *d_h_slice, uint8_t out[FK_MSM_RESULT_BYTES]);
diff --git a/fawkes-crypto_amd/csrc/msm.hip b/fawkes-crypto_amd/csrc/msm.hip
--- a/fawkes-crypto_amd/csrc/msm.hip
+++ b/fawkes-crypto_amd/csrc/msm.hip
@@ -829,6 +829,7 @@
         FK_HIP(ctx, hipStreamCreateWithFlags(&ln.st, hipStreamNonBlocking));
         FK_HIP(ctx, hipEventCreateWithFlags(&ln.ev_in, hipEventDisableTiming));
         FK_HIP(ctx, hipEventCreateWithFlags(&ln.ev_sorted, hipEventDisableTiming));
+        FK_HIP(ctx, hipEventCreateWithFlags(&ln.ev_lent, hipEventDisableTiming));
     }
     for (hipEvent_t *e : {&ctx->ev_main, &ctx->ev_z, &ctx->ev_upload_gate}) if (!*e) FK_HIP(ctx, hipEventCreateWithFlags(e, hipEventDisableTiming));
     return FK_OK;
@@ -839,6 +840,15 @@
     if (*p) { FK_HIP(ctx, hipHostFree(*p)); *p = nullptr; *cap = 0; }
     FK_HIP(ctx, hipHostMalloc(p, bytes + (bytes >> 2) + pad, hipHostMallocDefault));
     *cap = bytes + (bytes >> 2) + pad;
+    return FK_OK;
+}
+
+static int lane_reclaim(fk_ctx *ctx, MsmLane &ln, bool host_wait) {
+    if (ln.lent_pending) FK_SET_ERR(ctx, FK_ERR_BAD_ARG, "msm: this lane's sort is lent to a multiplication whose accumulation has not been queued yet");
+    if (!ln.lent_valid) return FK_OK;
+    if (host_wait) FK_HIP(ctx, hipEventSynchronize(ln.ev_lent));
+    else FK_HIP(ctx, hipStreamWaitEvent(ln.st, ln.ev_lent, 0));
+    ln.lent_valid = false;
     return FK_OK;
 }
 
@@ -853,6 +863,8 @@
     size_t n, WB, max_tasks, max_tiles, wp_bytes;
     uint32_t WR;
     bool merged, have_sort;
+    MsmLane *lender;
+    bool uncounted;
     MsmDyn *dyn;
     uint32_t *digits, *sorted, *totals, *starts, *perm;
     Task *tasks;
@@ -874,6 +886,26 @@
     const uint32_t nseg = p.W * p.nhi;
     const size_t max_tiles = j.max_tiles = (size_t)p.W * ((n + S2_TILE - 1) / S2_TILE) + nseg + 1;
     struct Need { DevBuf *b; size_t bytes; };
+    if (j.lender) {
+        MsmLane &ld = *j.lender;
+        const Need mine[] = {{&ln.buckets2, WB * sizeof(Xyzz<F>)}, {&ln.partials, max_tasks * sizeof(Xyzz<F>)}};
+        bool grow_mine = false;
+        for (const Need &nd : mine) grow_mine = grow_mine || nd.bytes > nd.b->cap;
+        if (grow_mine) {
+            FK_HIP(ctx, hipStreamSynchronize(ln.st));
+            for (const Need &nd : mine) FK_HIP(ctx, nd.b->reserve(nd.bytes));
+        }
+        FK_HIP(ctx, tl.d_wp.reserve(wp_dev_bytes));
+        FK_TRY(pinned_reserve(ctx, &tl.h_wp, &tl.h_cap, j.wp_bytes, 16));
+        j.dyn = (MsmDyn *)((char *)ld.overlist.p + OVER_MAX * sizeof(OverEntry));
+        j.tasks = ld.tasktab.as<Task>();
+        j.obs = (OverBucket *)((char *)ld.tasktab.p + ((max_tasks * sizeof(Task) + 15) & ~(size_t)15));
+        j.digits = nullptr; j.sorted = ld.sorted.as<uint32_t>();
+        j.totals = ld.totals.as<uint32_t>(); j.starts = ld.starts.as<uint32_t>();
+        j.winparts = tl.d_wp.as<Xyzz<F>>();
+        j.perm = ld.perm.as<uint32_t>();
+        return FK_OK;
+    }
     const Need needs[] = {
         {&ln.digits, (size_t)p.W * n * 4}, {&ln.sorted, (size_t)p.W * n * 4}, {&ln.totals, WB * 4}, {&ln.starts, WB * 4},
         {&ln.perm, WB * 4 + SIZE_BINS * 4}, {&ln.overlist, OVER_MAX * sizeof(OverEntry) + sizeof(MsmDyn) + 64}, {j.have_sort ? &ln.buckets2 : &ln.buckets, WB * sizeof(Xyzz<F>)},
@@ -883,6 +915,7 @@
     bool grow = false;
     for (const Need &nd : needs) grow = grow || nd.bytes > nd.b->cap;
     if (grow) {
+        FK_TRY(lane_reclaim(ctx, ln, true));
         FK_HIP(ctx, hipStreamSynchronize(ln.st));
         for (const Need &nd : needs) FK_HIP(ctx, nd.b->reserve(nd.bytes));
         if (!j.have_sort) ln.last_sort_scalars = nullptr;
@@ -981,6 +1014,9 @@
 static Xyzz<F> *bucket_buf(const MsmJob<F> &j) { return (j.have_sort ? j.ln->buckets2 : j.ln->buckets).template as<Xyzz<F>>(); }
 
 template <class F>
+static int queue_overflow(const MsmJob<F> &j);
+
+template <class F>
 static int queue_accumulate(MsmJob<F> j) {
     fk_ctx *ctx = j.ctx;
     const MsmPlan &p = j.p;
@@ -988,7 +1024,7 @@
     constexpr int MINW = std::is_same<F, Fq>::value ? 4 : 2;
     Xyzz<F> *buckets = bucket_buf(j);
     std::vector<EventPair> &evv = (sizeof(F) == sizeof(Fq)) ? ctx->ev_acc : ctx->ev_acc2;
-    FK_TRY(stats_begin(ctx, evv, (uint64_t)j.n, st));
+    if (!j.uncounted) FK_TRY(stats_begin(ctx, evv, (uint64_t)j.n, st));
     if (j.merged)
         hipLaunchKernelGGL(HIP_KERNEL_NAME(msm_accumulate_merged_kernel<F, MINW>), dim3((p.B + 255) / 256), dim3(256), 0, st, j.bases, j.lev, j.sorted, j.n,
                            j.starts, j.totals, p.B, p.W, j.dyn, j.perm, j.perm + p.B, buckets);
@@ -996,36 +1032,55 @@
         hipLaunchKernelGGL(HIP_KERNEL_NAME(msm_accumulate_kernel<F, MINW>), dim3((unsigned)((j.WB + 255) / 256)), dim3(256), 0, st, j.bases, j.sorted, j.n,
                            j.starts, j.totals, p.B, p.W, j.dyn, j.perm, buckets);
     FK_HIP(ctx, hipGetLastError());
-    FK_TRY(stats_end(ctx, evv, st));
+    if (!j.uncounted) FK_TRY(stats_end(ctx, evv, st));
     if (!ctx->ev_acc_done) FK_HIP(ctx, hipEventCreateWithFlags(&ctx->ev_acc_done, hipEventDisableTiming));
     FK_HIP(ctx, hipEventRecord(ctx->ev_acc_done, st)); ctx->ev_acc_done_valid = true;
     FK_DBG_ST(ctx, st, "msm_accumulate");
+    if (j.lender) {
+        FK_TRY(queue_overflow<F>(j));
+        FK_HIP(ctx, hipMemcpyAsync((char *)j.tl->h_wp + j.wp_bytes, &j.dyn->adds, 8, hipMemcpyDeviceToHost, st));
+        FK_HIP(ctx, hipMemcpyAsync((char *)j.tl->h_wp + j.wp_bytes + 8, &j.dyn->error, 4, hipMemcpyDeviceToHost, st));
+        FK_HIP(ctx, hipEventRecord(j.lender->ev_lent, st));
+        j.lender->lent_valid = true;
+        if (j.lender->lent_pending > 0) j.lender->lent_pending--;
+    }
+    return FK_OK;
+}
+
+template <class F>
+static int queue_overflow(const MsmJob<F> &j) {
+    using FC = typename ColdOf<F>::type;
+    fk_ctx *ctx = j.ctx;
+    MsmLane &ln = *j.ln;
+    hipStream_t st = ln.st;
+    hipLaunchKernelGGL(HIP_KERNEL_NAME(msm_overflow_kernel<F, FC>), dim3(2048), dim3(64), 0, st,
+                       j.bases, j.lev, j.sorted, j.n, j.starts, j.totals, j.p.B, j.dyn, j.tasks, ln.partials.as<Xyzz<FC>>());
+    FK_HIP(ctx, hipGetLastError());
+    FK_DBG_ST(ctx, st, "msm_overflow");
+    hipLaunchKernelGGL(HIP_KERNEL_NAME(msm_overflow_fold_kernel<F>), dim3(256), dim3(256), 0, st, j.obs, j.dyn, ln.partials.as<Xyzz<F>>(), bucket_buf(j));
+    FK_HIP(ctx, hipGetLastError());
+    FK_DBG_ST(ctx, st, "msm_overflow_fold");
     return FK_OK;
 }
 
 template <class F>
 static int queue_tail(MsmJob<F> j) {
-    using FC = typename ColdOf<F>::type;
     fk_ctx *ctx = j.ctx;
     const MsmPlan &p = j.p;
     MsmLane &ln = *j.ln;
     MsmTail &tl = *j.tl;
     hipStream_t st = ln.st;
     Xyzz<F> *buckets = bucket_buf(j);
-    hipLaunchKernelGGL(HIP_KERNEL_NAME(msm_overflow_kernel<F, FC>), dim3(2048), dim3(64), 0, st,
-                       j.bases, j.lev, j.sorted, j.n, j.starts, j.totals, p.B, j.dyn, j.tasks, ln.partials.as<Xyzz<FC>>());
-    FK_HIP(ctx, hipGetLastError());
-    FK_DBG_ST(ctx, st, "msm_overflow");
-    hipLaunchKernelGGL(HIP_KERNEL_NAME(msm_overflow_fold_kernel<F>), dim3(256), dim3(256), 0, st, j.obs, j.dyn, ln.partials.as<Xyzz<F>>(), buckets);
-    FK_HIP(ctx, hipGetLastError());
-    FK_DBG_ST(ctx, st, "msm_overflow_fold");
+    if (!j.lender) FK_TRY(queue_overflow<F>(j));
     hipLaunchKernelGGL(HIP_KERNEL_NAME(msm_bucket_reduce_kernel<F>), dim3(p.nblk, j.WR), dim3(256), 0, st, buckets, p.B, p.L, p.T, p.nblk, j.winparts);
     Xyzz<F> *folded = j.winparts + (size_t)j.WR * p.nblk;
     hipLaunchKernelGGL(HIP_KERNEL_NAME(msm_fold_partials_kernel<F>), dim3(j.WR), dim3(256), 0, st, j.winparts, p.nblk, folded);
     FK_HIP(ctx, hipGetLastError());
     FK_HIP(ctx, hipMemcpyAsync(tl.h_wp, folded, j.wp_bytes, hipMemcpyDeviceToHost, st));
-    FK_HIP(ctx, hipMemcpyAsync((char *)tl.h_wp + j.wp_bytes, &j.dyn->adds, 8, hipMemcpyDeviceToHost, st));
-    FK_HIP(ctx, hipMemcpyAsync((char *)tl.h_wp + j.wp_bytes + 8, &j.dyn->error, 4, hipMemcpyDeviceToHost, st));
+    if (!j.lender) {
+        FK_HIP(ctx, hipMemcpyAsync((char *)tl.h_wp + j.wp_bytes, &j.dyn->adds, 8, hipMemcpyDeviceToHost, st));
+        FK_HIP(ctx, hipMemcpyAsync((char *)tl.h_wp + j.wp_bytes + 8, &j.dyn->error, 4, hipMemcpyDeviceToHost, st));
+    }
     FK_HIP(ctx, hipEventRecord(tl.done, st));
     FK_DBG_ST(ctx, st, "msm_bucket_reduce");
     return FK_OK;
@@ -1039,8 +1094,10 @@
 }
 
 template <class F>
-static int msm_begin(fk_ctx *ctx, const Affine<F> *d_bases, const Fr *d_scalars, size_t n, bool reuse_sort, int *tail_out, hipEvent_t ready, const KeyPre *pre = nullptr, bool defer = false) {
+static int msm_begin(fk_ctx *ctx, const Affine<F> *d_bases, const Fr *d_scalars, size_t n, bool reuse_sort, int *tail_out, hipEvent_t ready, const KeyPre *pre = nullptr, bool defer = false,
+                     int lender_li = -1, int own_li = -1, bool *adopted = nullptr, bool uncounted = false) {
     *tail_out = -1;
+    if (adopted) *adopted = false;
     if (n == 0) return FK_OK;
     if (n >= ((size_t)1 << 31)) FK_SET_ERR(ctx, FK_ERR_BAD_ARG, "msm: n too large");
     int ti = -1;
@@ -1056,11 +1113,21 @@
     }
     MsmLane &prev = ctx->lanes[ctx->lane_prev];
     const bool have_sort = reuse_sort && prev.st && prev.last_sort_scalars == (const void *)d_scalars && prev.last_sort_n == n && prev.last_sort_c == p.c && prev.last_merged == merged;
-    const int li = have_sort ? ctx->lane_prev : ctx->lane_next;
+    MsmLane *lender = nullptr;
+    if (lender_li >= 0) {
+        if (lender_li >= MSM_LANES || own_li < 0 || own_li >= MSM_LANES) return FK_OK;
+        MsmLane &ld = ctx->lanes[lender_li];
+        if (lender_li == own_li || !ld.st || !ctx->lanes[own_li].st || ld.last_sort_scalars != (const void *)d_scalars || ld.last_sort_n != n ||
+            ld.last_sort_c != p.c || ld.last_merged != merged) return FK_OK;
+        lender = &ld;
+        *adopted = true;
+    }
+    const int li = lender ? own_li : (have_sort ? ctx->lane_prev : ctx->lane_next);
     MsmLane &ln = ctx->lanes[li];
     if (!ln.st) FK_SET_ERR(ctx, FK_ERR_HIP, "msm: the context's streams were not created");
-    lanes_advance(ctx, li, defer);
-    if (ready) FK_HIP(ctx, hipStreamWaitEvent(ln.st, ready, 0));
+    if (!lender) lanes_advance(ctx, li, defer);
+    if (lender) FK_HIP(ctx, hipStreamWaitEvent(ln.st, lender->ev_sorted, 0));
+    else if (ready) FK_HIP(ctx, hipStreamWaitEvent(ln.st, ready, 0));
     else {
         FK_HIP(ctx, hipEventRecord(ln.ev_in, ctx->stream));
         FK_HIP(ctx, hipStreamWaitEvent(ln.st, ln.ev_in, 0));
@@ -1068,9 +1135,11 @@
     MsmJob<F> job{};
     job.ctx = ctx; job.p = p; job.ln = &ln; job.tl = &tl;
     job.bases = d_bases; job.lev = merged ? (const Affine<F> *)pre->lev : nullptr; job.scalars = d_scalars;
-    job.n = n; job.merged = merged; job.have_sort = have_sort;
+    job.n = n; job.merged = merged; job.have_sort = have_sort || lender; job.lender = lender; job.uncounted = uncounted;
     FK_TRY(msm_reserve(job));
-    if (!have_sort) {
+    if (lender) lender->lent_pending++;
+    else if (!have_sort) {
+        FK_TRY(lane_reclaim(ctx, ln, false));
         FK_TRY(queue_sort(job));
         FK_TRY(queue_size_order(job));
         FK_HIP(ctx, hipEventRecord(ln.ev_sorted, ln.st)); ln.ev_sorted_valid = true;
@@ -1133,6 +1202,7 @@
     if (ctx->aux) (void)hipStreamSynchronize(ctx->aux);
     for (int i = 0; i < MSM_TAILS; i++) ctx->tails[i].active = false;
     for (MsmLane &ln : ctx->lanes) { if (ln.st) (void)hipStreamSynchronize(ln.st); ln.last_sort_scalars = nullptr; }
+    for (MsmLane &ln : ctx->lanes) { ln.lent_pending = 0; ln.lent_valid = false; }
 }
 
 void msm_release(fk_ctx *ctx) {
@@ -1150,6 +1220,7 @@
             b->release();
         if (ln.ev_in) (void)hipEventDestroy(ln.ev_in);
         if (ln.ev_sorted) (void)hipEventDestroy(ln.ev_sorted);
+        if (ln.ev_lent) (void)hipEventDestroy(ln.ev_lent);
         if (ln.st) (void)hipStreamDestroy(ln.st);
         ln = MsmLane();
     }
@@ -1162,8 +1233,12 @@
     }
 }
 
-int msm_g1_begin(fk_ctx *ctx, const G1Affine *d_bases, const Fr *d_scalars, size_t n, int *tail, hipEvent_t ready, const KeyPre *pre, bool defer) {
-    return msm_begin<Fq>(ctx, d_bases, d_scalars, n, false, tail, ready, pre, defer);
+int msm_g1_begin(fk_ctx *ctx, const G1Affine *d_bases, const Fr *d_scalars, size_t n, int *tail, hipEvent_t ready, const KeyPre *pre, bool defer, bool uncounted) {
+    return msm_begin<Fq>(ctx, d_bases, d_scalars, n, false, tail, ready, pre, defer, -1, -1, nullptr, uncounted);
+}
+int msm_g1_begin_adopt(fk_ctx *ctx, const G1Affine *d_bases, const Fr *d_scalars, size_t n, int lender, int lane, bool *adopted, int *tail, const KeyPre *pre, bool defer) {
+    if (lender < 0 || lane < 0 || !adopted) FK_SET_ERR(ctx, FK_ERR_BAD_ARG, "msm: no lender lane");
+    return msm_begin<Fq>(ctx, d_bases, d_scalars, n, false, tail, nullptr, pre, defer, lender, lane, adopted);
 }
 int msm_g1_end(fk_ctx *ctx, int tail, G1Xyzz *out) { return msm_end<Fq>(ctx, tail, out); }
 int msm_g2_begin(fk_ctx *ctx, const G2Affine *d_bases, const Fr *d_scalars, size_t n, bool reuse_sort, int *tail, hipEvent_t ready, const KeyPre *pre, bool defer) {
@@ -1211,6 +1286,7 @@
     job.scalars = d_scalars; job.n = n; job.merged = merged;
     const MsmPlan &p = job.p;
     FK_TRY(msm_reserve(job));
+    FK_TRY(lane_reclaim(ctx, ln, true));
     FK_TRY(queue_sort(job));
     FK_TRY(queue_size_order(job));
     ln.last_sort_scalars = nullptr;
@@ -1268,6 +1344,12 @@
 
 void key_pre_free(fk_key *k) {
     for (KeyPre *p : {&k->pre_h, &k->pre_l, &k->pre_a, &k->pre_b1, &k->pre_b2}) { if (p->lev) (void)hipFree(p->lev); *p = KeyPre(); }
+    std::lock_guard<std::mutex> lock(k->a_pad_mu);
+    for (fk_key::APad &c : k->a_pad) {
+        if (c.pre.lev) (void)hipFree(c.pre.lev);
+        if (c.d) (void)hipFree(c.d);
+        c = fk_key::APad();
+    }
 }
 
 static size_t proof_scratch_still_needed(fk_ctx *ctx, const fk_key *k) {
@@ -1362,6 +1444,99 @@
     return FK_OK;
 }
 
+
+__global__ __launch_bounds__(256) void query_fingerprint_kernel(const uint32_t *idx, size_t n, unsigned long long *out) {
+    unsigned long long mine = 0;
+    for (size_t i = (size_t)blockIdx.x * 256 + threadIdx.x; i < n; i += (size_t)gridDim.x * 256) {
+        unsigned long long z = ((unsigned long long)i << 32 | idx[i]) + 0x9E3779B97F4A7C15ull;
+        z = (z ^ (z >> 30)) * 0xBF58476D1CE4E5B9ull;
+        z = (z ^ (z >> 27)) * 0x94D049BB133111EBull;
+        mine += z ^ (z >> 31);
+    }
+    const unsigned long long all = wave_sum_u64(mine);
+    if ((threadIdx.x & 63) == 0) atomicAdd(out, all);
+}
+int query_fingerprint(fk_ctx *ctx, const uint32_t *d_idx, size_t n, uint64_t *out) {
+    unsigned long long *d = nullptr;
+    FK_HIP(ctx, hipMalloc((void **)&d, 8));
+    unsigned long long h = 0;
+    hipError_t e = hipMemsetAsync(d, 0, 8, ctx->stream);
+    if (e == hipSuccess && n) {
+        hipLaunchKernelGGL(query_fingerprint_kernel, dim3((unsigned)std::min<size_t>((n + 255) / 256, 1024)), dim3(256), 0, ctx->stream, d_idx, n, d);
+        e = hipGetLastError();
+    }
+    if (e == hipSuccess) e = hipMemcpyAsync(&h, d, 8, hipMemcpyDeviceToHost, ctx->stream);
+    if (e == hipSuccess) e = hipStreamSynchronize(ctx->stream);
+    (void)hipFree(d);
+    FK_HIP(ctx, e);
+    *out = (uint64_t)h + 0x5bd1e995u * (uint64_t)n;
+    return FK_OK;
+}
+
+__global__ __launch_bounds__(256) void a_pad_scatter_kernel(const G1Affine *a, const uint32_t *idx, size_t v_in, size_t n_a, size_t n_l, G1Affine *pad) {
+    const size_t k = v_in + (size_t)blockIdx.x * 256 + threadIdx.x;
+    if (k >= n_a) return;
+    const size_t v = idx[k];
+    if (v >= v_in && v - v_in < n_l) pad[v - v_in] = a[k];
+}
+
+static bool share_al_sort() {
+    static const bool on = [] { const char *e = getenv("FK_PROVE_SHARE_AL_SORT"); return !e || atoi(e) != 0; }();
+    return on;
+}
+
+int key_a_pad(fk_ctx *ctx, const fk_key *key, const QueryIdx *qi, const fk_key::APad **pad) {
+    *pad = nullptr;
+    if (!share_al_sort() || !key || !qi || !qi->a || !qi->a_fp_valid) return FK_OK;
+    const size_t v_in = key->num_input, n_l = key->l_hi - key->l_lo, n_a = key->n_a;
+    if (key->a_lo != 0 || key->a_hi != key->n_a || key->l_lo != 0 || key->l_hi != key->n_l || key->n_l != key->num_aux || !v_in || !n_l || n_a < v_in || qi->n_a != n_a || !key->d_a || !key->d_l) return FK_OK;
+    if (key->m > ((uint64_t)1 << 25)) return FK_OK;
+    const bool l_merged = key->pre_l.lev != nullptr, a_merged = key->pre_a.lev != nullptr;
+    std::lock_guard<std::mutex> lock(key->a_pad_mu);
+    fk_key::APad *slot = nullptr;
+    for (fk_key::APad &c : key->a_pad) {
+        if (c.used && c.fp == qi->a_fp && c.n_a == n_a && c.n_l == n_l) {
+            if (!c.refused && c.d && (c.pre.lev != nullptr) == l_merged) *pad = &c;
+            return FK_OK;
+        }
+        if (!c.used && !slot) slot = &c;
+    }
+    if (!slot) return FK_OK;
+    fk_key::APad c;
+    c.used = true; c.refused = true; c.fp = qi->a_fp; c.n_a = n_a; c.n_l = n_l;
+    const std::string warnings = ctx->err;
+    auto done = [&](int rc) -> int { *slot = c; ctx->err = rc == FK_OK ? warnings : ctx->err; return rc; };
+    if (a_merged != l_merged) return done(FK_OK);
+    const size_t pad_bytes = n_l * sizeof(G1Affine) + 64;
+    if (l_merged) {
+        const MsmPlan p = make_plan(n_l, ctx->window_bits, true);
+        const size_t lev_bytes = (size_t)(p.W - 1) * n_l * sizeof(G1Affine);
+        size_t fr = 0, tot = 0;
+        FK_HIP(ctx, hipMemGetInfo(&fr, &tot));
+        if (pad_bytes + lev_bytes + proof_scratch_still_needed(ctx, key) + ((size_t)2 << 30) > fr) return done(FK_OK);
+    }
+    if (hipMalloc((void **)&c.d, pad_bytes) != hipSuccess) { (void)hipGetLastError(); c.d = nullptr; return done(FK_OK); }
+    hipError_t e = hipMemsetAsync(c.d, 0, pad_bytes, ctx->stream);
+    if (e == hipSuccess && n_a > v_in) {
+        hipLaunchKernelGGL(a_pad_scatter_kernel, dim3((unsigned)((n_a - v_in + 255) / 256)), dim3(256), 0, ctx->stream, key->d_a, qi->a, v_in, n_a, n_l, c.d);
+        e = hipGetLastError();
+    }
+    if (e == hipSuccess) e = hipStreamSynchronize(ctx->stream);
+    if (e != hipSuccess) { (void)hipFree(c.d); c.d = nullptr; (void)done(FK_ERR_HIP); FK_HIP(ctx, e); }
+    if (l_merged) {
+        const int rc = precompute_levels<Fq>(ctx, c.d, n_l, &c.pre, "a (padded to l)", false, 0);
+        if (rc != FK_OK || !c.pre.lev || c.pre.W != key->pre_l.W || c.pre.cb != key->pre_l.cb || c.pre.wide != key->pre_l.wide) {
+            if (c.pre.lev) { (void)hipFree(c.pre.lev); c.pre = KeyPre(); }
+            (void)hipFree(c.d); c.d = nullptr;
+            return done(rc);
+        }
+    }
+    c.refused = false;
+    (void)done(FK_OK);
+    *pad = slot;
+    return FK_OK;
+}
+
 static __host__ __device__ inline uint64_t splitmix64(uint64_t &s) {
     s += 0x9E3779B97F4A7C15ull;
     uint64_t z = s;
diff --git a/fawkes-crypto_amd/csrc/prover.hip b/fawkes-crypto_amd/csrc/prover.hip
--- a/fawkes-crypto_amd/csrc/prover.hip
+++ b/fawkes-crypto_amd/csrc/prover.hip
@@ -2,6 +2,7 @@
 #include <signal.h>
 #include <unistd.h>
 #include "common.hpp"
+#include "../../include/fawkes_hip_inspect.h"
 #include <chrono>
 #include <mutex>
 #include <string.h>
@@ -342,6 +343,20 @@
     return FK_OK;
 }
 
+int fk_key_a_pad_info(const fk_key *k, uint64_t out[6]) {
+    if (!k || !out) return FK_ERR_BAD_ARG;
+    for (int i = 0; i < 6; i++) out[i] = 0;
+    std::lock_guard<std::mutex> lock(k->a_pad_mu);
+    for (const fk_key::APad &c : k->a_pad) {
+        if (!c.used) continue;
+        out[4]++;
+        if (c.refused || !c.d) { out[3]++; continue; }
+        out[0]++; out[1] = c.n_l; out[2] = c.pre.lev ? c.pre.W : 0;
+        out[5] += (c.n_l + 1) * sizeof(G1Affine) + (c.pre.lev ? (uint64_t)(c.pre.W - 1) * c.pre.n * sizeof(G1Affine) : 0);
+    }
+    return FK_OK;
+}
+
 int fk_key_levels_plan(const fk_key *k, double out[15]) {
     if (!k || !out) return FK_ERR_BAD_ARG;
     const KeyPre *p[5] = {&k->pre_h, &k->pre_l, &k->pre_a, &k->pre_b1, &k->pre_b2};
@@ -453,12 +468,15 @@
     lanes_choose(ctx, key);
     FK_HIP(ctx, hipSetDevice(ctx->device));
     const uint32_t v_in = key->num_input, v_aux = key->num_aux;
-    for (int i = 0; i < 4; i++) ctx->wit_tail[i] = -1;
+    for (int i = 0; i < 5; i++) ctx->wit_tail[i] = -1;
+    const fk_key::APad *pad = nullptr;
+    FK_TRY(key_a_pad(ctx, key, q.idx, &pad));
+    const bool share_al = pad != nullptr;
     auto body = [&]() -> int {
         hipStream_t ax = opt.gather_on_main ? ctx->stream : ctx->aux;
         if (z_ready && !opt.gather_on_main) FK_HIP(ctx, hipStreamWaitEvent(ax, z_ready, 0));
         FK_HIP(ctx, ctx->sc_b.reserve(((size_t)v_in + v_aux) * sizeof(Fr)));
-        FK_HIP(ctx, ctx->sc_a.reserve(((size_t)v_in + v_aux) * sizeof(Fr)));
+        if (!share_al) FK_HIP(ctx, ctx->sc_a.reserve(((size_t)v_in + v_aux) * sizeof(Fr)));
         Fr *sb = ctx->sc_b.as<Fr>(), *sa = ctx->sc_a.as<Fr>();
         if (const QueryIdx *qi = q.idx) {
             if (qi->n_b != key->n_b) FK_SET_ERR(ctx, FK_ERR_KEY_MISMATCH, "prove: b query needs %llu points, key holds %llu",
@@ -475,7 +493,7 @@
                     if (c_hi < hi) FK_TRY(gather_scalars(ctx, d_z, qi->b + c_hi, hi - c_hi, sb + c_hi, ax));
                 }
             }
-            FK_TRY(gather_scalars(ctx, d_z, qi->a + key->a_lo, key->a_hi - key->a_lo, sa + key->a_lo, ax));
+            if (!share_al) FK_TRY(gather_scalars(ctx, d_z, qi->a + key->a_lo, key->a_hi - key->a_lo, sa + key->a_lo, ax));
         } else {
             uint64_t n_b_in = 0, n_b_aux = 0, n_a_aux = 0;
             FK_TRY(compact_scalars(ctx, d_z, q.d_b_in, v_in, sb, &n_b_in, ax));
@@ -491,6 +509,24 @@
         FK_TRY(msm_g1_begin(ctx, key->d_b1, sb + key->b_lo, key->b_hi - key->b_lo, &ctx->wit_tail[0], ctx->ev_aux, &key->pre_b1, opt.defer_back));
         FK_TRY(msm_g2_begin(ctx, key->d_b2, sb + key->b2_lo, key->b2_hi - key->b2_lo, key->b2_lo == key->b_lo && key->b2_hi == key->b_hi,
                             &ctx->wit_tail[1], ctx->ev_aux, &key->pre_b2, opt.defer_back));
+        if (share_al) {
+            FK_TRY(msm_g1_begin(ctx, key->d_a, d_z, v_in, &ctx->wit_tail[4], z_ready ? z_ready : ctx->ev_aux, nullptr, false, true));
+            const int a_lane = ctx->lane_prev;
+            FK_TRY(msm_g1_begin(ctx, key->d_l, d_z + v_in, key->l_hi - key->l_lo, &ctx->wit_tail[2], z_ready ? z_ready : ctx->ev_aux, &key->pre_l, opt.defer_back));
+            const int l_lane = ctx->lane_prev;
+            bool adopted = false;
+            FK_TRY(msm_g1_begin_adopt(ctx, pad->d, d_z + v_in, key->l_hi - key->l_lo, l_lane, a_lane, &adopted, &ctx->wit_tail[3], &pad->pre, opt.defer_back));
+            if (adopted) return FK_OK;
+            G1Xyzz drop;
+            FK_TRY(msm_g1_end(ctx, ctx->wit_tail[4], &drop));
+            ctx->wit_tail[4] = -1;
+            FK_HIP(ctx, ctx->sc_a.reserve(((size_t)v_in + v_aux) * sizeof(Fr)));
+            sa = ctx->sc_a.as<Fr>();
+            FK_TRY(gather_scalars(ctx, d_z, q.idx->a, key->n_a, sa, ax));
+            FK_HIP(ctx, hipEventRecord(ctx->ev_aux, ax));
+            FK_TRY(msm_g1_begin(ctx, key->d_a, sa, key->n_a, &ctx->wit_tail[3], ctx->ev_aux, &key->pre_a, opt.defer_back));
+            return FK_OK;
+        }
         FK_TRY(msm_g1_begin(ctx, key->d_l, d_z + v_in + key->l_lo, key->l_hi - key->l_lo, &ctx->wit_tail[2], z_ready ? z_ready : ctx->ev_aux, &key->pre_l, opt.defer_back));
         FK_TRY(msm_g1_begin(ctx, key->d_a, sa + key->a_lo, key->a_hi - key->a_lo, &ctx->wit_tail[3], ctx->ev_aux, &key->pre_a, opt.defer_back));
         return FK_OK;
@@ -503,11 +539,11 @@
 
 extern "C++" {
 namespace fk {
-int early_witness_begin(fk_ctx *ctx, const fk_key *key, const void *d_z, const WitnessQueries &q, int tails_out[4]) {
+int early_witness_begin(fk_ctx *ctx, const fk_key *key, const void *d_z, const WitnessQueries &q, int tails_out[5]) {
     if (!early_front_applies(key)) return 0;
     const int rc = witness_begin(ctx, key, (const Fr *)d_z, q, ctx->ev_z, FrontOpts{true, true});
     if (rc != FK_OK) return -rc;
-    memcpy(tails_out, ctx->wit_tail, 4 * sizeof(int));
+    memcpy(tails_out, ctx->wit_tail, 5 * sizeof(int));
     return 1;
 }
 bool early_front_applies(const fk_key *key) {
@@ -523,13 +559,15 @@
         ctx->wit_active = false;
         tails = ctx->wit_tail;
     }
-    const int tw[4] = {tails[0], tails[1], tails[2], tails[3]};
-    G1Xyzz H = G1Xyzz::inf(), L, A, B1; G2Xyzz B2;
+    const int tw[5] = {tails[0], tails[1], tails[2], tails[3], tails[4]};
+    G1Xyzz H = G1Xyzz::inf(), L, A, A_in, B1; G2Xyzz B2;
     auto body = [&]() -> int {
         FK_TRY(msm_g1_end(ctx, tw[0], &B1));
         FK_TRY(msm_g2_end(ctx, tw[1], &B2));
         FK_TRY(msm_g1_end(ctx, tw[2], &L));
         FK_TRY(msm_g1_end(ctx, tw[3], &A));
+        FK_TRY(msm_g1_end(ctx, tw[4], &A_in));
+        A.add(A_in);
         if (tail_h >= 0) FK_TRY(msm_g1_end(ctx, tail_h, &H));
         return FK_OK;
     };
@@ -600,7 +638,7 @@
         if (rch != FK_OK) { msm_abandon(ctx); return rch; }
         const double t2w = now_ms();
         if (gate && run.before_block) {
-            int mine[4];
+            int mine[5];
             memcpy(mine, ctx->wit_tail, sizeof mine);
             ctx->wit_active = false;
             int rce;
diff --git a/fawkes-crypto_amd/csrc/spmv.hip b/fawkes-crypto_amd/csrc/spmv.hip
--- a/fawkes-crypto_amd/csrc/spmv.hip
+++ b/fawkes-crypto_amd/csrc/spmv.hip
@@ -565,6 +565,9 @@
         if ((ia.size() && hipMemcpy(r->d_idx_a, ia.data(), ia.size() * 4, hipMemcpyHostToDevice) != hipSuccess) ||
             (ib.size() && hipMemcpy(r->d_idx_b, ib.data(), ib.size() * 4, hipMemcpyHostToDevice) != hipSuccess)) { ctx->err = "r1cs: upload failed"; return fail(FK_ERR_HIP); }
         r->qidx.a = r->d_idx_a; r->qidx.b = r->d_idx_b; r->qidx.n_a = ia.size(); r->qidx.n_b = ib.size();
+        const int rcf = query_fingerprint(ctx, r->d_idx_a, ia.size(), &r->qidx.a_fp);
+        if (rcf != FK_OK) return fail(rcf);
+        r->qidx.a_fp_valid = true;
     }
     *out = r;
     return FK_OK;
@@ -913,7 +916,7 @@
     const size_t mb = key->m * sizeof(Fr);
     if (mb > ctx->stage_a.cap || mb > ctx->stage_b.cap || mb > ctx->stage_c.cap) return FK_OK;
     FK_HIP(ctx, hipEventRecord(ctx->ev_z, ctx->stream));
-    int tails[4];
+    int tails[5];
     const int wb = early_witness_begin(ctx, key, d_z, r1cs_queries(r), tails);
     if (wb < 0) return -wb;
     if (wb == 0) return FK_OK;
diff --git a/include/fawkes_hip_inspect.h b/include/fawkes_hip_inspect.h
--- a/include/fawkes_hip_inspect.h
+++ b/include/fawkes_hip_inspect.h
@@ -8,6 +8,8 @@
 int fk_r1cs_alias_info(const fk_r1cs_dev *r1cs, uint64_t out[4]);
 int fk_r1cs_aliases(const fk_r1cs_dev *r1cs, uint64_t cap, uint32_t *dst_mtx, uint32_t *dst_row, uint32_t *src_mtx, uint32_t *src_row);
 
+int fk_key_a_pad_info(const fk_key *key, uint64_t out[6]);
+
 #ifdef __cplusplus
 }
 #endif
```

Result: faster. 4.527, median of 6 (+1.6%).
